# Eurus-Holmes/VAG-NMT

Hardware: AMD Instinct MI355X
Metric: training sentence-pairs/sec (Multi30K en->de, B=64) (higher is better)
Workload: dtype f32; 1 GPU; configs[1]: multimodal en->de train step, B=64/GPU, Ts=Tt=40, E=256, H=512, S=512, I=2048, Vs=8507, V=9391, dropout 0.3/0.5/0.5, tied emb, teacher_force_ratio=1; global_batch=64, parallelism=dp1, hip_graph=True

## Files before the change

include/vag_nmt.h:

```cpp
#ifndef VAG_NMT_H
#define VAG_NMT_H
#include <stddef.h>
#include <stdint.h>

#ifdef __cplusplus
extern "C" {
#endif

typedef void* vag_stream_t;

typedef struct { const float *w_ih, *w_hh, *b_ih, *b_hh; } vag_gru_w;
typedef struct { float *w_ih, *w_hh, *b_ih, *b_hh; } vag_gru_g;

typedef struct {
    const float* emb;
    vag_gru_w gru1;
    const float *attn_h, *attn_v, *c2h;
    vag_gru_w gru2;
} vag_dec_w;
typedef struct {
    float* emb;
    vag_gru_g gru1;
    float *attn_h, *attn_v, *c2h;
    vag_gru_g gru2;
// ... 328 lines not shown
#define VAG_ADAM_SCRATCH_SKIPPED_OFFSET 28
#define VAG_ADAM_SCRATCH_GUARD_OFFSET 32
int vag_clip_adam_flat(float* p, float* g, float* m, float* v, int64_t n, int nseg, const int64_t* seg_off,
                       const float* seg_lr, const float* seg_wd, float clip, float grad_scale, float beta1,
                       float beta2, float eps, int zero_grad, int32_t* step, float* norm_out, void* scratch,
                       const float* lr_dev, vag_stream_t stream);

int vag_clip_adam_shard(float* p, float* g, float* m, float* v, int64_t n, int nseg, const int64_t* seg_off,
                        const float* seg_lr, const float* seg_wd, float clip, float grad_scale, float beta1,
                        float beta2, float eps, int zero_grad, int32_t* step, float* norm_out, void* scratch,
                        const float* lr_dev, int64_t lo, int64_t hi, int phase, double* sumsq, vag_stream_t stream);

typedef struct {
    const float* enc_emb;
    vag_gru_w enc_fw, enc_bw;
    const float *im_w, *im_b, *txt_w, *txt_b, *ctx2ctx, *emb2ctx, *mlp_w;
    const float *ini_w, *ini_b;
    const float* attn_e;
    vag_dec_w dec;
    vag_head_w head;
} vag_model_w;
typedef struct {
    float* enc_emb;
    vag_gru_g enc_fw, enc_bw;
    float *im_w, *im_b, *txt_w, *txt_b, *ctx2ctx, *emb2ctx, *mlp_w;
    float *ini_w, *ini_b;
    float* attn_e;
    vag_dec_g dec;
    vag_head_g head;
} vag_model_g;
typedef struct {
    int64_t B, Ts, Tt, Es, Et, H, S, I, V, ldl;
    int32_t multimodal;
    int32_t attn_method;
    int32_t activation_vse;
    int32_t rank_kind;
    int32_t free_run;
    int32_t storage;
    float margin, loss_w, init_split, p_emb, p_ctx, p_out;
    int32_t loss_ring;
    void* guard;
    float label_smoothing;
    int32_t mrt_n;
    float mrt_alpha, mrt_scale;
    const float *mrt_cost, *mrt_valid;
} vag_step_cfg;
int64_t vag_step_ws_floats(const vag_step_cfg* cfg);
int64_t vag_step_ws_offset(const vag_step_cfg* cfg, int which);
int vag_train_step(const vag_step_cfg* cfg, const vag_model_w* w, const vag_model_g* g, const int64_t* src,
                   const int32_t* lengths, const int64_t* tgt, const float* im, const float* vocab_weight, uint64_t* rng,
                   const float* derived, float* ws, float* losses, int phases, vag_stream_t stream);
int vag_set_operator_context(const float* derived, int storage);
int vag_set_option(const char* name, int64_t value);
int vag_copy4(const void* const* src, void* const* dst, const int64_t* bytes, int n, vag_stream_t stream);
int64_t vag_derived_floats(int64_t H);
int vag_derive_weights(vag_dec_w w, const float* enc_whh_fw, const float* enc_whh_bw, int64_t H, int with_fp16,
                       float* derived, vag_stream_t stream);

int vag_recurrence_supported(int kind, int64_t B, int64_t Ts, int64_t Tt, int64_t H);
int vag_persistent_timeouts(void);
int vag_set_operator_guard(void* guard);
int vag_recurrence_time(int kind, double* ms_total, int* launches);
int vag_gemm_group_plan(int n, const int64_t* M, const int64_t* N, const int64_t* K, const int* accumulate, int* split, int* order);
int64_t vag_recurrence_sync_words(int kind, int64_t B, int64_t T);
int vag_cgru_recurrence_fwd(const float* pe, const float* mask, const float* h0, const float* xp1, vag_dec_w w, const float* wcat,
                            const float* bcat, const float* encwp, int64_t B, int64_t Ts, int64_t Tt, int64_t H, float* h1,
                            float* g1, float* qhp, float* alpha, float* h2_all, float* g2, float* psc, void* sync,
                            vag_stream_t stream);

#define VAG_COMM_ID_BYTES 128
typedef struct vag_comm_s* vag_comm_t;
int vag_comm_unique_id(void* id);
int vag_comm_init(vag_comm_t* comm, int nranks, int rank, const void* id);
int vag_comm_allreduce(vag_comm_t comm, float* buf, int64_t n, vag_stream_t stream);
int vag_comm_size(vag_comm_t comm);
int vag_comm_destroy(vag_comm_t comm);

int vag_dropout_mask(const uint64_t* rng, int which, int64_t n, float p, float* out, vag_stream_t stream);
int vag_rng_advance(uint64_t* rng, vag_stream_t stream);

#ifdef __cplusplus
}
#endif
#endif
```

vag-nmt_amd/csrc/api.hip:

```cpp
#include "../../include/vag_nmt.h"
#include "kernels.h"
#include <cstring>

#define S_(x) reinterpret_cast<hipStream_t>(x)

static inline int zero_async(void* p, size_t bytes, hipStream_t s) {
    if (bytes == 0) return VAG_OK;
    return vag_axpy_launch(0.f, reinterpret_cast<const float*>(p), reinterpret_cast<float*>(p), (int64_t)(bytes / 4), 2, s);
}
static inline int copy_async(void* dst, const void* src, size_t bytes, hipStream_t s) {
    if (bytes == 0) return VAG_OK;
    return vag_axpy_launch(1.f, reinterpret_cast<const float*>(src), reinterpret_cast<float*>(dst), (int64_t)(bytes / 4), 0, s);
}
static int linear_fwd(int64_t M, int64_t N, int64_t K, const float* x, int64_t ldx, const float* W, const float* bias,
                      int act, float* y, int64_t ldy, hipStream_t s) {
    if (M <= 256) return vag_skinny_launch(M, N, K, x, ldx, W, K, bias, nullptr, 0, y, ldy, act, s);
    return vag_gemm_launch(M, N, K, 1.f, x, ldx, 1, W, 1, K, 0.f, y, ldy, bias, act, s);
}
static int gemm_tn_acc(int64_t M, int64_t N, int64_t R, const float* A, int64_t lda, const float* B, int64_t ldb, float* C,
                       int64_t ldc, hipStream_t s, float* g_bias = nullptr) {
    if (R == 0) return VAG_OK;
    return vag_gemm_launch(M, N, R, 1.f, A, 1, lda, B, ldb, 1, 1.f, C, ldc, nullptr, VAG_ACT_NONE, s, 0, g_bias);
}
static int gemm_nn(int64_t M, int64_t N, int64_t K, const float* A, int64_t lda, const float* B, int64_t ldb, float beta,
// ... 4 lines not shown

static thread_local VagCallCtx g_base_ctx;
static thread_local VagCallCtx* g_active_ctx = nullptr;
VagCallCtx& vag_ctx() { return g_active_ctx ? *g_active_ctx : g_base_ctx; }
VagCallScope::VagCallScope(VagCallCtx& c) : ctx(c), prev(g_active_ctx) { g_active_ctx = &c; }
VagCallScope::~VagCallScope() {
    (void)vag_loss_defer_flush();
    if (ctx.leaf_on) vag_leaf_drop();
    g_active_ctx = prev;
}
static inline const float* as_f(const vag_half* p) { return reinterpret_cast<const float*>(p); }

static bool head_grads_one_plane() {
    return vag_opt().head_bf16_grads != 0 && vag_ctx().store16;
}
static int head_dt_gemm(int64_t R, int64_t E, int64_t V, const float* dlogits, int64_t ldl, const float* out_w, float* dt,
                        hipStream_t s, const void* dl16 = nullptr) {
    if (dl16) return vag_gemm_launch_planes(1, R, E, V, 1.f, reinterpret_cast<const float*>(dl16), ldl, 1, out_w, E, 1, 0.f, dt, E, s, 1);
    if (head_grads_one_plane() && R > 128) return vag_gemm_launch_planes(1, R, E, V, 1.f, dlogits, ldl, 1, out_w, E, 1, 0.f, dt, E, s);
    return gemm_nn(R, E, V, dlogits, ldl, out_w, E, 0.f, dt, E, s);
}
static int head_outw_gemm(int64_t V, int64_t E, int64_t R, const float* dlogits, int64_t ldl, const float* tmid, float* g_out_w,
                          hipStream_t s, const void* dl16 = nullptr) {
    if (R == 0) return VAG_OK;
    if (dl16) return vag_gemm_launch_planes(1, V, E, R, 1.f, reinterpret_cast<const float*>(dl16), 1, ldl, tmid, E, 1, 1.f, g_out_w, E, s, 1);
    if (head_grads_one_plane() && R > 128) return vag_gemm_launch_planes(1, V, E, R, 1.f, dlogits, 1, ldl, tmid, E, 1, 1.f, g_out_w, E, s);
    return gemm_tn_acc(V, E, R, dlogits, ldl, tmid, E, g_out_w, E, s);
}

static void* head_dl16_slot(float* logits, int64_t ldl, int64_t R, int64_t CH, int64_t E) {
    if (!head_grads_one_plane() || CH <= 128 || vag_opt().head_bf16_dlogits == 0) return nullptr;
    if (E <= 64 || vag_opt().gemm_f32mfma != 0 || vag_opt().gemm_force_tile != 0) return nullptr;
    if (CH * 3 > R * 2) return nullptr;
    return logits + CH * ldl;
}

VagOptions& vag_opt() {
    static VagOptions o;
    return o;
}

extern "C" {

int vag_version(void) { return 330; }

int vag_set_option(const char* name, int64_t value) {
    VAG_CHECK_ARG(name != nullptr);
    VagOptions& o = vag_opt();
    const struct { const char* n; int* p; } ints[] = {
        {"gemm_f32mfma", &o.gemm_f32mfma}, {"gemm_slabs", &o.gemm_slabs}, {"gemm_nogroup", &o.gemm_nogroup}, {"gemm_big", &o.gemm_big}, {"gemm_force_tile", &o.gemm_force_tile},
        {"gemm_force_splitk", &o.gemm_force_splitk}, {"head_fuse", &o.head_fuse},
        {"head_bf16_grads", &o.head_bf16_grads}, {"persistent", &o.persistent}, {"persistent_dec_bwd", &o.persistent_dec_bwd}, {"persistent_enc_bwd", &o.persistent_enc_bwd}, {"free_persistent", &o.free_persistent}, {"attn_dot_reg", &o.attn_dot_reg},
        {"persist_timing", &o.persist_timing}, {"s16_one_plane", &o.s16_one_plane}, {"leaf_queue", &o.leaf_queue}, {"attn_row", &o.attn_row}, {"dec_xcd_map", &o.dec_xcd_map}, {"loss_ride", &o.loss_ride}, {"step_fork", &o.step_fork},
        {"head_bf16_dlogits", &o.head_bf16_dlogits}};
    for (const auto& e : ints)
        if (strcmp(name, e.n) == 0) { *e.p = (int)value; return VAG_OK; }
    if (strcmp(name, "head_chunk") == 0) { o.head_chunk = value; return VAG_OK; }
    if (strcmp(name, "persist_spin_limit") == 0) { o.persist_spin_limit = value; return VAG_OK; }
#ifdef VAG_LAB
    if (strcmp(name, "dec_stamps") == 0) { o.dec_stamps = value; return VAG_OK; }
    if (strcmp(name, "dec_bwd_stamps") == 0) { o.dec_bwd_stamps = value; return VAG_OK; }
    if (strcmp(name, "gemm_debug") == 0) { o.gemm_debug = (int)value; return VAG_OK; }
    if (strcmp(name, "gemm_planes") == 0) {
        g_base_ctx.gemm_planes = (value == 2 || value == 1 || value == 11) ? (int)value : 3;
        return VAG_OK;
    }
#endif
    return VAG_EINVAL;
}

int vag_set_operator_context(const float* derived, int storage) {
    VAG_CHECK_ARG(storage == 0 || (storage == 1 && derived));
    g_base_ctx.derived = derived;
    g_base_ctx.store16 = storage == 1;
    g_base_ctx.gemm_planes = storage == 1 ? 2 : 3;
    return VAG_OK;
}

int vag_gemm_f32(int64_t M, int64_t N, int64_t K, float alpha, const float* A, int64_t sam, int64_t sak, const float* B,
                 int64_t sbk, int64_t sbn, float beta, float* C, int64_t ldc, const float* bias, int act,
                 vag_stream_t stream) {
    return vag_gemm_launch(M, N, K, alpha, A, sam, sak, B, sbk, sbn, beta, C, ldc, bias, act, S_(stream));
}

int vag_linear_fwd(int64_t M, int64_t N, int64_t K, const float* x, const float* W, const float* bias, int act, float* y,
                   vag_stream_t stream) {
    VAG_CHECK_ARG(x && W && y && M >= 0 && N > 0 && K > 0);
    return linear_fwd(M, N, K, x, K, W, bias, act, y, N, S_(stream));
}

int vag_linear_bwd(int64_t M, int64_t N, int64_t K, const float* x, const float* W, const float* y, float* dy, int act,
                   float* d_x, int accumulate_dx, float* g_W, float* g_b, vag_stream_t stream) {
    hipStream_t s = S_(stream);
    VAG_CHECK_ARG(x && W && dy && M >= 0 && N > 0 && K > 0 && (!act || y));
    if (M == 0) return VAG_OK;
    if (act) VAG_TRY(vag_tanh_bwd_launch(y, dy, dy, M * N, nullptr, 0, 0.f, s));
    if (d_x) VAG_TRY(gemm_nn(M, K, N, dy, N, W, K, accumulate_dx ? 1.f : 0.f, d_x, K, s));
    if (g_W) VAG_TRY(gemm_tn_acc(N, K, M, dy, N, x, K, g_W, K, s));
    if (g_b) VAG_TRY(vag_colsum_launch(dy, M, N, N, g_b, s));
    return VAG_OK;
}

int vag_embed_fwd(const int64_t* idx, int64_t n, const float* W, int64_t E, float* out, vag_stream_t stream) {
    return vag_embed_gather_launch(idx, 1, 0, n, 1, W, E, out, nullptr, 0, 0.f, S_(stream));
}
int vag_embed_bwd(const int64_t* idx, int64_t n, const float* d_out, int64_t E, float* g_W, vag_stream_t stream) {
    return vag_embed_scatter_launch(idx, 1, 0, n, 1, d_out, E, g_W, nullptr, 0, 0.f, S_(stream));
}

struct DerivedW {
    float *prep, *wcatT, *whh1T, *encT;
    vag_half *wcat16, *wcatT16, *whh1_16, *whh1T16, *enc16, *encT16;
    int64_t total;
};
static int64_t cgru_prep_total(int64_t H);
static DerivedW derived_layout(float* p, int64_t H) {
    DerivedW w;
    const int64_t C = 2 * H, Q = C + 3 * H;
    WsCarver c(p);
    w.prep = c.take(cgru_prep_total(H)); w.wcatT = c.take(Q * H); w.whh1T = c.take(3 * H * H); w.encT = c.take(2 * 3 * H * H);
    w.wcat16 = c.take_as<vag_half>(Q * H); w.wcatT16 = c.take_as<vag_half>(Q * H);
    w.whh1_16 = c.take_as<vag_half>(3 * H * H); w.whh1T16 = c.take_as<vag_half>(3 * H * H);
    w.enc16 = c.take_as<vag_half>(2 * 3 * H * H); w.encT16 = c.take_as<vag_half>(2 * 3 * H * H);
    w.total = c.off;
    return w;
}

struct BiGruWs {
    float *x, *xp, *hst, *gates, *dgh, *carry, *dx, *whhT, *gx;
    unsigned *sync, *sync_b;
    int64_t total;
};
static BiGruWs bigru_ws(float* ws, int64_t B, int64_t Ts, int64_t E, int64_t H) {
    BiGruWs w;
    WsCarver c(ws);
    w.x = c.take(Ts * B * E);
    w.xp = c.take(Ts * B * 6 * H);
    w.hst = c.take(2 * (Ts + 1) * B * H);
    w.gates = c.take(2 * Ts * 4 * B * H);
    w.dgh = c.take(2 * Ts * B * 3 * H);
    w.carry = c.take(4 * B * H);
    w.dx = c.take(Ts * B * E);
    w.whhT = c.take(2 * 3 * H * H);
    w.gx = c.take(3 * Ts * B * H);
    w.sync = c.take_as<unsigned>(vag_enc_persistent_sync_words(B, Ts));
    w.sync_b = c.take_as<unsigned>(vag_enc_persistent_sync_words(B, Ts));
    w.total = c.off;
    return w;
}
int64_t vag_bigru_ws_floats(int64_t B, int64_t Ts, int64_t E, int64_t H) { return bigru_ws(nullptr, B, Ts, E, H).total; }

int vag_bigru_seq_fwd(const int64_t* src, const int32_t* lengths, const float* emb, vag_gru_w fw, vag_gru_w bw, float p_emb,
                      float p_ctx, const uint64_t* rng, int64_t B, int64_t Ts, int64_t E, int64_t H, float* enc,
                      float* mask, float* ws, vag_stream_t stream) {
    hipStream_t s = S_(stream);
    VAG_CHECK_ARG(src && lengths && emb && enc && mask && ws && B > 0 && Ts > 0 && E > 0 && H > 0);
    VAG_CHECK_ARG(E % 4 == 0 && H % 4 == 0 && aligned16(ws) && aligned16(enc));
    VAG_CHECK_ARG(fw.w_ih && fw.w_hh && fw.b_ih && fw.b_hh && bw.w_ih && bw.w_hh && bw.b_ih && bw.b_hh);
    BiGruWs w = bigru_ws(ws, B, Ts, E, H);
    const int64_t R = Ts * B;
    VAG_TRY(vag_embed_gather_launch(src, 1, Ts, Ts, B, emb, E, w.x, rng, VAG_DROP_ENC_EMB, p_emb, s, mask));
    VagGemmGroup grp0;
    VAG_TRY(vag_gemm_launch(R, 3 * H, E, 1.f, w.x, E, 1, fw.w_ih, 1, E, 0.f, w.xp, 6 * H, fw.b_ih, 0, s));
    VAG_TRY(vag_gemm_launch(R, 3 * H, E, 1.f, w.x, E, 1, bw.w_ih, 1, E, 0.f, w.xp + 3 * H, 6 * H, bw.b_ih, 0, s));
    VAG_TRY(grp0.end(s));
    const int64_t BH = B * H;
    const bool s16 = vag_ctx().store16 && vag_ctx().derived;
    VAG_CHECK_ARG(!vag_ctx().store16 || (vag_ctx().derived && H % 8 == 0));
    if (!s16 && vag_opt().persistent && vag_enc_persistent_ok(B, Ts, H)) {
        return vag_enc_fwd_persistent_launch(w.xp, fw.w_hh, bw.w_hh, fw.b_hh, bw.b_hh, lengths, w.hst, w.gates, enc, w.sync, rng,
                                             p_ctx, B, Ts, H, s);
    }
    const vag_half* w16 = s16 ? derived_layout(const_cast<float*>(vag_ctx().derived), H).enc16 : nullptr;
    if (s16 && vag_opt().persistent && vag_enc_wide16_ok(B, Ts, H) && B >= 64) {
        return vag_enc_fwd_wide16_launch(w.xp, w16, w16 + 3 * H * H, fw.b_hh, bw.b_hh, lengths, w.hst, w.gates, enc,
                                         reinterpret_cast<vag_half*>(w.dgh), w.sync, rng, p_ctx, B, Ts, H, s);
    }
    {
        const VagJob zj[2] = {{nullptr, w.hst, B, H, H, H, 0}, {nullptr, w.hst + (Ts + 1) * BH, B, H, H, H, 0}};
        VAG_TRY(vag_jobs_launch(zj, 2, s));
    }
    GruStepArgs a = {};
    a.lda = H; a.ldw = H; a.ldother = 6 * H; a.ldh = H; a.ld2 = Ts * 2 * H;
    a.M = (int)B; a.K = (int)H; a.H = (int)H; a.lengths = lengths; a.comp_hidden = 1;
    for (int64_t k = 0; k < Ts; ++k) {
        for (int d = 0; d < 2; ++d) {
            const int64_t t = d == 0 ? k : Ts - 1 - k;
            const vag_gru_w& g = d == 0 ? fw : bw;
            float* hs = w.hst + d * (Ts + 1) * BH;
            GruSide& sd = a.s[d];
            sd.A = hs + k * BH; sd.W = s16 ? as_f(w16 + d * 3 * H * H) : g.w_hh; sd.bias = g.b_hh;
            sd.other = w.xp + t * B * 6 * H + d * 3 * H;
            sd.hprev = hs + k * BH; sd.hout = hs + (k + 1) * BH;
            sd.out2 = enc + t * 2 * H + d * H;
            sd.save = w.gates + (d * Ts + k) * 4 * BH;
            sd.t = (int)t;
        }
        VAG_TRY(vag_gru_step_launch(a, 2, s, s16));
    }
    VAG_TRY(vag_dropout_apply_launch(enc, B * Ts * 2 * H, 0, rng, VAG_DROP_ENC_CTX, p_ctx, s));
    return VAG_OK;
}

int vag_bigru_seq_bwd(const int64_t* src, const int32_t* lengths, vag_gru_w fw, vag_gru_w bw, float p_emb, float p_ctx,
                      const uint64_t* rng, int64_t B, int64_t Ts, int64_t E, int64_t H, float* d_enc, float* ws,
                      float* g_emb, vag_gru_g g_fw, vag_gru_g g_bw, vag_stream_t stream) {
    hipStream_t s = S_(stream);
    VAG_CHECK_ARG(src && lengths && d_enc && ws && g_emb && B > 0 && Ts > 0 && E % 4 == 0 && H % 4 == 0);
    BiGruWs w = bigru_ws(ws, B, Ts, E, H);
    const int64_t R = Ts * B, BH = B * H;
    float* d_xp = w.xp;
    const float* whhT = w.whhT;
    const bool s16 = vag_ctx().store16 && vag_ctx().derived;
    VAG_CHECK_ARG(!vag_ctx().store16 || (vag_ctx().derived && H % 8 == 0));
    if (s16) {
        whhT = as_f(derived_layout(const_cast<float*>(vag_ctx().derived), H).encT16);
    } else if (vag_ctx().derived) {
        whhT = derived_layout(const_cast<float*>(vag_ctx().derived), H).encT;
    } else {
        for (int d = 0; d < 2; ++d) {
            const vag_gru_w& g = d == 0 ? fw : bw;
            VAG_TRY(vag_transpose_launch(g.w_hh, 3 * H, H, w.whhT + d * 3 * H * H, s));
        }
    }
    const bool pers_on = vag_opt().persistent && vag_opt().persistent_enc_bwd;
    const bool wide16 = s16 && pers_on && vag_enc_wide16_ok(B, Ts, H) && B >= 64;
    const bool persist = wide16 || (!s16 && pers_on && (H == 512 || H == 256) && vag_enc_persistent_ok(B, Ts, H));
    if (wide16) {
        VAG_TRY(vag_enc_bwd_wide16_launch(reinterpret_cast<const vag_half*>(whhT), d_enc, w.gates, w.hst, lengths, rng, p_ctx, d_xp,
                                          w.dgh, reinterpret_cast<vag_half*>(w.gx), w.sync_b, B, Ts, H, s));
    } else if (persist) {
        VAG_TRY(vag_enc_bwd_persistent_launch(whhT, d_enc, w.gates, w.hst, lengths, rng, p_ctx, d_xp, w.dgh, w.sync_b, B, Ts, H, s));
    }
    GruBwdArgs a = {};
    a.ld_add = Ts * 2 * H; a.ldh = H; a.ldgi = 6 * H; a.ldgh = 3 * H;
    a.M = (int)B; a.H = (int)H; a.lengths = lengths; a.rng = rng; a.sid = VAG_DROP_ENC_CTX; a.p = p_ctx;
    int cur = 0;
    auto cell_of = [&](auto& sd, int d, int64_t k) {
        const int64_t t = d == 0 ? k : Ts - 1 - k;
        sd.dh_add = d_enc + t * 2 * H + d * H;
        sd.drop_idx0 = t * 2 * H + d * H;
        sd.save = w.gates + (d * Ts + k) * 4 * BH;
        sd.hprev = w.hst + (d * (Ts + 1) + k) * BH;
        sd.dgi = d_xp + t * B * 6 * H + d * 3 * H;
        sd.dgh = w.dgh + (d * Ts + k) * B * 3 * H;
        sd.t = (int)t;
    };
    for (int d = 0; d < 2; ++d) {
        GruBwdSide& sd = a.s[d];
        cell_of(sd, d, Ts - 1);
        sd.dh_carry = nullptr;
        sd.dh_prev = w.carry + (d * 2 + cur) * BH;
    }
    if (!persist) VAG_TRY(vag_gru_bwd_elem_launch(a, 2, s));
    GruBwdStepArgs f = {};
    f.lda = 3 * H; f.ldw = 3 * H; f.ld_add = Ts * 2 * H; f.ldh = H; f.ldgi = 6 * H; f.ldgh = 3 * H;
    f.M = (int)B; f.K = (int)(3 * H); f.H = (int)H; f.lengths = lengths; f.rng = rng; f.sid = VAG_DROP_ENC_CTX; f.p = p_ctx;
    f.has_cell = 1;
    for (int64_t k = Ts - 1; k >= 1 && !persist; --k) {
        for (int d = 0; d < 2; ++d) {
            GruBwdStepSide& sd = f.s[d];
            cell_of(sd, d, k - 1);
            sd.A = w.dgh + (d * Ts + k) * B * 3 * H;
            sd.WT = s16 ? as_f(reinterpret_cast<const vag_half*>(whhT) + d * 3 * H * H) : whhT + d * 3 * H * H;
            sd.addend = w.carry + (d * 2 + cur) * BH;
            sd.dh_direct = w.carry + (d * 2 + (cur ^ 1)) * BH;
            sd.dh_out = nullptr;
        }
        VAG_TRY(vag_gru_bwd_step_launch(f, 2, s, s16));
        cur ^= 1;
    }
    VagGemmGroup grp1;
    for (int d = 0; d < 2; ++d) {
        const vag_gru_g& gg = d == 0 ? g_fw : g_bw;
        const float* dgh = w.dgh + d * Ts * B * 3 * H;
        const float* hs = w.hst + d * (Ts + 1) * BH;
        VAG_TRY(gemm_tn_acc(3 * H, H, R, dgh, 3 * H, hs, H, gg.w_hh, H, s, gg.b_hh));
        VAG_TRY(gemm_tn_acc(3 * H, E, R, d_xp + d * 3 * H, 6 * H, w.x, E, gg.w_ih, E, s, gg.b_ih));
    }
    VAG_TRY(grp1.end(s));
    if (!vag_ctx().step_zeroed) VAG_TRY(zero_async(w.dx, R * E * sizeof(float), s));
    VagGemmGroup grp2;
    for (int d = 0; d < 2; ++d)
        VAG_TRY(gemm_nn(R, E, 3 * H, d_xp + d * 3 * H, 6 * H, (d == 0 ? fw : bw).w_ih, E, 1.f, w.dx, E, s));
    VAG_TRY(grp2.end(s));
// ... 407 lines not shown
    return cgru_bwd_scratch(scratch, B, Ts, Tt, E, H).du_all;
}
extern "C" {
int64_t vag_cgru_bwd_scratch_floats(int64_t B, int64_t Ts, int64_t Tt, int64_t E, int64_t H) {
    return cgru_bwd_scratch(nullptr, B, Ts, Tt, E, H).total;
}

int vag_cgru_attn_decode_seq_bwd_loop(const float* enc, const float* pe, const float* mask, const float* h0, const int64_t* tok,
                                 vag_dec_w w, int64_t B, int64_t Ts, int64_t Tt, int64_t E, int64_t H, int64_t V,
                                 const float* h2_all, const float* c_all, const float* e_all, float* d_h2_all,
                                 float* d_c_all, const float* d_e_all, float* ws, float* d_enc_out, int accumulate_enc,
                                 float* d_pe, float* d_h0, float* scratch, vag_stream_t stream) {
    hipStream_t s = S_(stream);
    VAG_CHECK_ARG(enc && pe && mask && h0 && tok && h2_all && c_all && e_all && d_h2_all && d_c_all && ws && d_enc_out &&
                  d_pe && d_h0 && scratch && dec_w_ok(w));
    VAG_CHECK_ARG(B > 0 && Ts > 0 && Tt > 0 && E % 4 == 0 && H % 4 == 0 && aligned16(ws) && aligned16(scratch));
    (void)V; (void)mask; (void)d_e_all;
    const int64_t C = 2 * H, Q = C + 3 * H, BH = B * H;
    CgruWs k = cgru_ws(ws, B, Ts, Tt, E, H);
    CgruPrep p = cgru_prep(k.prep, H);
    CgruBwdScratch z = cgru_bwd_scratch(scratch, B, Ts, Tt, E, H);
    const bool s16 = vag_ctx().store16;
    VAG_CHECK_ARG(!s16 || (vag_ctx().derived && H % 8 == 0));
    if (vag_ctx().derived) {
        DerivedW dw = derived_layout(const_cast<float*>(vag_ctx().derived), H);
        p = cgru_prep(dw.prep, H);
        z.wcatT = dw.wcatT; z.whh1T = dw.whh1T;
        if (s16) {
            z.wcatT = const_cast<float*>(as_f(dw.wcatT16)); z.whh1T = const_cast<float*>(as_f(dw.whh1T16));
        }
    } else {
        VAG_TRY(vag_transpose_launch(p.wcat, Q, H, z.wcatT, s));
        VAG_TRY(vag_transpose_launch(w.gru1.w_hh, 3 * H, H, z.whh1T, s));
    }
    const bool persist = !s16 && vag_opt().persistent && vag_opt().persistent_dec_bwd && vag_dec_bwd_persistent_ok(B, Ts, Tt, H);
    if (!persist) {
        GruBwdArgs a = {};
        a.ld_add = H; a.ldh = H; a.ldgi = 3 * H; a.ldgh = Q; a.M = (int)B; a.H = (int)H;
        const int64_t t = Tt - 1;
        GruBwdSide& sd = a.s[0];
        sd.dh_carry = nullptr; sd.dh_add = d_h2_all + t * BH; sd.drop_idx0 = 0;
        sd.save = k.g2 + t * 4 * BH; sd.hprev = k.h1 + t * BH;
        sd.dgi = z.dgi2 + t * B * 3 * H; sd.dgh = z.dqgh + t * B * Q + C; sd.dh_prev = z.dh1d; sd.t = 0;
        VAG_TRY(vag_gru_bwd_elem_launch(a, 1, s));
    }
    GruBwdStepArgs f = {};
    f.ld_add = H; f.ldh = H; f.M = (int)B; f.H = (int)H; f.lengths = nullptr; f.rng = nullptr; f.sid = 0; f.p = 0.f;
    if (C % 4 == 0 && aligned16(enc) && aligned16(d_c_all) && B < 65536)
        VAG_TRY(vag_skinny_batched_launch(B, Tt, Ts, C, d_c_all, B * C, C, enc, C, Ts * C, z.dah, B * Ts, Ts, s));
    else
        VAG_TRY(vag_attn_scores_ex_launch(1, enc, d_c_all, C, nullptr, nullptr, Tt * B, 1, B, Ts, C, nullptr, z.dah, s));
    if (persist) {
        VAG_TRY(vag_dec_bwd_persistent_launch(pe, k.encwp, w.attn_v, z.wcatT, z.whh1T, h0, h2_all, k.h1, k.g1, k.g2, k.qhp, k.alpha,
                                              d_h2_all, z.dah, z.dgi2, z.dqgh, z.ds, z.dgi1, z.dgh1, d_h0, k.dal, k.sync_b, B, Ts, Tt, H,
                                              s));
    }
    for (int64_t t = Tt - 1; t >= 0 && !persist; --t) {
        float* dgi2 = z.dgi2 + t * B * 3 * H;
        float* dqgh = z.dqgh + t * B * Q;
        const float* wside = s16 ? as_f(reinterpret_cast<const vag_half*>(z.wcatT) + C) : z.wcatT + C;
        VAG_TRY(vag_attn_dot_side_launch(1, k.encwp, dgi2, 3 * H, nullptr, nullptr, z.dah + t * B * Ts, B, Ts, 3 * H, z.dalpha,
                                         B, H, 3 * H, dqgh + C, Q, wside, Q, nullptr, z.dh1d, z.pbuf, H, s, s16));
        VAG_TRY(vag_attn_dq_launch(pe, k.qhp + t * B * Q, Q, w.attn_v, k.alpha + t * B * Ts, z.dalpha, z.ds + t * B * Ts, B,
                                   Ts, C, dqgh, Q, s, s16));
        f.lda = Q; f.ldw = Q; f.K = (int)C; f.ldgi = 3 * H; f.ldgh = 3 * H; f.has_cell = 1;
        GruBwdStepSide& sd = f.s[0];
        sd.A = dqgh; sd.WT = z.wcatT; sd.addend = z.pbuf; sd.dh_add = nullptr; sd.drop_idx0 = 0;
        sd.save = k.g1 + t * 4 * BH; sd.hprev = (t == 0) ? h0 : h2_all + (t - 1) * BH;
        sd.dgi = z.dgi1 + t * B * 3 * H; sd.dgh = z.dgh1 + t * B * 3 * H; sd.dh_direct = z.carry; sd.dh_out = nullptr; sd.t = 0;
        VAG_TRY(vag_gru_bwd_step_launch(f, 1, s, s16));
        f.lda = 3 * H; f.ldw = 3 * H; f.K = (int)(3 * H);
        sd.A = z.dgh1 + t * B * 3 * H; sd.WT = z.whh1T; sd.addend = z.carry;
        if (t > 0) {
            const int64_t t1 = t - 1;
            f.has_cell = 1; f.ldgi = 3 * H; f.ldgh = Q;
            sd.dh_add = d_h2_all + t1 * BH;
            sd.save = k.g2 + t1 * 4 * BH; sd.hprev = k.h1 + t1 * BH;
            sd.dgi = z.dgi2 + t1 * B * 3 * H; sd.dgh = z.dqgh + t1 * B * Q + C; sd.dh_direct = z.dh1d; sd.dh_out = nullptr;
        } else {
            f.has_cell = 0;
            sd.dh_add = nullptr; sd.save = nullptr; sd.hprev = nullptr; sd.dgi = nullptr; sd.dgh = nullptr;
            sd.dh_direct = nullptr; sd.dh_out = d_h0;
        }
        VAG_TRY(vag_gru_bwd_step_launch(f, 1, s, s16));
    }
    VAG_TRY(vag_attn_post_bwd_launch(pe, k.qhp, Q, w.attn_v, z.ds, k.alpha, d_c_all, B, Ts, Tt, C, d_pe, z.dvp, d_enc_out,
                                     accumulate_enc, s, s16));
    {
        VagGemmGroup now;
        VAG_TRY(gemm_nn(Tt * B, H, 3 * H, z.dgi2, 3 * H, w.gru2.w_ih, H, 0.f, z.du_all, H, s));
        VAG_TRY(now.end(s));
    }
    VAG_TRY(vag_attn_wsum_pair_launch(k.alpha, z.du_all, H, z.duk, k.uk, H, z.u_all, B, Ts, Tt, s));
    vag_ctx().u_all_ready = z.u_all;
    return gemm_nn(B * Ts, C, H, z.duk, H, w.c2h, C, 1.f, d_enc_out, C, s);
}

int vag_cgru_attn_decode_seq_bwd_weights(const float* h0, const int64_t* tok, vag_dec_w w, int64_t B, int64_t Ts, int64_t Tt,
                                         int64_t E, int64_t H, const float* h2_all, const float* c_all, const float* e_all,
                                         const float* d_e_all, float* ws, vag_dec_g g, float* scratch, vag_stream_t stream) {
    hipStream_t s = S_(stream);
    VAG_CHECK_ARG(h0 && tok && h2_all && c_all && e_all && ws && scratch && dec_w_ok(w));
    VAG_CHECK_ARG(g.emb && g.gru1.w_ih && g.gru1.w_hh && g.gru1.b_ih && g.gru1.b_hh && g.attn_h && g.attn_v && g.c2h &&
                  g.gru2.w_ih && g.gru2.w_hh && g.gru2.b_ih && g.gru2.b_hh);
    const int64_t C = 2 * H;
    CgruBwdScratch z = cgru_bwd_scratch(scratch, B, Ts, Tt, E, H);
    VagGemmGroup grp3;
    VAG_TRY(vag_colsum_launch(z.dvp, VAG_POST_CHUNKS(Ts) * B, C, C, g.attn_v, s));
// ... 858 lines not shown
                          int32_t* di_state, int64_t max_len, int64_t* tok_out, int64_t B, int64_t n, int64_t V, float temperature,
                          int64_t top_k, const uint64_t* rng, int32_t* n_alive, float top_p, int32_t* set_size,
                          vag_stream_t stream) {
    VAG_CHECK_ARG(di_state != nullptr);
    return vag_sample_step_p_launch(logp, ldl, M, toks, token_logp, 0, di_state, max_len, nullptr, nullptr, nullptr, tok_out, B, n,
                                    V, temperature, top_k, rng, n_alive, top_p, set_size, S_(stream));
}
int vag_sample_noise(const uint64_t* rng, int64_t di, int64_t N, int64_t V, float* out, vag_stream_t stream) {
    return vag_sample_noise_launch(rng, di, N, V, out, S_(stream));
}

int vag_mbr_supported(int64_t Nh, int64_t Lh, int64_t Nr, int64_t Lr) { return vag_mbr_supported_host(Nh, Lh, Nr, Lr); }
int vag_mbr_select(const int64_t* hyps, const int64_t* refs, const float* weights, int64_t B, int64_t Nh, int64_t Lh, int64_t Nr,
                   int64_t Lr, int utility, int32_t* matches, float* util, float* expected, int64_t* best, vag_stream_t stream) {
    return vag_mbr_select_launch(hyps, refs, weights, B, Nh, Lh, Nr, Lr, utility, matches, util, expected, best, S_(stream));
}

int vag_mrt_weights(const float* nll, const float* cost, const float* valid, int64_t B, int64_t Tt, int64_t N, float alpha, float scale,
                    float* inv_cnt, float* q, float* risk, vag_stream_t stream) {
    VAG_CHECK_ARG(risk != nullptr);
    return vag_mrt_weights_launch(nll, cost, valid, B, Tt, N, alpha, scale, inv_cnt, q, risk, nullptr, 0.f, 0, S_(stream));
}
int vag_mrt_pack(const int64_t* cand, int64_t G, int64_t Nc, int64_t L, const int64_t* gold, int64_t Tg, int include_gold, int64_t* tgt,
                 int64_t Tt, float* valid, vag_stream_t stream) {
    return vag_mrt_pack_launch(cand, G, Nc, L, gold, Tg, include_gold, tgt, Tt, valid, S_(stream));
}

int vag_clip_adam_flat(float* p, float* g, float* m, float* v, int64_t n, int nseg, const int64_t* seg_off,
                       const float* seg_lr, const float* seg_wd, float clip, float grad_scale, float beta1, float beta2,
                       float eps, int zero_grad, int32_t* step, float* norm_out, void* scratch, const float* lr_dev,
                       vag_stream_t stream) {
    return vag_clip_adam_launch(p, g, m, v, n, nseg, seg_off, seg_lr, seg_wd, clip, grad_scale, beta1, beta2, eps, zero_grad,
                                step, norm_out, scratch, lr_dev, S_(stream));
}

int vag_clip_adam_shard(float* p, float* g, float* m, float* v, int64_t n, int nseg, const int64_t* seg_off, const float* seg_lr,
                        const float* seg_wd, float clip, float grad_scale, float beta1, float beta2, float eps, int zero_grad,
                        int32_t* step, float* norm_out, void* scratch, const float* lr_dev, int64_t lo, int64_t hi, int phase,
                        double* sumsq, vag_stream_t stream) {
    return vag_clip_adam_shard_launch(p, g, m, v, n, nseg, seg_off, seg_lr, seg_wd, clip, grad_scale, beta1, beta2, eps, zero_grad,
                                      step, norm_out, scratch, lr_dev, lo, hi, phase, sumsq, S_(stream));
}

int vag_copy4(const void* const* src, void* const* dst, const int64_t* bytes, int n, vag_stream_t stream) {
    return vag_copy4_launch(src, dst, bytes, n, S_(stream));
}

int vag_recurrence_supported(int kind, int64_t B, int64_t Ts, int64_t Tt, int64_t H) {
    if (kind == 0) return vag_enc_persistent_ok(B, Ts, H) ? 1 : 0;
    if (kind == 1) return vag_dec_persistent_ok(B, Ts, Tt, H) ? 1 : 0;
    return 0;
}
int vag_persistent_timeouts(void) { return vag_persistent_timeouts_read(); }
int vag_set_operator_guard(void* guard) {
    VAG_CHECK_ARG((reinterpret_cast<uintptr_t>(guard) & 3) == 0);
    g_base_ctx.guard = reinterpret_cast<unsigned*>(guard);
    return VAG_OK;
}
int vag_gemm_group_plan(int n, const int64_t* M, const int64_t* N, const int64_t* K, const int* accumulate, int* split,
                        int* order) {
    return vag_gemm_group_plan_host(n, M, N, K, accumulate, split, order);
}
int vag_recurrence_time(int kind, double* ms_total, int* launches) { return vag_persistent_time_read(kind, ms_total, launches); }
int64_t vag_recurrence_sync_words(int kind, int64_t B, int64_t T) {
    return kind == 0 ? vag_enc_persistent_sync_words(B, T) : vag_dec_persistent_sync_words(B, T);
}
int vag_cgru_recurrence_fwd(const float* pe, const float* mask, const float* h0, const float* xp1, vag_dec_w w, const float* wcat,
                            const float* bcat, const float* encwp, int64_t B, int64_t Ts, int64_t Tt, int64_t H, float* h1,
                            float* g1, float* qhp, float* alpha, float* h2_all, float* g2, float* psc, void* sync,
                            vag_stream_t stream) {
    VAG_CHECK_ARG(dec_w_ok(w) && vag_dec_persistent_ok(B, Ts, Tt, H));
    return vag_dec_fwd_persistent_launch(pe, mask, h0, xp1, w.gru1.w_hh, w.gru1.b_hh, wcat, bcat, w.attn_v, encwp, w.gru2.b_ih, h1,
                                         g1, qhp, alpha, h2_all, g2, psc, reinterpret_cast<unsigned*>(sync), B, Ts, Tt, H,
                                         S_(stream));
}

int vag_dropout_mask(const uint64_t* rng, int which, int64_t n, float p, float* out, vag_stream_t stream) {
    VAG_CHECK_ARG(which >= 1 && which <= 3);
    return vag_dropout_mask_launch(rng, which, n, p, out, S_(stream));
}
int vag_rng_advance(uint64_t* rng, vag_stream_t stream) { return vag_rng_advance_launch(rng, S_(stream)); }

}
```

vag-nmt_amd/csrc/call_ctx.h:

```cpp
#pragma once
#include <hip/hip_runtime.h>
#include <stdint.h>
#include "../../include/vag_nmt.h"

struct LossTask {
    const float* nll = nullptr; const float* inv_cnt = nullptr; float* losses = nullptr;
    int B = 0, Tt = 0, has_vse = 0, ring = 0;
    float w_mt = 0.f, w_vse = 0.f;
};
struct RmwDefer {
    float* out = nullptr;
    const float *a1 = nullptr, *x1 = nullptr, *a2 = nullptr, *x2 = nullptr;
    const float *mask = nullptr, *dx = nullptr; float coef = 0.f;
    int64_t B = 0, Ts = 0, C = 0;
};

struct VagCallCtx {
    const float* derived = nullptr;
    bool store16 = false;
    int gemm_planes = 3;
    unsigned* guard = nullptr;

    int64_t head_chunk = 0;
    struct HeadFuse { const vag_head_g* g = nullptr; const float* d_loss = nullptr; float* dt = nullptr; bool done = false; } head_fuse;
    bool step_zeroed = false;
    bool step_gathered = false;
    bool poison_inject = false;
    bool persist_prezeroed = false;
    int loss_ring = 0;
    struct Mrt { int n = 0; float alpha = 0.f, scale = 0.f; const float* cost = nullptr; const float* valid = nullptr; } mrt;
    struct GemmScratch { float* slab = nullptr; int64_t floats = 0; unsigned* tickets = nullptr; int64_t ntickets = 0; hipStream_t stream = nullptr; } gemm_scratch;
    const float* gemm_prezeroed[4] = {nullptr, nullptr, nullptr, nullptr};
    struct LeafStream { hipStream_t stream = nullptr; hipEvent_t event = nullptr; bool used = false; } leaf_stream;

    struct RowMix { float* xmix = nullptr; float split = 0.f; const float* done = nullptr; } row_mix;
    struct Dh0Tanh { bool req = false; const float* done = nullptr; } dh0_tanh;
    struct LossDefer { bool on = false; LossTask task; hipStream_t stream = nullptr; } loss_defer;
    RmwDefer rmw;
    bool leaf_on = false;
    const float* u_all_ready = nullptr;
};

VagCallCtx& vag_ctx();

struct VagCallScope {
    VagCallCtx& ctx;
    VagCallCtx* prev;
    explicit VagCallScope(VagCallCtx& c);
    ~VagCallScope();
    VagCallScope(const VagCallScope&) = delete;
    VagCallScope& operator=(const VagCallScope&) = delete;
};
```

vag-nmt_amd/csrc/common.h:

```cpp
#pragma once
#include <hip/hip_runtime.h>
#include <stdint.h>
#include <stddef.h>

#define VAG_OK 0
#define VAG_EINVAL (-22)
#define VAG_ENOSYS (-38)

#define VAG_CHECK_ARG(cond)                     \
    do {                                        \
        if (!(cond)) return VAG_EINVAL;         \
    } while (0)

#define VAG_LAUNCH_CHECK()                                  \
    do {                                                    \
        hipError_t e__ = hipGetLastError();                 \
        if (e__ != hipSuccess) return (int)e__;             \
    } while (0)

#define VAG_TRY(expr)                  \
    do {                               \
        int r__ = (expr);              \
        if (r__ != 0) return r__;      \
    } while (0)
// ... 26 lines not shown
}
__device__ __forceinline__ float wave_sum(float v) { return wave_allreduce<false>(v); }
__device__ __forceinline__ float wave_max(float v) { return wave_allreduce<true>(v); }
__device__ __forceinline__ float vag_tanh(float x) {
    float e = __expf(2.0f * x);
    return 1.0f - 2.0f * __builtin_amdgcn_rcpf(e + 1.0f);
}
__device__ __forceinline__ float vag_sigmoid(float x) { return __builtin_amdgcn_rcpf(1.0f + __expf(-x)); }

__device__ __host__ __forceinline__ uint64_t vag_mix64(uint64_t z) {
    z += 0x9E3779B97F4A7C15ull;
    z = (z ^ (z >> 30)) * 0xBF58476D1CE4E5B9ull;
    z = (z ^ (z >> 27)) * 0x94D049BB133111EBull;
    return z ^ (z >> 31);
}
__device__ __forceinline__ float vag_drop_mul(const uint64_t* rng, uint32_t stream_id, uint64_t idx, float p) {
    if (rng == nullptr || p <= 0.0f) return 1.0f;
    uint64_t key = vag_mix64(rng[0] ^ (rng[1] * 0xD1342543DE82EF95ull) ^ ((uint64_t)stream_id << 56));
    uint64_t r = vag_mix64(key + idx);
    float u = (float)(r >> 40) * (1.0f / 16777216.0f);
    return (u >= p) ? 1.0f / (1.0f - p) : 0.0f;
}

typedef _Float16 vag_half;
__device__ __forceinline__ float h16_lo(unsigned p) { return (float)__builtin_bit_cast(vag_half, (unsigned short)(p & 0xffffu)); }
__device__ __forceinline__ float h16_hi(unsigned p) { return (float)__builtin_bit_cast(vag_half, (unsigned short)(p >> 16)); }
template <bool XH> __device__ __forceinline__ float4 ld4_any(const float* base, int64_t elem) {
    if (XH) {
        const uint2 p = *reinterpret_cast<const uint2*>(reinterpret_cast<const vag_half*>(base) + elem);
        return make_float4(h16_lo(p.x), h16_hi(p.x), h16_lo(p.y), h16_hi(p.y));
    }
    return *reinterpret_cast<const float4*>(base + elem);
}
template <bool XH> __device__ __forceinline__ float ld1_any(const float* base, int64_t elem) {
    if (XH) return (float)reinterpret_cast<const vag_half*>(base)[elem];
    return base[elem];
}

struct VagOptions {
    int gemm_f32mfma = 0;
    int gemm_big = 1;
    int gemm_slabs = 1;
    int gemm_nogroup = 0;
    int gemm_force_tile = 0;
    int gemm_force_splitk = 0;
    int gemm_debug = 0;
    int64_t head_chunk = -1;
    int head_fuse = 1;
    int head_bf16_grads = 1;
    int persistent = 1;
    int persistent_dec_bwd = 1;
    int persistent_enc_bwd = 1;
    int attn_dot_reg = 1;
    int free_persistent = 1;
    int s16_one_plane = 1;
    int head_bf16_dlogits = 1;
    int leaf_queue = 1;
    int attn_row = 1;
    int loss_ride = 1;
    int dec_xcd_map = 33;
    int step_fork = 0;
    int64_t persist_spin_limit = 0;
    int persist_timing = 0;
    int64_t dec_bwd_stamps = 0;
    int64_t dec_stamps = 0;
};
VagOptions& vag_opt();

enum { VAG_ACT_NONE = 0, VAG_ACT_TANH = 1 };
enum { VAG_DROP_ENC_EMB = 1, VAG_DROP_ENC_CTX = 2, VAG_DROP_DEC_OUT = 3 };

int vag_gemm_launch(int64_t M, int64_t N, int64_t K, float alpha, const float* A, int64_t sam, int64_t sak,
                    const float* B, int64_t sbk, int64_t sbn, float beta, float* C, int64_t ldc,
                    const float* bias, int act, hipStream_t stream, int c_half = 0,
                    float* rowsum = nullptr,
                    int a_bf16 = 0);
int vag_gemm_launch_planes(int planes, int64_t M, int64_t N, int64_t K, float alpha, const float* A, int64_t sam, int64_t sak,
                           const float* B, int64_t sbk, int64_t sbn, float beta, float* C, int64_t ldc, hipStream_t stream,
                           int a_bf16 = 0);
int64_t vag_logits_parts_count(int64_t M, int64_t N, int64_t K, const float* A, int64_t lda, const float* W, int64_t ldw);
int vag_logits_parts_launch(int64_t M, int64_t N, int64_t K, const float* A, int64_t lda, const float* W, int64_t ldw,
                            const float* bias, float* out, int64_t ldo, float* parts, hipStream_t stream);
int vag_skinny_launch(int64_t M, int64_t N, int64_t K, const float* A, int64_t lda, const float* W, int64_t ldw,
                      const float* bias, const float* addend, int64_t ldadd, float* out, int64_t ldo, int act,
                      hipStream_t stream, bool w16 = false);
int vag_attn_dot_side_launch(int mode, const float* x, const float* q, int64_t ldq, const float* v, const float* mask,
                             const float* addend, int64_t N, int64_t Ts, int64_t W, float* out, int64_t M, int64_t Np,
                             int64_t K, const float* A, int64_t lda, const float* Wt, int64_t ldw, const float* pbias,
                             const float* padd, float* P, int64_t ldp, hipStream_t stream, bool s16 = false);
int vag_skinny_gather_launch(int64_t M, int64_t N, int64_t K, const float* table, int64_t ldt, const int64_t* idx, const float* W,
                             int64_t ldw, const float* bias, float* out, int64_t ldo, float* gathered, int64_t ldg,
                             hipStream_t stream);
int vag_skinny3_launch(int64_t M, int64_t N, const float* const* A, const int64_t* lda, const float* const* W, const int64_t* ldw,
                       const int64_t* K, const float* const* bias, float* out, int64_t ldo, int act, const uint64_t* rng, int sid,
                       float p, int64_t drop_idx0, hipStream_t stream, const float* addend = nullptr, int64_t ldadd = 0,
                       const float* addend2 = nullptr, const int64_t* idx2 = nullptr, int64_t ldadd2 = 0);
int vag_skinny_batched_launch(int64_t nb, int64_t M, int64_t N, int64_t K, const float* A, int64_t lda, int64_t bsA,
                              const float* W, int64_t ldw, int64_t bsW, float* out, int64_t ldo, int64_t bsO,
                              hipStream_t stream);
int vag_skinny_nn_launch(int64_t M, int64_t N, int64_t K, const float* A, int64_t lda, const float* B, int64_t ldb,
                         float beta, float* C, int64_t ldc, hipStream_t stream,
                         float* out2 = nullptr, int64_t ldo2 = 0, float scale2 = 0.f, int acc2 = 0);
void vag_gemm_group_begin();
int vag_gemm_group_end(hipStream_t stream);
void vag_gemm_group_abort();
struct VagGemmGroup {
// ... 59 lines not shown
```

vag-nmt_amd/csrc/kernels.h:

```cpp
#pragma once
#include "common.h"
#include "call_ctx.h"
#include "../../include/vag_nmt.h"

static inline int64_t round64(int64_t n) { return (n + 63) & ~63ll; }
struct WsCarver {
    float* base;
    int64_t off = 0;
    explicit WsCarver(float* b) : base(b) {}
    float* take(int64_t n) {
        float* q = base ? base + off : nullptr;
        off += round64(n);
        return q;
    }
    template <class T> T* take_as(int64_t n) {
        return reinterpret_cast<T*>(take((n * (int64_t)sizeof(T) + 3) / 4));
    }
};
struct DecTables {
    float *embp, *embw3, *encw2;
    unsigned long long* cand;
    int64_t total;
};
DecTables vag_dec_tables(float* base, int64_t B, int64_t Ts, int64_t Tt, int64_t E, int64_t H, int64_t V, bool token_only = false);
// ... 74 lines not shown
                        int64_t C, float* alpha, float* ctx, hipStream_t s);
int vag_softmax_bwd_launch(const float* alpha, const float* dalpha, int64_t N, int64_t Ts, float* dscore, hipStream_t s);
int vag_attn_dq_launch(const float* pe, const float* q, int64_t ldq, const float* v, const float* alpha,
                       const float* dalpha, float* dscore, int64_t N, int64_t Ts, int64_t C, float* dq, int64_t lddq,
                       hipStream_t s, bool x16 = false);
int vag_attn_post_bwd_launch(const float* pe, const float* q_all, int64_t ldq, const float* v, const float* ds_all,
                             const float* alpha_all, const float* dc_all, int64_t B, int64_t Ts, int64_t Tt,
                             int64_t C, float* d_pe, float* dvp, float* d_enc, int accumulate_enc, hipStream_t s,
                             bool x16 = false);
int vag_outer2_launch(const float* a1, const float* x1, const float* a2, const float* x2, int64_t B, int64_t Ts,
                      int64_t C, float* out, int accumulate, hipStream_t s);

inline bool vag_label_smoothing_ok(float eps) { return eps >= 0.f && eps < 1.f; }
int vag_lse_nll_launch(const float* logits, int64_t ldl, int64_t rows, int64_t V, const int64_t* tgt, int64_t B,
                       int64_t Tt, const float* vw, float* lse, float* nll, int64_t* argmax, int64_t argmax_stride,
                       float* logp_out, int64_t ldlp, hipStream_t s, float eps);
int vag_inv_cnt_launch(const int64_t* tgt, int64_t B, int64_t Tt, float* inv_cnt, hipStream_t s);
int vag_loss_mt_launch(const float* nll, const float* inv_cnt, int64_t B, int64_t Tt, float* loss, hipStream_t s);
int vag_loss_mt_mix_launch(const float* nll, const float* inv_cnt, int64_t B, int64_t Tt, float* losses, float w_mt,
                           float w_vse, int has_vse, hipStream_t s);
int vag_ce_bwd_launch(float* logits, int64_t ldl, int64_t rows, int64_t V, const int64_t* tgt, int64_t B, int64_t Tt,
                      const float* vw, const float* lse, const float* inv_cnt, const float* d_loss, hipStream_t s,
                      float eps);
int vag_ce_bwd_colsum_launch(float* logits, int64_t ldl, int64_t rows, int64_t V, const int64_t* tgt, int64_t B, int64_t Tt,
                             const float* vw, const float* lse, const float* inv_cnt, const float* d_loss, float* g_bias,
                             hipStream_t s, void* out16, float eps);

int vag_logsoftmax_bwd_launch(const float* logp, int64_t ldlp, float* d, int64_t ldd, int64_t rows, int64_t V,
                              hipStream_t s);

int vag_l2norm_fwd_launch(const float* y, int64_t B, int64_t S, float* nrm, float* out, hipStream_t s);
int vag_l2norm_bwd_launch(const float* y, const float* nrm, const float* out, const float* d_out, int64_t B, int64_t S,
                          int act, float* dy, hipStream_t s);
int vag_rank_loss_launch(const float* scores, int64_t B, float margin, int kind, float* G, float* loss, hipStream_t s,
                         const float* g_scale = nullptr);
int vag_retrieval_rank_launch(const float* scores, int64_t N, int* ranks, hipStream_t s);
int vag_scale_by_dev_launch(float* x, int64_t n, const float* scalar, hipStream_t s);

int vag_clip_adam_shard_launch(float* p, float* g, float* m, float* v, int64_t n, int nseg, const int64_t* seg_off,
                               const float* seg_lr, const float* seg_wd, float clip, float grad_scale, float beta1, float beta2,
                               float eps, int zero_grad, int32_t* step, float* norm_out, void* scratch, const float* lr_dev,
                               int64_t lo, int64_t hi, int phase, double* sumsq, hipStream_t s);
int vag_clip_adam_launch(float* p, float* g, float* m, float* v, int64_t n, int nseg, const int64_t* seg_off,
                         const float* seg_lr, const float* seg_wd, float clip, float grad_scale, float beta1,
                         float beta2, float eps, int zero_grad, int32_t* step, float* norm_out, void* scratch, const float* lr_dev,
                         hipStream_t s);

bool vag_enc_persistent_ok(int64_t B, int64_t Ts, int64_t H);
int64_t vag_enc_persistent_sync_words(int64_t B, int64_t Ts);
int vag_enc_fwd_persistent_launch(const float* xp, const float* w_fw, const float* w_bw, const float* b_fw, const float* b_bw,
                                  const int* lengths, float* hst, float* gates, float* enc, unsigned* sync, const uint64_t* rng,
                                  float p_ctx, int64_t B, int64_t Ts, int64_t H, hipStream_t s);
int vag_enc_bwd_persistent_launch(const float* whhT, const float* d_enc, const float* gates, const float* hst, const int* lengths,
                                  const uint64_t* rng, float p_ctx, float* d_xp, float* dgh, unsigned* sync, int64_t B, int64_t Ts,
                                  int64_t H, hipStream_t s);
bool vag_enc_wide16_ok(int64_t B, int64_t Ts, int64_t H);
int vag_enc_fwd_wide16_launch(const float* xp, const vag_half* w16_fw, const vag_half* w16_bw, const float* b_fw, const float* b_bw,
                              const int* lengths, float* hst, float* gates, float* enc, vag_half* hx, unsigned* sync, const uint64_t* rng,
                              float p_ctx, int64_t B, int64_t Ts, int64_t H, hipStream_t s);
int vag_enc_bwd_wide16_launch(const vag_half* wt16, const float* d_enc, const float* gates, const float* hst, const int* lengths,
                              const uint64_t* rng, float p_ctx, float* d_xp, float* dgh, vag_half* gx, unsigned* sync, int64_t B,
                              int64_t Ts, int64_t H, hipStream_t s);
int vag_gemm_group_plan_host(int n, const int64_t* M, const int64_t* N, const int64_t* K, const int* accumulate, int* split,
                             int* order);
int vag_persistent_timeouts_read(void);
unsigned* vag_persist_guard(void);
int vag_persistent_time_read(int kind, double* ms_total, int* launches);
bool vag_dec_bwd_persistent_ok(int64_t B, int64_t Ts, int64_t Tt, int64_t H);
int vag_dec_bwd_persistent_launch(const float* pe, const float* encwp, const float* v, const float* wcatT, const float* whh1T,
                                  const float* h0, const float* h2_all, const float* h1, const float* g1, const float* g2,
                                  const float* qhp, const float* alpha, const float* d_h2_all, const float* dah, float* dgi2,
                                  float* dqgh, float* ds, float* dgi1, float* dgh1, float* d_h0, float* dal, unsigned* sync,
                                  int64_t B, int64_t Ts, int64_t Tt, int64_t H, hipStream_t s);
float* vag_cgru_bwd_scratch_de(float* scratch, int64_t B, int64_t Ts, int64_t Tt, int64_t E, int64_t H);
float* vag_cgru_bwd_scratch_du(float* scratch, int64_t B, int64_t Ts, int64_t Tt, int64_t E, int64_t H);
int vag_attn_dot_row_launch(bool bwd, const float* x, const float* q, int64_t ldq, const float* mask, const float* alpha, int64_t B,
                            int64_t Ts, int64_t C, float* wout, float* sum, hipStream_t s);
int vag_rank_bwd_launch(const float* G, const float* im, const float* sv, const float* d_loss, int64_t B, int64_t S, float* d_im,
                        float* d_s, hipStream_t s);
int vag_attn_wsum_pair_launch(const float* a, const float* y, int64_t Wy, float* out_src, const float* x, int64_t Wx, float* out_time,
                              int64_t B, int64_t Ts, int64_t T, hipStream_t s);
int vag_loss_defer_flush();
bool vag_attn_row_gru_ok(int64_t N, int64_t Ts, int64_t H, int64_t W2);
int vag_attn_row_gru_launch(const float* pe, const float* q, int64_t ldq, const float* v, const float* mask, const float* keys,
                            const float* x2, int64_t N, int64_t rps, int64_t Ts, int64_t H, int64_t W2, const float* b_ih,
                            const float* hp, int64_t ldhp, const float* hprev, float* alpha, float* hout, float* out2, hipStream_t s);
int vag_rmw_defer_flush(hipStream_t s);
bool vag_rmw_defer_meanpool(const float* mask, const float* dx, float coef, int64_t B, int64_t Ts, int64_t C, float* out, int accumulate);
void vag_step_zero_ranges(float* ws_enc, float* ws_dec, int64_t B, int64_t Ts, int64_t Tt, int64_t Es, int64_t Et, int64_t H,
                          unsigned** p, int64_t* n);
bool vag_dec_persistent_ok(int64_t B, int64_t Ts, int64_t Tt, int64_t H);
int64_t vag_dec_persistent_sync_words(int64_t B, int64_t Tt);
int vag_dec_fwd_persistent_launch(const float* pe, const float* mask, const float* h0, const float* xp1, const float* W1,
                                  const float* b1, const float* wcat, const float* bcat, const float* v, const float* encwp,
                                  const float* b_ih2, float* h1, float* g1, float* qhp, float* alpha, float* h2_all, float* g2,
                                  float* psc, unsigned* sync, int64_t B, int64_t Ts, int64_t Tt, int64_t H, hipStream_t s);
bool vag_dec_free_persistent_ok(int64_t B, int64_t Ts, int64_t Tt, int64_t E, int64_t H, int64_t V);
int vag_dec_free_persistent_launch(const float* pe, const float* mask, const float* h0, const float* W1, const float* b1,
                                   const float* wcat, const float* bcat, const float* v, const float* encwp, const float* b_ih2,
                                   float* h1, float* g1, float* qhp, float* alpha, float* h2_all, float* g2, float* psc,
                                   unsigned* sync, const DecTables& tab, const float* hw1, const float* hb1, const float* hb2,
                                   const float* hb3, const float* out_w, const float* out_b, float* tmid, float* logits, int64_t ldl,
                                   int64_t* tok, const uint64_t* rng, float p_out, int64_t B, int64_t Ts, int64_t Tt, int64_t E,
                                   int64_t H, int64_t V, hipStream_t s);

int64_t vag_beam_scratch_bytes_impl(int64_t B, int64_t k, int64_t V);
int vag_beam_step_launch(float* logp, int64_t ldl, float* nll, int64_t* beam, int64_t di, int32_t* di_state,
                         int64_t max_len, const float* h_in, float* h_out, int64_t* tok_out, int64_t B, int64_t k,
                         int64_t V, int64_t H, int32_t* n_alive, void* scratch, hipStream_t s, const float* parts = nullptr,
                         int64_t nparts = 0, int flags = 0);
int vag_beam_finish_launch(const float* nll, const int64_t* beam, int64_t max_len, int64_t steps, int64_t B, int64_t k,
                           int64_t* out, float* best, hipStream_t s);
int vag_beam_ens_step_launch(const float* const* logp, const int64_t* ldl, int64_t M, float* nll, int64_t* beam, int64_t di,
                             int32_t* di_state, int64_t max_len, const float* const* h_in, float* const* h_out, const int64_t* H,
                             int64_t* tok_out, int64_t B, int64_t k, int64_t V, int32_t* n_alive, void* scratch, hipStream_t s,
                             int flags = 0);
int vag_beam_finish_nbest_launch(const float* nll, const int64_t* beam, int64_t max_len, int64_t steps, int64_t B, int64_t k,
                                 int64_t n, int64_t* out, float* scores, hipStream_t s);
int vag_beam_finish_nbest_slots_launch(const float* nll, const int64_t* beam, int64_t max_len, int64_t steps, int64_t B, int64_t k,
                                       int64_t n, int64_t* out, float* scores, int64_t* slots, hipStream_t s);
int64_t vag_beam_div_scratch_bytes_impl(int64_t B, int64_t k, int64_t V);
int vag_beam_div_step_launch(const float* const* logp, const int64_t* ldl, int64_t M, float* nll, int64_t* beam, int64_t di,
                             int32_t* di_state, int64_t max_len, const float* const* h_in, float* const* h_out, const int64_t* H,
                             int64_t* tok_out, int64_t B, int64_t k, int64_t V, int32_t* n_alive, void* scratch, int flags,
                             int64_t groups, float strength, hipStream_t s);
int64_t vag_beam_req_scratch_bytes_impl(int64_t B, int64_t k, int64_t V);
// ... 82 lines not shown
```

vag-nmt_amd/csrc/persist.hip:

```cpp
#include "kernels.h"
#include "gemm_shared.h"
#include <algorithm>
#include <atomic>
#include <mutex>

namespace {

typedef unsigned __attribute__((address_space(1))) gu32;
#define RLX_AGENT __ATOMIC_RELAXED, __HIP_MEMORY_SCOPE_AGENT

constexpr unsigned SPIN_LIMIT = 1u << 19;
__device__ unsigned g_persist_timeouts;
__device__ unsigned g_persist_guard[2];
__device__ __forceinline__ void note_timeout(unsigned* err, unsigned* guard) {
    __hip_atomic_store((gu32*)err, 1u, RLX_AGENT);
    __hip_atomic_store((gu32*)guard, 1u, RLX_AGENT);
    atomicAdd(guard + 1, 1u);
    atomicAdd(&g_persist_timeouts, 1u);
}

struct EncPArgs {
    const float* xp;
    const float* W[2];
    const float* bias[2];
// ... 65 lines not shown
#ifndef VAG_TAGGED
#define VAG_TAGGED 1
#endif
__device__ __forceinline__ float tag1(float x) { return VAG_TAGGED ? __uint_as_float(__float_as_uint(x) | 1u) : x; }
__device__ __forceinline__ float4 tag4(float4 v) { return make_float4(tag1(v.x), tag1(v.y), tag1(v.z), tag1(v.w)); }
__device__ __forceinline__ unsigned tagbits(float4 v) {
    return __float_as_uint(v.x) & __float_as_uint(v.y) & __float_as_uint(v.z) & __float_as_uint(v.w);
}
template <int N>
__device__ __forceinline__ void ld_rows_tagged(const float* p, float4 (&a)[N], float4 (&b)[N], unsigned spin, bool& dead,
                                               unsigned* err, unsigned* guard) {
    for (unsigned tries = 0;; ++tries) {
        ld_rows_sc1<N>(p, a, b);
        if (!VAG_TAGGED) return;
        unsigned m = 1u;
#pragma unroll
        for (int s = 0; s < N; ++s) m &= tagbits(a[s]) & tagbits(b[s]);
        if (__all((m & 1u) != 0u) || dead) return;
        if (tries > spin) { if ((threadIdx.x & 63) == 0) note_timeout(err, guard); dead = true; return; }
    }
}
__device__ __forceinline__ void st_sc1_f1(float* p, float v) {
    asm volatile("global_store_dword %0, %1, off sc1\n\ts_nop 1" :: "v"(p), "v"(v) : "memory");
}
__device__ __forceinline__ int ld_row(int lane) { return 4 * ((lane >> 2) & 3) + (lane >> 4); }
__device__ __forceinline__ int ld_src4(int lane) { return 4 * (16 * (lane & 3) + 4 * ((lane & 15) >> 2) + (lane >> 4)); }
__device__ __forceinline__ float4 perm4(float4 v, int src4) {
    float4 o;
    o.x = __int_as_float(__builtin_amdgcn_ds_bpermute(src4, __float_as_int(v.x)));
    o.y = __int_as_float(__builtin_amdgcn_ds_bpermute(src4, __float_as_int(v.y)));
    o.z = __int_as_float(__builtin_amdgcn_ds_bpermute(src4, __float_as_int(v.z)));
    o.w = __int_as_float(__builtin_amdgcn_ds_bpermute(src4, __float_as_int(v.w)));
    return o;
}
__device__ __forceinline__ void split8(const float4 a, const float4 b, bf16x8 (&p)[3]) {
    unsigned q[3][4];
    split3(a.x, a.y, q[0][0], q[1][0], q[2][0]);
    split3(a.z, a.w, q[0][1], q[1][1], q[2][1]);
    split3(b.x, b.y, q[0][2], q[1][2], q[2][2]);
    split3(b.z, b.w, q[0][3], q[1][3], q[2][3]);
#pragma unroll
    for (int i = 0; i < 3; ++i) {
        const u32x4 t = {q[i][0], q[i][1], q[i][2], q[i][3]};
        p[i] = __builtin_bit_cast(bf16x8, t);
    }
}
__device__ __forceinline__ f32x4 mma6(const bf16x8 (&a)[3], const bf16x8 (&b)[3], f32x4 acc) {
    acc = __builtin_amdgcn_mfma_f32_16x16x32_bf16(a[0], b[2], acc, 0, 0, 0);
    acc = __builtin_amdgcn_mfma_f32_16x16x32_bf16(a[1], b[1], acc, 0, 0, 0);
    acc = __builtin_amdgcn_mfma_f32_16x16x32_bf16(a[2], b[0], acc, 0, 0, 0);
    acc = __builtin_amdgcn_mfma_f32_16x16x32_bf16(a[0], b[1], acc, 0, 0, 0);
    acc = __builtin_amdgcn_mfma_f32_16x16x32_bf16(a[1], b[0], acc, 0, 0, 0);
    acc = __builtin_amdgcn_mfma_f32_16x16x32_bf16(a[0], b[0], acc, 0, 0, 0);
    return acc;
}

template <int KS>
__global__ __launch_bounds__(512, 1) void enc_fwd_persistent_kernel(EncPArgs a) {
    __shared__ __attribute__((aligned(16))) float lds[21504];
    const int wg = blockIdx.x;
    const int cs = wg % a.CS, rt = a.rt0 + (wg / a.CS) % a.RTP, d = wg / (a.CS * a.RTP);
    const int lane = threadIdx.x & 63, wave = threadIdx.x >> 6;
    const int H = a.H, B = a.B, Ts = a.Ts;
    const int m0 = rt * 16, u0 = cs * 16;
    const int fr = lane & 15, fg = lane >> 4;
    const int kbase = wave * (H >> 3);
    const int64_t BH = (int64_t)B * H;

    bf16x8 wf[KS][3][3];
    {
        const float* W = a.W[d];
#pragma unroll
        for (int s = 0; s < KS; ++s)
#pragma unroll
            for (int j = 0; j < 3; ++j) {
                const float* p = W + (int64_t)(j * H + u0 + fr) * H + kbase + 32 * s + 8 * fg;
                split8(*reinterpret_cast<const float4*>(p), *reinterpret_cast<const float4*>(p + 4), wf[s][j]);
            }
    }
    const int erow = lane >> 2, equad = lane & 3, eslot = erow + 16 * equad;
    const int em = m0 + erow, eu = u0 + 4 * equad;
    const bool eok = wave == 0 && em < B;
    float4 bb[3] = {make_float4(0, 0, 0, 0), make_float4(0, 0, 0, 0), make_float4(0, 0, 0, 0)};
    int len = 0;
    if (eok) {
#pragma unroll
        for (int j = 0; j < 3; ++j) bb[j] = *reinterpret_cast<const float4*>(a.bias[d] + j * H + eu);
        len = a.lengths[em];
    }
    float4 hp = make_float4(0.f, 0.f, 0.f, 0.f);

    float* hs = a.hst + (int64_t)d * (Ts + 1) * BH;
    if (eok) *reinterpret_cast<float4*>(hs + (int64_t)em * H + eu) = hp;
    const __amdgpu_buffer_rsrc_t rs = __builtin_amdgcn_make_buffer_rsrc(hs, 0, (unsigned)((int64_t)(Ts + 1) * BH * 4), 0x00020000);
    gu32* cnt = (gu32*)(a.cnt + ((int64_t)d * a.RT + rt) * Ts);
    const int lrow = min(m0 + ld_row(lane), B - 1);
    const int src4 = ld_src4(lane);
    float4* red = reinterpret_cast<float4*>(lds);
    bool dead = false;

    for (int k = 0; k < Ts; ++k) {
        const int t = d == 0 ? k : Ts - 1 - k;
        float4 xo[3];
        if (eok) {
            const float* xp = a.xp + ((int64_t)t * B + em) * 6 * H + d * 3 * H + eu;
#pragma unroll
// ... 221 lines not shown
            const float cr[4] = {c[0].x, c[0].y, c[0].z, c[0].w}, cz[4] = {c[1].x, c[1].y, c[1].z, c[1].w};
            const float cn[4] = {c[2].x, c[2].y, c[2].z, c[2].w};
            const float xr[4] = {xo[0].x, xo[0].y, xo[0].z, xo[0].w}, xz[4] = {xo[1].x, xo[1].y, xo[1].z, xo[1].w};
            const float xn[4] = {xo[2].x, xo[2].y, xo[2].z, xo[2].w};
            const float hpv[4] = {hp.x, hp.y, hp.z, hp.w};
            float rr[4], zz[4], nn[4], ho[4], o2[4];
#pragma unroll
            for (int i = 0; i < 4; ++i) {
                rr[i] = vag_sigmoid(cr[i] + xr[i]);
                zz[i] = vag_sigmoid(cz[i] + xz[i]);
                nn[i] = vag_tanh(xn[i] + rr[i] * cn[i]);
                const float hn = (1.f - zz[i]) * nn[i] + zz[i] * hpv[i];
                ho[i] = active ? hn : hpv[i];
                o2[i] = active ? hn : 0.f;
            }
            hp = make_float4(ho[0], ho[1], ho[2], ho[3]);
            const int64_t o = (int64_t)em * H + eu;
            st_sc1_h4(hx + (int64_t)(k + 1) * BH + o, ho[0], ho[1], ho[2], ho[3]);
            asm volatile("s_waitcnt vmcnt(0)" ::: "memory");
            if (lane == 0) __hip_atomic_fetch_add(cnt + k, 1u, RLX_AGENT);
            *reinterpret_cast<float4*>(hs + (int64_t)(k + 1) * BH + o) = hp;
            float* sv = a.gates + ((int64_t)(d * Ts + k) * 4) * BH + o;
            *reinterpret_cast<float4*>(sv) = make_float4(rr[0], rr[1], rr[2], rr[3]);
            *reinterpret_cast<float4*>(sv + BH) = make_float4(zz[0], zz[1], zz[2], zz[3]);
            *reinterpret_cast<float4*>(sv + 2 * BH) = make_float4(nn[0], nn[1], nn[2], nn[3]);
            *reinterpret_cast<float4*>(sv + 3 * BH) = c[2];
            const int64_t eo = ((int64_t)em * Ts + t) * 2 * H + d * H + eu;
            if (a.rng && a.p_ctx > 0.f) {
#pragma unroll
                for (int i = 0; i < 4; ++i) o2[i] *= vag_drop_mul(a.rng, VAG_DROP_ENC_CTX, (uint64_t)eo + i, a.p_ctx);
            }
            *reinterpret_cast<float4*>(a.enc + eo) = make_float4(o2[0], o2[1], o2[2], o2[3]);
        } else if (lane == 0) {
            __hip_atomic_fetch_add(cnt + k, 1u, RLX_AGENT);
        }
    }
}

struct EncBArgs {
    const float* WT[2];
    const float* d_enc;
    const float* gates;
    const float* hst;
    const int* lengths;
    const uint64_t* rng; float p_ctx;
    float* d_xp;
    float* dgh;
    unsigned* cnt;
    unsigned* err;
    unsigned* guard;
    unsigned spin;
    int B, Ts, H, RT, CS;
    int rt0, RTP;
};
template <int KS>
__global__ __launch_bounds__(512, 1) void enc_bwd_persistent_kernel(EncBArgs a) {
    __shared__ __attribute__((aligned(16))) float lds[21504];
    const int wg = blockIdx.x;
    const int cs = wg % a.CS, rt = a.rt0 + (wg / a.CS) % a.RTP, d = wg / (a.CS * a.RTP);
    const int lane = threadIdx.x & 63, wave = threadIdx.x >> 6;
    const int H = a.H, B = a.B, Ts = a.Ts, K = 3 * H;
    const int m0 = rt * 16, u0 = cs * 16;
    const int fr = lane & 15, fg = lane >> 4;
    const int kbase = wave * (K >> 3);
    const int64_t BH = (int64_t)B * H;
    bf16x8 wf[KS][3];
    {
        const float* WT = a.WT[d] + (int64_t)(u0 + fr) * K + kbase + 8 * fg;
#pragma unroll
        for (int s = 0; s < KS; ++s) split8(*reinterpret_cast<const float4*>(WT + 32 * s), *reinterpret_cast<const float4*>(WT + 32 * s + 4), wf[s]);
    }
    const int erow = lane >> 2, equad = lane & 3, eslot = erow + 16 * equad;
    const int em = m0 + erow, eu = u0 + 4 * equad;
    const bool eok = wave == 0 && em < B;
    const int len = eok ? a.lengths[em] : 0;
    float4 carry = make_float4(0.f, 0.f, 0.f, 0.f);
    float* dghd = a.dgh + (int64_t)d * Ts * B * K;
    gu32* cnt = (gu32*)(a.cnt + ((int64_t)d * a.RT + rt) * Ts);
    const int lrow = min(m0 + ld_row(lane), B - 1);
    const int src4 = ld_src4(lane);
    float4* red = reinterpret_cast<float4*>(lds);
    bool dead = false;
    const int64_t ld_add = (int64_t)Ts * 2 * H;

    for (int k = Ts - 1; k >= 0; --k) {
        const int t = d == 0 ? k : Ts - 1 - k;
        float4 sv[4], hp, e4;
        if (eok) {
            const int64_t o = (int64_t)em * H + eu;
            const float* g = a.gates + ((int64_t)(d * Ts + k) * 4) * BH + o;
#pragma unroll
            for (int q = 0; q < 4; ++q) sv[q] = *reinterpret_cast<const float4*>(g + q * BH);
            hp = *reinterpret_cast<const float4*>(a.hst + ((int64_t)d * (Ts + 1) + k) * BH + o);
            e4 = *reinterpret_cast<const float4*>(a.d_enc + (int64_t)em * ld_add + (int64_t)t * 2 * H + d * H + eu);
        }
        float4 dh = carry;
        if (k < Ts - 1) {
            if (threadIdx.x == 0 && !dead) {
                unsigned spins = 0;
                while (__hip_atomic_load(cnt + (k + 1), RLX_AGENT) < (unsigned)a.CS) {
                    if (++spins > a.spin) { note_timeout(a.err, a.guard); dead = true; break; }
                }
            }
            __syncthreads();
            f32x4 acc = {0.f, 0.f, 0.f, 0.f};
            float4 ga[KS], gb[KS];
            ld_rows_sc1<KS>(dghd + ((int64_t)(k + 1) * B + lrow) * K + kbase + 8 * (lane & 3), ga, gb);
#pragma unroll
            for (int s = 0; s < KS; ++s) {
                bf16x8 hf[3];
                split8(perm4(ga[s], src4), perm4(gb[s], src4), hf);
                acc = mma6(wf[s], hf, acc);
            }
            red[wave * 64 + lane] = make_float4(acc[0], acc[1], acc[2], acc[3]);
            __syncthreads();
            if (wave == 0) {
#pragma unroll
                for (int w = 0; w < 8; ++w) {
                    const float4 o = red[w * 64 + eslot];
                    dh.x += o.x; dh.y += o.y; dh.z += o.z; dh.w += o.w;
                }
            }
        }
        if (eok) {
            const bool active = t < len;
            float dhv[4] = {dh.x, dh.y, dh.z, dh.w};
            float gi[3][4], gh[3][4], cy[4];
            if (!active) {
#pragma unroll
                for (int q = 0; q < 4; ++q) { gi[0][q] = gi[1][q] = gi[2][q] = gh[0][q] = gh[1][q] = gh[2][q] = 0.f; cy[q] = dhv[q]; }
            } else {
                const float ev[4] = {e4.x, e4.y, e4.z, e4.w};
                const float r_[4] = {sv[0].x, sv[0].y, sv[0].z, sv[0].w}, z_[4] = {sv[1].x, sv[1].y, sv[1].z, sv[1].w};
                const float n_[4] = {sv[2].x, sv[2].y, sv[2].z, sv[2].w}, hn[4] = {sv[3].x, sv[3].y, sv[3].z, sv[3].w};
                const float hpv[4] = {hp.x, hp.y, hp.z, hp.w};
#pragma unroll
                for (int q = 0; q < 4; ++q) {
                    float e = ev[q];
                    if (a.rng && a.p_ctx > 0.f)
                        e *= vag_drop_mul(a.rng, VAG_DROP_ENC_CTX, (uint64_t)em * ld_add + (uint64_t)t * 2 * H + d * H + eu + q, a.p_ctx);
                    const float x = dhv[q] + e;
                    const float dn_pre = x * (1.f - z_[q]) * (1.f - n_[q] * n_[q]);
                    const float dz_pre = x * (hpv[q] - n_[q]) * z_[q] * (1.f - z_[q]);
                    const float dr_pre = dn_pre * hn[q] * r_[q] * (1.f - r_[q]);
                    gi[0][q] = dr_pre; gi[1][q] = dz_pre; gi[2][q] = dn_pre;
                    gh[0][q] = dr_pre; gh[1][q] = dz_pre; gh[2][q] = dn_pre * r_[q];
                    cy[q] = x * z_[q];
                }
            }
            carry = make_float4(cy[0], cy[1], cy[2], cy[3]);
            float* gho = dghd + ((int64_t)k * B + em) * K + eu;
#pragma unroll
            for (int g = 0; g < 3; ++g) st_sc1_f4(gho + g * H, make_float4(gh[g][0], gh[g][1], gh[g][2], gh[g][3]));
            asm volatile("s_waitcnt vmcnt(0)" ::: "memory");
            if (lane == 0) __hip_atomic_fetch_add(cnt + k, 1u, RLX_AGENT);
            float* gio = a.d_xp + ((int64_t)t * B + em) * 6 * H + d * 3 * H + eu;
#pragma unroll
            for (int g = 0; g < 3; ++g) *reinterpret_cast<float4*>(gio + g * H) = make_float4(gi[g][0], gi[g][1], gi[g][2], gi[g][3]);
        }
    }
}

struct EncWBArgs {
    const vag_half* WT16[2];
    const float* d_enc;
    const float* gates;
    const float* hst;
    const int* lengths;
    const uint64_t* rng; float p_ctx;
    float* d_xp;
    float* dgh;
    vag_half* gx;
    unsigned* cnt;
    unsigned* err;
    unsigned* guard;
    unsigned spin;
    int B, Ts, H, RG, CS;
};
template <> __device__ __forceinline__ void ld16_sc1<6>(const vag_half* p, u32x4 (&v)[6]) {
    asm volatile("global_load_dwordx4 %0, %6, off sc1\n\tglobal_load_dwordx4 %1, %6, off offset:64 sc1\n\t"
                 "global_load_dwordx4 %2, %6, off offset:128 sc1\n\tglobal_load_dwordx4 %3, %6, off offset:192 sc1\n\t"
                 "global_load_dwordx4 %4, %6, off offset:256 sc1\n\tglobal_load_dwordx4 %5, %6, off offset:320 sc1\n\t"
                 "s_waitcnt vmcnt(0)"
                 : "=&v"(v[0]), "=&v"(v[1]), "=&v"(v[2]), "=&v"(v[3]), "=&v"(v[4]), "=&v"(v[5]) : "v"(p) : "memory");
}
template <> __device__ __forceinline__ void ld16_sc1<12>(const vag_half* p, u32x4 (&v)[12]) {
    asm volatile("global_load_dwordx4 %0, %12, off sc1\n\tglobal_load_dwordx4 %1, %12, off offset:64 sc1\n\t"
                 "global_load_dwordx4 %2, %12, off offset:128 sc1\n\tglobal_load_dwordx4 %3, %12, off offset:192 sc1\n\t"
                 "global_load_dwordx4 %4, %12, off offset:256 sc1\n\tglobal_load_dwordx4 %5, %12, off offset:320 sc1\n\t"
                 "global_load_dwordx4 %6, %12, off offset:384 sc1\n\tglobal_load_dwordx4 %7, %12, off offset:448 sc1\n\t"
                 "global_load_dwordx4 %8, %12, off offset:512 sc1\n\tglobal_load_dwordx4 %9, %12, off offset:576 sc1\n\t"
                 "global_load_dwordx4 %10, %12, off offset:640 sc1\n\tglobal_load_dwordx4 %11, %12, off offset:704 sc1\n\t"
                 "s_waitcnt vmcnt(0)"
                 : "=&v"(v[0]), "=&v"(v[1]), "=&v"(v[2]), "=&v"(v[3]), "=&v"(v[4]), "=&v"(v[5]), "=&v"(v[6]), "=&v"(v[7]),
                   "=&v"(v[8]), "=&v"(v[9]), "=&v"(v[10]), "=&v"(v[11])
                 : "v"(p) : "memory");
}

template <int HK>
__global__ __launch_bounds__(512, 1) void enc_bwd_wide16_kernel(EncWBArgs a) {
    extern __shared__ __attribute__((aligned(16))) float wide_lds[];
    constexpr float GSCALE = 4096.f;
    const int wg = blockIdx.x;
    const int cs = wg % a.CS, rg = (wg / a.CS) % a.RG, d = wg / (a.CS * a.RG);
    const int lane = threadIdx.x & 63, wave = threadIdx.x >> 6;
    const int kq = wave & 3, ch = wave >> 2;
    const int er = wave & 3, ech = wave >> 2;
    const int H = a.H, B = a.B, Ts = a.Ts, K = 3 * H;
// ... 728 lines not shown
                const float4 x = *reinterpret_cast<const float4*>(bs_s + 48 + g * 8 + 4 * hq);
                const float4 y = *reinterpret_cast<const float4*>(hp_s + fr * 24 + g * 8 + 4 * hq);
                bi[g][0] = x.x; bi[g][1] = x.y; bi[g][2] = x.z; bi[g][3] = x.w;
                hh[g][0] = y.x; hh[g][1] = y.y; hh[g][2] = y.z; hh[g][3] = y.w;
            }
            const float* hr = hh[0];
            const float* hz = hh[1];
            const float* hn = hh[2];
            const float4 h1v = *reinterpret_cast<const float4*>(hs_s + fr * 8 + 4 * hq);
            const float h1a[4] = {h1v.x, h1v.y, h1v.z, h1v.w};
            float rr[4], zz[4], nn[4], ho[4];
#pragma unroll
            for (int q = 0; q < 4; ++q) {
                rr[q] = vag_sigmoid(gi[0][q] + bi[0][q] + hr[q]);
                zz[q] = vag_sigmoid(gi[1][q] + bi[1][q] + hz[q]);
                nn[q] = vag_tanh(gi[2][q] + bi[2][q] + rr[q] * hn[q]);
                ho[q] = (1.f - zz[q]) * nn[q] + zz[q] * h1a[q];
            }
            const float4 h2v = tag4(make_float4(ho[0], ho[1], ho[2], ho[3]));
            *reinterpret_cast<float4*>(hs_s + 128 + fr * 8 + 4 * hq) = h2v;
            const int64_t o = (int64_t)em * H + eu;
            st_sc1_f4(a.h2_all + (int64_t)t * BH + o, h2v);
            if (!VAG_TAGGED) asm volatile("s_waitcnt vmcnt(0)" ::: "memory");
            if (VAG_TAGGED && tx == 0) arrive(c1 + t * CNT_WORDS, i);
            float* sv = a.g2 + (int64_t)t * 4 * BH + o;
            *reinterpret_cast<float4*>(sv) = make_float4(rr[0], rr[1], rr[2], rr[3]);
            *reinterpret_cast<float4*>(sv + BH) = make_float4(zz[0], zz[1], zz[2], zz[3]);
            *reinterpret_cast<float4*>(sv + 2 * BH) = make_float4(nn[0], nn[1], nn[2], nn[3]);
            *reinterpret_cast<float4*>(sv + 3 * BH) = make_float4(hn[0], hn[1], hn[2], hn[3]);
        }
        if (tx == 0 && (!VAG_TAGGED || !eok)) arrive(c1 + t * CNT_WORDS, i);
    }
#ifdef VAG_LAB
    if (!FREE && a.dbg && threadIdx.x == 0 && i == 0 && rt < 8) a.dbg[(Tt + 2) * 8 + rt] = __builtin_amdgcn_s_memrealtime();
#endif
#undef VAG_STAMP
}

struct DecBArgs {
    const float *pe, *encwp, *v, *wcatT, *whh1T;
    const float *h0, *h2_all, *h1, *g1, *g2, *qhp, *alpha;
    const float *d_h2_all, *dah;
    float *dgi2, *dqgh, *ds, *dgi1, *dgh1, *d_h0;
    float* dal;
    unsigned* cnt;
    unsigned* err;
    unsigned* guard;
    unsigned spin;
    unsigned long long* dbg;
    int B, Ts, Tt, H, RT;
    int rt0;
    int xcd_map;
    int h0_tanh;
};

__device__ __forceinline__ void cell_bwd4(const float (&dh)[4], const float4 (&sv)[4], const float4 hp, float (&gi)[3][4],
                                          float (&gh)[3][4], float (&direct)[4]) {
    const float r_[4] = {sv[0].x, sv[0].y, sv[0].z, sv[0].w}, z_[4] = {sv[1].x, sv[1].y, sv[1].z, sv[1].w};
    const float n_[4] = {sv[2].x, sv[2].y, sv[2].z, sv[2].w}, hn[4] = {sv[3].x, sv[3].y, sv[3].z, sv[3].w};
    const float hpv[4] = {hp.x, hp.y, hp.z, hp.w};
#pragma unroll
    for (int q = 0; q < 4; ++q) {
        const float dn_pre = dh[q] * (1.f - z_[q]) * (1.f - n_[q] * n_[q]);
        const float dz_pre = dh[q] * (hpv[q] - n_[q]) * z_[q] * (1.f - z_[q]);
        const float dr_pre = dn_pre * hn[q] * r_[q] * (1.f - r_[q]);
        gi[0][q] = dr_pre; gi[1][q] = dz_pre; gi[2][q] = dn_pre;
        gh[0][q] = dr_pre; gh[1][q] = dz_pre; gh[2][q] = dn_pre * r_[q];
        direct[q] = dh[q] * z_[q];
    }
}

template <int WGS>
__global__ __launch_bounds__(512, 1) void dec_bwd_persistent_kernel(DecBArgs a) {
    extern __shared__ __attribute__((aligned(16))) float dlds[];
    constexpr int H = WGS * DEC_U, C = 2 * H, Q = C + 3 * H;
    constexpr unsigned PER_SHARD = WGS / SHARDS;
    int i, rt;
    dec_slice_map<WGS>(a.xcd_map, a.rt0, i, rt);
    const int lane = threadIdx.x & 63, wave = threadIdx.x >> 6;
    const int B = a.B, Ts = a.Ts, Tt = a.Tt;
#ifdef VAG_LAB
#define VAG_BPSTAMP(k) do { if (a.dbg && blockIdx.x == 0 && threadIdx.x == 0) a.dbg[Tt * 8 + (k)] = __builtin_amdgcn_s_memrealtime(); } while (0)
#else
#define VAG_BPSTAMP(k) do { } while (0)
#endif
    VAG_BPSTAMP(0);
    const int m0 = rt * 16, u0 = i * DEC_U;
    const int fr = lane & 15, fg = lane >> 4;
    const int64_t BH = (int64_t)B * H;
    const int NP = 16 * Ts;
    float4* red = reinterpret_cast<float4*>(dlds);
    float* pe_s = dlds + 2048;
    float* ew_t = pe_s + NP * 16;
    float* da_s = ew_t + 24 * NP;
    float* al_s = da_s + NP;
    float* gi_s = al_s + NP;
    float* d1_s = gi_s + 384;
    float* pb_s = d1_s + 128;
    float* c1_s = pb_s + 128;
    float* dq_s = c1_s + 128;
    float* wb_s = dq_s + 256;
    constexpr int WBLD = C + 4;

    constexpr int KB = C / 8 / 32, KC = 3 * H / 8 / 32;
    bf16x8 wc[KC][3];
    {
        const float* pc = a.whh1T + (int64_t)(u0 + (fr & 7)) * (3 * H) + wave * (3 * H >> 3) + 8 * fg;
#pragma unroll
        for (int s = 0; s < KC; ++s) split8(*reinterpret_cast<const float4*>(pc + 32 * s), *reinterpret_cast<const float4*>(pc + 32 * s + 4), wc[s]);
    }
    for (int x = threadIdx.x; x < 8 * (C / 4); x += 512) {
        const int u = x / (C / 4), c4 = x - u * (C / 4);
        *reinterpret_cast<float4*>(wb_s + u * WBLD + 4 * c4) = *reinterpret_cast<const float4*>(a.wcatT + (int64_t)(u0 + u) * Q + 4 * c4);
    }
    const float* wb_row = wb_s + (fr & 7) * WBLD + wave * (C >> 3) + 8 * fg;
    const float* wa_row = a.wcatT + (int64_t)(u0 + (ld_row(lane) & 7)) * Q + C + wave * (3 * H >> 3) + 8 * (lane & 3);
    for (int x = threadIdx.x; x < NP * 4; x += 512) {
        const int P = x >> 2, c4 = x & 3;
        const int r = P / Ts, sp = P - r * Ts, b = min(m0 + r, B - 1);
        reinterpret_cast<float4*>(pe_s)[x] = *reinterpret_cast<const float4*>(a.pe + ((int64_t)b * Ts + sp) * C + 16 * i + 4 * c4);
    }
    for (int x = threadIdx.x; x < NP * 6; x += 512) {
        const int hf = x & 1, g = (x >> 1) % 3, P = x / 6;
        const int r = P / Ts, sp = P - r * Ts, b = min(m0 + r, B - 1);
        const float4 e = *reinterpret_cast<const float4*>(a.encwp + ((int64_t)b * Ts + sp) * 3 * H + g * H + u0 + 4 * hf);
        const int col = g * 8 + 4 * hf;
        ew_t[(col + 0) * NP + P] = e.x; ew_t[(col + 1) * NP + P] = e.y; ew_t[(col + 2) * NP + P] = e.z; ew_t[(col + 3) * NP + P] = e.w;
    }
    const int hq = (threadIdx.x >> 4) & 1;
    const int em = m0 + fr, eu = u0 + 4 * hq;
    const bool ep = threadIdx.x < 32, eok = ep && em < B;
    const int lrow = min(m0 + ld_row(lane), B - 1);
    const int src4 = ld_src4(lane);
    gu32* cA = (gu32*)(a.cnt + ((int64_t)0 * a.RT + rt) * Tt * CNT_WORDS);
    gu32* cB = (gu32*)(a.cnt + ((int64_t)1 * a.RT + rt) * Tt * CNT_WORDS);
    gu32* cC = (gu32*)(a.cnt + ((int64_t)2 * a.RT + rt) * Tt * CNT_WORDS);
    bool dead = false;
    const float vq = a.v[16 * i + (threadIdx.x & 15)];

    auto cell2_bwd = [&](int t, const float (&dh2)[4], const float4 (&sv)[4], const float4 hp) {
        float gi[3][4], gh[3][4], dr[4];
        cell_bwd4(dh2, sv, hp, gi, gh, dr);
#pragma unroll
        for (int g = 0; g < 3; ++g) {
            st_sc1_f4(a.dqgh + ((int64_t)t * B + em) * Q + C + g * H + eu, make_float4(gh[g][0], gh[g][1], gh[g][2], gh[g][3]));
            const float4 x = make_float4(gi[g][0], gi[g][1], gi[g][2], gi[g][3]);
            *reinterpret_cast<float4*>(gi_s + fr * 24 + g * 8 + 4 * hq) = x;
            *reinterpret_cast<float4*>(a.dgi2 + ((int64_t)t * B + em) * 3 * H + g * H + eu) = x;
        }
        *reinterpret_cast<float4*>(d1_s + fr * 8 + 4 * hq) = make_float4(dr[0], dr[1], dr[2], dr[3]);
    };
    auto red4 = [&](float (&x)[4]) {
        float4 sum = red[hq * 16 + fr];
#pragma unroll
        for (int w = 1; w < 8; ++w) {
            const float4 o = red[w * 64 + hq * 16 + fr];
            sum.x += o.x; sum.y += o.y; sum.z += o.z; sum.w += o.w;
        }
        x[0] = sum.x; x[1] = sum.y; x[2] = sum.z; x[3] = sum.w;
    };

    VAG_BPSTAMP(1);
    if (ep) {
        if (eok) {
            const float4 d = *reinterpret_cast<const float4*>(a.d_h2_all + (int64_t)(Tt - 1) * BH + (int64_t)em * H + eu);
            const float dh2[4] = {d.x, d.y, d.z, d.w};
            const int64_t o = (int64_t)em * H + eu;
            float4 sv[4];
#pragma unroll
            for (int q = 0; q < 4; ++q) sv[q] = *reinterpret_cast<const float4*>(a.g2 + ((int64_t)(Tt - 1) * 4 + q) * BH + o);
            cell2_bwd(Tt - 1, dh2, sv, *reinterpret_cast<const float4*>(a.h1 + (int64_t)(Tt - 1) * BH + o));
        } else {
#pragma unroll
            for (int g = 0; g < 3; ++g) *reinterpret_cast<float4*>(gi_s + fr * 24 + g * 8 + 4 * hq) = make_float4(0.f, 0.f, 0.f, 0.f);
            *reinterpret_cast<float4*>(d1_s + fr * 8 + 4 * hq) = make_float4(0.f, 0.f, 0.f, 0.f);
        }
    }
    __syncthreads();

#ifdef VAG_LAB
    const bool stamp = a.dbg != nullptr && blockIdx.x == 0 && threadIdx.x == 0;
#define VAG_STAMP(k) do { if (stamp) a.dbg[t * 8 + (k)] = __builtin_amdgcn_s_memrealtime(); } while (0)
#else
#define VAG_STAMP(k) do { } while (0)
#endif
    for (int t = Tt - 1; t >= 0; --t) {
        VAG_STAMP(0);
        for (int P = threadIdx.x; P < NP; P += 512) {
            const int r = P / Ts;
            const float* g = gi_s + r * 24;
            float acc = 0.f;
#pragma unroll
            for (int k = 0; k < 24; ++k) acc += ew_t[k * NP + P] * g[k];
            if (m0 + r < B)
                atomicAdd(a.dal + (((int64_t)t * ACC_SHARDS + (i & (ACC_SHARDS - 1))) * B + m0 + r) * Ts + (P - r * Ts), acc);
        }
        asm volatile("s_waitcnt vmcnt(0)" ::: "memory");
        __syncthreads();
        if (threadIdx.x == 0) arrive(cA + t * CNT_WORDS, i);
        VAG_STAMP(1);
        float4 hga[KC], hgb[KC];
        static_assert(KC == 6 || KC == 3, "ld_acc_shards_and_rows<KC>");
        float al0 = 0.f, al1 = 0.f, dh0 = 0.f, dh1_ = 0.f;
        const int x0 = threadIdx.x, x1 = threadIdx.x + 512;
        {
            const int r0 = min(x0, NP - 1) / Ts, r1 = min(x1, NP - 1) / Ts;
            const int64_t o0 = ((int64_t)t * B + min(m0 + r0, B - 1)) * Ts + (min(x0, NP - 1) - r0 * Ts);
            const int64_t o1 = ((int64_t)t * B + min(m0 + r1, B - 1)) * Ts + (min(x1, NP - 1) - r1 * Ts);
            al0 = a.alpha[o0]; dh0 = a.dah[o0];
            if (x1 < NP) { al1 = a.alpha[o1]; dh1_ = a.dah[o1]; }
            const float qv = a.qhp[((int64_t)t * B + min(m0 + (int)((threadIdx.x & 255) >> 4), B - 1)) * Q + 16 * i + (threadIdx.x & 15)];
            wait_count(cA + t * CNT_WORDS, PER_SHARD, a.err, a.guard, a.spin, dead);
            VAG_STAMP(2);
            float v0, v1;
            const float* p0 = a.dal + o0 + (int64_t)t * (ACC_SHARDS - 1) * B * Ts;
            const float* p1 = a.dal + o1 + (int64_t)t * (ACC_SHARDS - 1) * B * Ts;
            ld_acc_shards_and_rows(p0, p1, (int64_t)B * Ts, v0, v1,
                                   a.dqgh + ((int64_t)t * B + lrow) * Q + C + wave * (3 * H >> 3) + 8 * (lane & 3), hga, hgb);
            if (x0 < NP) { da_s[x0] = v0 + dh0; al_s[x0] = al0; }
            if (x1 < NP) { da_s[x1] = v1 + dh1_; al_s[x1] = al1; }
            __syncthreads();
            for (int r = wave; r < 16; r += 8) {
                float dot = 0.f;
                for (int sp = lane; sp < Ts; sp += 64) dot += al_s[r * Ts + sp] * da_s[r * Ts + sp];
                dot = wave_sum(dot);
                for (int sp = lane; sp < Ts; sp += 64) {
                    const float d = al_s[r * Ts + sp] * (da_s[r * Ts + sp] - dot);
                    da_s[r * Ts + sp] = d;
                    if (((r * Ts + sp) & (WGS - 1)) == i && m0 + r < B) a.ds[((int64_t)t * B + m0 + r) * Ts + sp] = d;
                }
            }
            __syncthreads();
            {
                const int tt = threadIdx.x & 255, half = threadIdx.x >> 8;
                const int r = tt >> 4, c = tt & 15;
                const float* pr = pe_s + (int64_t)r * Ts * 16 + c;
                const float* dsr = da_s + r * Ts;
                float acc0 = 0.f, acc1 = 0.f;
                int sp = half;
                for (; sp + 2 < Ts; sp += 4) {
                    const float t0 = vag_tanh(pr[sp * 16] + qv), t1 = vag_tanh(pr[(sp + 2) * 16] + qv);
                    acc0 += dsr[sp] * (1.f - t0 * t0);
                    acc1 += dsr[sp + 2] * (1.f - t1 * t1);
                }
                if (sp < Ts) { const float t0 = vag_tanh(pr[sp * 16] + qv); acc0 += dsr[sp] * (1.f - t0 * t0); }
                float* half_s = reinterpret_cast<float*>(red);
                if (half) half_s[tt] = acc0 + acc1;
                __syncthreads();
                if (!half) dq_s[tt] = ((acc0 + acc1) + half_s[tt]) * vq;
            }
            __syncthreads();
            if (threadIdx.x < 64) {
                const int r = threadIdx.x >> 2, c4 = threadIdx.x & 3;
                if (m0 + r < B) st_sc1_f4(a.dqgh + ((int64_t)t * B + m0 + r) * Q + 16 * i + 4 * c4, *reinterpret_cast<const float4*>(dq_s + r * 16 + 4 * c4));
                asm volatile("s_waitcnt vmcnt(0)" ::: "memory");
                if (threadIdx.x == 0) arrive(cB + t * CNT_WORDS, i);
            }
        }
        VAG_STAMP(3);
        {
            f32x4 acc = {0.f, 0.f, 0.f, 0.f};
#pragma unroll
            for (int s = 0; s < KC; ++s) {
                bf16x8 wf[3], hf[3];
                split8(perm4(*reinterpret_cast<const float4*>(wa_row + 32 * s), src4),
                       perm4(*reinterpret_cast<const float4*>(wa_row + 32 * s + 4), src4), wf);
                split8(perm4(hga[s], src4), perm4(hgb[s], src4), hf);
                acc = mma6(wf, hf, acc);
            }
            red[wave * 64 + lane] = make_float4(acc[0], acc[1], acc[2], acc[3]);
            __syncthreads();
            if (ep) {
                float x[4];
                red4(x);
                const float4 d1 = *reinterpret_cast<const float4*>(d1_s + fr * 8 + 4 * hq);
                *reinterpret_cast<float4*>(pb_s + fr * 8 + 4 * hq) = make_float4(x[0] + d1.x, x[1] + d1.y, x[2] + d1.z, x[3] + d1.w);
            }
        }
        float4 s1[4], hp1 = make_float4(0.f, 0.f, 0.f, 0.f);
        if (eok) {
            const int64_t o = (int64_t)em * H + eu;
#pragma unroll
            for (int q = 0; q < 4; ++q) s1[q] = *reinterpret_cast<const float4*>(a.g1 + ((int64_t)t * 4 + q) * BH + o);
            hp1 = *reinterpret_cast<const float4*>((t > 0 ? a.h2_all + (int64_t)(t - 1) * BH : a.h0) + o);
        }
        VAG_STAMP(4);
        wait_count(cB + t * CNT_WORDS, PER_SHARD, a.err, a.guard, a.spin, dead);
        VAG_STAMP(5);
        {
            f32x4 acc = {0.f, 0.f, 0.f, 0.f};
            float4 ga[KB], gb[KB];
            ld_rows_sc1<KB>(a.dqgh + ((int64_t)t * B + lrow) * Q + wave * (C >> 3) + 8 * (lane & 3), ga, gb);
#pragma unroll
            for (int s = 0; s < KB; ++s) { ga[s] = perm4(ga[s], src4); gb[s] = perm4(gb[s], src4); }
#pragma unroll
            for (int s = 0; s < KB; ++s) {
                bf16x8 wf[3], hf[3];
                split8(*reinterpret_cast<const float4*>(wb_row + 32 * s), *reinterpret_cast<const float4*>(wb_row + 32 * s + 4), wf);
                split8(ga[s], gb[s], hf);
                acc = mma6(wf, hf, acc);
            }
            red[wave * 64 + lane] = make_float4(acc[0], acc[1], acc[2], acc[3]);
        }
        __syncthreads();
        if (ep) {
            float x[4];
            red4(x);
            if (eok) {
                const float4 pbv = *reinterpret_cast<const float4*>(pb_s + fr * 8 + 4 * hq);
                const float dh1[4] = {x[0] + pbv.x, x[1] + pbv.y, x[2] + pbv.z, x[3] + pbv.w};
                float gi[3][4], gh[3][4], dr[4];
                cell_bwd4(dh1, s1, hp1, gi, gh, dr);
#pragma unroll
                for (int g = 0; g < 3; ++g)
                    st_sc1_f4(a.dgh1 + ((int64_t)t * B + em) * 3 * H + g * H + eu, make_float4(gh[g][0], gh[g][1], gh[g][2], gh[g][3]));
                asm volatile("s_waitcnt vmcnt(0)" ::: "memory");
                if (threadIdx.x == 0) arrive(cC + t * CNT_WORDS, i);
#pragma unroll
                for (int g = 0; g < 3; ++g)
                    *reinterpret_cast<float4*>(a.dgi1 + ((int64_t)t * B + em) * 3 * H + g * H + eu) = make_float4(gi[g][0], gi[g][1], gi[g][2], gi[g][3]);
                *reinterpret_cast<float4*>(c1_s + fr * 8 + 4 * hq) = make_float4(dr[0], dr[1], dr[2], dr[3]);
            } else if (threadIdx.x == 0) {
                arrive(cC + t * CNT_WORDS, i);
            }
        }
        float4 dadd = make_float4(0.f, 0.f, 0.f, 0.f), s2[4], hp2 = make_float4(0.f, 0.f, 0.f, 0.f);
        if (eok && t > 0) {
            const int64_t o = (int64_t)em * H + eu;
            dadd = *reinterpret_cast<const float4*>(a.d_h2_all + (int64_t)(t - 1) * BH + o);
#pragma unroll
            for (int q = 0; q < 4; ++q) s2[q] = *reinterpret_cast<const float4*>(a.g2 + ((int64_t)(t - 1) * 4 + q) * BH + o);
            hp2 = *reinterpret_cast<const float4*>(a.h1 + (int64_t)(t - 1) * BH + o);
        }
        VAG_STAMP(6);
        wait_count(cC + t * CNT_WORDS, PER_SHARD, a.err, a.guard, a.spin, dead);
        VAG_STAMP(7);
        {
            f32x4 acc = {0.f, 0.f, 0.f, 0.f};
            float4 ga[KC], gb[KC];
            ld_rows_sc1<KC>(a.dgh1 + ((int64_t)t * B + lrow) * 3 * H + wave * (3 * H >> 3) + 8 * (lane & 3), ga, gb);
#pragma unroll
            for (int s = 0; s < KC; ++s) { ga[s] = perm4(ga[s], src4); gb[s] = perm4(gb[s], src4); }
#pragma unroll
            for (int s = 0; s < KC; ++s) {
                bf16x8 hf[3];
                split8(ga[s], gb[s], hf);
                acc = mma6(wc[s], hf, acc);
            }
            red[wave * 64 + lane] = make_float4(acc[0], acc[1], acc[2], acc[3]);
        }
        __syncthreads();
        if (ep) {
            float x[4];
            red4(x);
            if (eok) {
                const float4 c1 = *reinterpret_cast<const float4*>(c1_s + fr * 8 + 4 * hq);
                const float dh2[4] = {x[0] + c1.x + dadd.x, x[1] + c1.y + dadd.y, x[2] + c1.z + dadd.z, x[3] + c1.w + dadd.w};
                if (t > 0) cell2_bwd(t - 1, dh2, s2, hp2);
                else {
                    float4 o = make_float4(dh2[0], dh2[1], dh2[2], dh2[3]);
                    if (a.h0_tanh) {
                        const float4 h = *reinterpret_cast<const float4*>(a.h0 + (int64_t)em * H + eu);
                        o.x *= 1.f - h.x * h.x; o.y *= 1.f - h.y * h.y; o.z *= 1.f - h.z * h.z; o.w *= 1.f - h.w * h.w;
                    }
                    *reinterpret_cast<float4*>(a.d_h0 + (int64_t)em * H + eu) = o;
                }
            }
        }
        __syncthreads();
    }
    VAG_BPSTAMP(2);
#undef VAG_STAMP
}

__global__ __launch_bounds__(256) void zero_u32_kernel(unsigned* p, int n) {
    const int i = blockIdx.x * 256 + threadIdx.x;
    if (i < n) p[i] = 0u;
}
__global__ __launch_bounds__(256) void zero2_u32_kernel(unsigned* p, int n, unsigned* q, int m) {
    const int i = blockIdx.x * 256 + threadIdx.x;
    if (i < n) p[i] = 0u;
    else if (i - n < m) q[i - n] = 0u;
}

}

struct PersistTimer { hipEvent_t e0 = nullptr, e1 = nullptr; bool pending = false; double ms = 0.0; int n = 0; };
static PersistTimer g_ptimer[4];
static std::mutex g_ptimer_mu;
static void ptimer_collect(PersistTimer& t) {
    if (!t.pending) return;
    float ms = 0.f;
    if (hipEventSynchronize(t.e1) == hipSuccess && hipEventElapsedTime(&ms, t.e0, t.e1) == hipSuccess) { t.ms += ms; ++t.n; }
    t.pending = false;
}
static bool ptimer_begin(int kind, hipStream_t s) {
    if (!vag_opt().persist_timing) return false;
    hipStreamCaptureStatus st = hipStreamCaptureStatusNone;
    if (hipStreamIsCapturing(s, &st) != hipSuccess) { (void)hipGetLastError(); return false; }
    if (st != hipStreamCaptureStatusNone) return false;
    std::lock_guard<std::mutex> lk(g_ptimer_mu);
    PersistTimer& t = g_ptimer[kind];
    ptimer_collect(t);
    if (!t.e0 && (hipEventCreate(&t.e0) != hipSuccess || hipEventCreate(&t.e1) != hipSuccess)) return false;
    return hipEventRecord(t.e0, s) == hipSuccess;
}
static void ptimer_end(int kind, hipStream_t s) {
    std::lock_guard<std::mutex> lk(g_ptimer_mu);
    if (hipEventRecord(g_ptimer[kind].e1, s) == hipSuccess) g_ptimer[kind].pending = true;
}
struct PTimerScope {
    const int kind;
    const hipStream_t s;
    const bool on;
    PTimerScope(int k, hipStream_t st) : kind(k), s(st), on(ptimer_begin(k, st)) {}
    ~PTimerScope() { if (on) ptimer_end(kind, s); }
};
int vag_persistent_time_read(int kind, double* ms_total, int* launches) {
// ... 221 lines not shown
    if (!(H == 512 || H == 1024) || B < 1 || Ts < 1) return false;
    const int64_t wgs = 2 * cdiv64(B, 64) * (H / 32);
    if (wgs > persist_cu_count() || !persist_lds_ok(160 * 1024)) return false;
    return 2 * cdiv64(B, 64) * Ts + 64 <= vag_enc_persistent_sync_words(B, Ts);
}
int vag_enc_fwd_wide16_launch(const float* xp, const vag_half* w16_fw, const vag_half* w16_bw, const float* b_fw, const float* b_bw,
                              const int* lengths, float* hst, float* gates, float* enc, vag_half* hx, unsigned* sync, const uint64_t* rng,
                              float p_ctx, int64_t B, int64_t Ts, int64_t H, hipStream_t s) {
    VAG_CHECK_ARG(xp && w16_fw && w16_bw && b_fw && b_bw && lengths && hst && gates && enc && hx && sync &&
                  vag_enc_wide16_ok(B, Ts, H));
    VAG_CHECK_ARG(aligned16(xp) && aligned16(w16_fw) && aligned16(w16_bw) && aligned16(b_fw) && aligned16(b_bw) && aligned16(hst) &&
                  aligned16(gates) && aligned16(enc) && aligned16(hx));
    EncWArgs a;
    a.xp = xp; a.W16[0] = w16_fw; a.W16[1] = w16_bw; a.bias[0] = b_fw; a.bias[1] = b_bw; a.lengths = lengths;
    a.hst = hst; a.gates = gates; a.enc = enc; a.hx = hx; a.rng = rng; a.p_ctx = p_ctx;
    a.B = (int)B; a.Ts = (int)Ts; a.H = (int)H; a.RG = (int)cdiv64(B, 64); a.CS = (int)(H / 32);
    VAG_TRY(sync_begin(a, sync, vag_enc_persistent_sync_words(B, Ts), s));
    const size_t lds = 96 * 1024;
    if (!max_lds_once<enc_fwd_wide16_kernel<4>>() || !max_lds_once<enc_fwd_wide16_kernel<8>>()) return VAG_EINVAL;
    const dim3 grid((unsigned)(2 * a.RG * a.CS));
    {
        PTimerScope timed(0, s);
        if (H == 512) hipLaunchKernelGGL(enc_fwd_wide16_kernel<4>, grid, dim3(512), lds, s, a);
        else hipLaunchKernelGGL(enc_fwd_wide16_kernel<8>, grid, dim3(512), lds, s, a);
    }
    VAG_LAUNCH_CHECK();
    return VAG_OK;
}

int vag_enc_bwd_wide16_launch(const vag_half* wt16, const float* d_enc, const float* gates, const float* hst, const int* lengths,
                              const uint64_t* rng, float p_ctx, float* d_xp, float* dgh, vag_half* gx, unsigned* sync, int64_t B,
                              int64_t Ts, int64_t H, hipStream_t s) {
    VAG_CHECK_ARG(wt16 && d_enc && gates && hst && lengths && d_xp && dgh && gx && sync && vag_enc_wide16_ok(B, Ts, H));
    VAG_CHECK_ARG(aligned16(wt16) && aligned16(d_enc) && aligned16(gates) && aligned16(hst) && aligned16(d_xp) && aligned16(dgh) &&
                  aligned16(gx));
    EncWBArgs a;
    a.WT16[0] = wt16; a.WT16[1] = wt16 + 3 * H * H; a.d_enc = d_enc; a.gates = gates; a.hst = hst; a.lengths = lengths;
    a.rng = rng; a.p_ctx = p_ctx; a.d_xp = d_xp; a.dgh = dgh; a.gx = gx;
    a.B = (int)B; a.Ts = (int)Ts; a.H = (int)H; a.RG = (int)cdiv64(B, 64); a.CS = (int)(H / 32);
    VAG_TRY(sync_begin(a, sync, vag_enc_persistent_sync_words(B, Ts), s));
    const size_t lds = 84 * 1024;
    if (!max_lds_once<enc_bwd_wide16_kernel<6>>() || !max_lds_once<enc_bwd_wide16_kernel<12>>()) return VAG_EINVAL;
    const dim3 grid((unsigned)(2 * a.RG * a.CS));
    {
        PTimerScope timed(2, s);
        if (H == 512) hipLaunchKernelGGL(enc_bwd_wide16_kernel<6>, grid, dim3(512), lds, s, a);
        else hipLaunchKernelGGL(enc_bwd_wide16_kernel<12>, grid, dim3(512), lds, s, a);
    }
    VAG_LAUNCH_CHECK();
    return VAG_OK;
}

int vag_enc_bwd_persistent_launch(const float* whhT, const float* d_enc, const float* gates, const float* hst, const int* lengths,
                                  const uint64_t* rng, float p_ctx, float* d_xp, float* dgh, unsigned* sync, int64_t B, int64_t Ts,
                                  int64_t H, hipStream_t s) {
    VAG_CHECK_ARG(whhT && d_enc && gates && hst && lengths && d_xp && dgh && sync && (H == 512 || H == 256) && vag_enc_persistent_ok(B, Ts, H));
    VAG_CHECK_ARG(aligned16(whhT) && aligned16(d_enc) && aligned16(gates) && aligned16(hst) && aligned16(d_xp) && aligned16(dgh));
    EncBArgs a;
    a.WT[0] = whhT; a.WT[1] = whhT + 3 * H * H; a.d_enc = d_enc; a.gates = gates; a.hst = hst; a.lengths = lengths;
    a.rng = rng; a.p_ctx = p_ctx; a.d_xp = d_xp; a.dgh = dgh;
    a.B = (int)B; a.Ts = (int)Ts; a.H = (int)H; a.RT = (int)cdiv64(B, 16); a.CS = (int)(H / 16);
    VAG_TRY(sync_begin(a, sync, vag_enc_persistent_sync_words(B, Ts), s));
    {
        PTimerScope timed(2, s);
        row_tile_passes(a.RT, enc_tiles_per_pass(H), [&](int rt0, int tiles) {
            a.rt0 = rt0; a.RTP = tiles;
            const dim3 grid((unsigned)(2 * a.RTP * a.CS));
            if (H == 512) hipLaunchKernelGGL(enc_bwd_persistent_kernel<6>, grid, dim3(512), 0, s, a);
            else hipLaunchKernelGGL(enc_bwd_persistent_kernel<3>, grid, dim3(512), 0, s, a);
        });
    }
    VAG_LAUNCH_CHECK();
    return VAG_OK;
}

unsigned* vag_persist_guard(void) {
    if (vag_ctx().guard) return vag_ctx().guard;
    void* p = nullptr;
    if (hipGetSymbolAddress(&p, HIP_SYMBOL(g_persist_guard)) != hipSuccess) { (void)hipGetLastError(); return nullptr; }
    return reinterpret_cast<unsigned*>(p);
}
int vag_persistent_timeouts_read(void) {
    unsigned v = 0, z = 0;
    const unsigned zz[2] = {0u, 0u};
    if (hipMemcpyFromSymbol(&v, HIP_SYMBOL(g_persist_timeouts), sizeof(v)) != hipSuccess) return -1;
    if (v != 0 && (hipMemcpyToSymbol(HIP_SYMBOL(g_persist_timeouts), &z, sizeof(z)) != hipSuccess ||
                   hipMemcpyToSymbol(HIP_SYMBOL(g_persist_guard), zz, sizeof(zz)) != hipSuccess)) return -1;
    return (int)v;
}

static int64_t dec_bwd_persistent_lds_bytes(int64_t Ts, int64_t H = 512) {
    const int64_t NP = 16 * Ts;
    return 4 * (2048 + NP * 16 + 24 * NP + 2 * NP + 384 + 3 * 128 + 256 + 8 * (2 * H + 4) + 64);
}
bool vag_dec_bwd_persistent_ok(int64_t B, int64_t Ts, int64_t Tt, int64_t H) {
    return vag_dec_persistent_ok(B, Ts, Tt, H) && dec_bwd_persistent_lds_bytes(Ts, H) <= 160 * 1024;
}
int vag_dec_bwd_persistent_launch(const float* pe, const float* encwp, const float* v, const float* wcatT, const float* whh1T,
                                  const float* h0, const float* h2_all, const float* h1, const float* g1, const float* g2,
                                  const float* qhp, const float* alpha, const float* d_h2_all, const float* dah, float* dgi2,
                                  float* dqgh, float* ds, float* dgi1, float* dgh1, float* d_h0, float* dal, unsigned* sync,
                                  int64_t B, int64_t Ts, int64_t Tt, int64_t H, hipStream_t s) {
    VAG_CHECK_ARG(pe && encwp && v && wcatT && whh1T && h0 && h2_all && h1 && g1 && g2 && qhp && alpha && d_h2_all && dah && dgi2 &&
                  dqgh && ds && dgi1 && dgh1 && d_h0 && dal && sync && vag_dec_bwd_persistent_ok(B, Ts, Tt, H));
    VAG_CHECK_ARG(aligned16(pe) && aligned16(encwp) && aligned16(wcatT) && aligned16(whh1T) && aligned16(h0) && aligned16(h2_all) &&
                  aligned16(h1) && aligned16(g1) && aligned16(g2) && aligned16(qhp) && aligned16(d_h2_all) && aligned16(dgi2) &&
                  aligned16(dqgh) && aligned16(dgi1) && aligned16(dgh1) && aligned16(d_h0));
    DecBArgs a;
    a.pe = pe; a.encwp = encwp; a.v = v; a.wcatT = wcatT; a.whh1T = whh1T; a.h0 = h0; a.h2_all = h2_all; a.h1 = h1; a.g1 = g1;
    a.g2 = g2; a.qhp = qhp; a.alpha = alpha; a.d_h2_all = d_h2_all; a.dah = dah; a.dgi2 = dgi2; a.dqgh = dqgh; a.ds = ds;
    a.dgi1 = dgi1; a.dgh1 = dgh1; a.d_h0 = d_h0; a.dal = dal;
    VagCallCtx::Dh0Tanh& dh0 = vag_ctx().dh0_tanh;
    a.h0_tanh = dh0.req ? 1 : 0;
    if (dh0.req) dh0.done = d_h0;
    dh0.req = false;
#ifdef VAG_LAB
    a.dbg = reinterpret_cast<unsigned long long*>(vag_opt().dec_bwd_stamps);
#else
    a.dbg = nullptr;
#endif
    a.B = (int)B; a.Ts = (int)Ts; a.Tt = (int)Tt; a.H = (int)H; a.RT = (int)cdiv64(B, 16);
    a.xcd_map = vag_opt().dec_xcd_map >> 4;
    VAG_TRY(sync_begin(a, sync, vag_dec_persistent_sync_words(B, Tt), s, dal, (int)(Tt * B * Ts) * ACC_SHARDS));
    int64_t lds = dec_bwd_persistent_lds_bytes(Ts, H);
    if (lds < 84 * 1024) lds = 84 * 1024;
    if (!max_lds_once<dec_bwd_persistent_kernel<64>>()) return VAG_EINVAL;
    if (H == 256 && !max_lds_once<dec_bwd_persistent_kernel<32>>()) return VAG_EINVAL;
    {
        PTimerScope timed(3, s);
        row_tile_passes(a.RT, dec_tiles_per_pass(H), [&](int rt0, int tiles) {
            a.rt0 = rt0;
            if (H == 512) hipLaunchKernelGGL(dec_bwd_persistent_kernel<64>, dim3(tiles * 64u), dim3(512), (size_t)lds, s, a);
            else hipLaunchKernelGGL(dec_bwd_persistent_kernel<32>, dim3(tiles * 32u), dim3(512), (size_t)lds, s, a);
        });
    }
    VAG_LAUNCH_CHECK();
    return VAG_OK;
}
```

vag-nmt_amd/vagnmt_hip/_lib.py:

```python
import ctypes as C
import os
import subprocess

import torch

_HERE = os.path.dirname(os.path.abspath(__file__))
PKG_ROOT = os.path.dirname(_HERE)
CSRC = os.path.join(PKG_ROOT, "csrc")
LIB_PATH = os.environ.get("VAG_LIB") or os.path.join(PKG_ROOT, "lib", "libvagnmt.so")

P = C.c_void_p
I64 = C.c_int64
I32 = C.c_int
F = C.c_float


class GruW(C.Structure):
    _fields_ = [("w_ih", P), ("w_hh", P), ("b_ih", P), ("b_hh", P)]


class DecW(C.Structure):
    _fields_ = [("emb", P), ("gru1", GruW), ("attn_h", P), ("attn_v", P), ("c2h", P), ("gru2", GruW)]


# ... 112 lines not shown
    "vag_ens_max_models": (I32, []),
    "vag_beam_ens_step": (I32, [P, P, I64, P, P, I64, I64, P, P, P, I64, I64, I64, P, P, P]),
    "vag_beam_ens_step_dev": (I32, [P, P, I64, P, P, P, I64, P, P, P, P, I64, I64, I64, P, P, P]),
    "vag_ens_argmax": (I32, [P, P, I64, I64, I64, P, P]),
    "vag_beam_step_opt": (I32, [P, I64, P, P, I64, I64, P, P, I64, I64, I64, I64, P, P, I32, P]),
    "vag_beam_step_dev_opt": (I32, [P, I64, P, P, P, I64, P, P, P, I64, I64, I64, I64, P, P, I32, P]),
    "vag_beam_step_logits_dev_opt": (I32, [P, I64, P, I64, P, P, P, I64, P, P, P, I64, I64, I64, I64, P, P, I32, P]),
    "vag_beam_ens_step_opt": (I32, [P, P, I64, P, P, I64, I64, P, P, P, I64, I64, I64, P, P, I32, P]),
    "vag_beam_ens_step_dev_opt": (I32, [P, P, I64, P, P, P, I64, P, P, P, P, I64, I64, I64, P, P, I32, P]),
    "vag_beam_finish_nbest": (I32, [P, P, I64, I64, I64, I64, I64, P, P, P]),
    "vag_beam_finish_nbest_slots": (I32, [P, P, I64, I64, I64, I64, I64, P, P, P, P]),
    "vag_beam_div_scratch_bytes": (I64, [I64, I64, I64, I64]),
    "vag_beam_div_step": (I32, [P, P, I64, P, P, I64, I64, P, P, P, I64, I64, I64, P, P, I32, I64, F, P]),
    "vag_beam_div_step_dev": (I32, [P, P, I64, P, P, P, I64, P, P, P, P, I64, I64, I64, P, P, I32, I64, F, P]),
    "vag_beam_req_scratch_bytes": (I64, [I64, I64, I64, I64]),
    "vag_beam_req_step": (I32, [P, P, I64, P, P, I64, I64, P, P, P, I64, I64, I64, P, P, I32, P, P, P]),
    "vag_beam_req_step_dev": (I32, [P, P, I64, P, P, P, I64, P, P, P, P, I64, I64, I64, P, P, I32, P, P, P]),
    "vag_beam_sbs_scratch_bytes": (I64, [I64, I64, I64, I64]),
    "vag_beam_sbs_step": (I32, [P, P, I64, P, P, I64, I64, P, P, P, I64, I64, I64, P, P, I32, P, P, P]),
    "vag_beam_sbs_step_dev": (I32, [P, P, I64, P, P, P, I64, P, P, P, P, I64, I64, I64, P, P, I32, P, P, P]),
    "vag_beam_pen_scratch_bytes": (I64, [I64, I64, I64, I64]),
    "vag_beam_cover": (I32, [P, I64, P, P, P, I64, I64, I64, I64, I64, F, P, P, P]),
    "vag_beam_cover_dev": (I32, [P, I64, P, P, P, P, I64, I64, I64, I64, F, P, P, P]),
    "vag_beam_pen_step": (I32, [P, P, I64, P, P, I64, I64, P, P, P, I64, I64, I64, P, P, I32, P, P, P, P, P, I64, P, P, I32, P]),
    "vag_beam_pen_step_dev": (I32, [P, P, I64, P, P, P, I64, P, P, P, P, I64, I64, I64, P, P, I32, P, P, P, P, P, I64, P, P, I32,
                                    P]),
    "vag_beam_finish_pen": (I32, [P, P, P, P, P, P, I64, I64, I64, I64, I64, P, P, P, P, P, P, P]),
    "vag_beam_constrain": (I32, [P, P, I64, P, I64, I64, I64, I64, I64, P, I64, P, P, I64, I64, P]),
    "vag_beam_constrain_dev": (I32, [P, P, I64, P, P, I64, I64, I64, I64, P, I64, P, P, I64, I64, P]),
    "vag_forced_score": (I32, [P, P, P, I64, P, I64, I64, I64, P, P, P, P]),
    "vag_beam_attn_record": (I32, [P, I64, P, I64, I64, I64, I64, I64, P]),
    "vag_beam_attn_record_dev": (I32, [P, I64, P, P, I64, I64, I64, I64, P]),
    "vag_beam_finish_align": (I32, [P, P, P, I64, I64, I64, I64, I64, I64, I64, P, P, P, P, P]),
    "vag_forced_align": (I32, [P, I64, P, I64, I64, I64, P, P, P]),
    "vag_sample_step": (I32, [P, P, I64, P, P, I64, I64, P, P, P, P, I64, I64, I64, F, I64, P, P, P]),
    "vag_sample_step_dev": (I32, [P, P, I64, P, P, P, I64, P, I64, I64, I64, F, I64, P, P, P]),
    "vag_sample_step_p": (I32, [P, P, I64, P, P, I64, I64, P, P, P, P, I64, I64, I64, F, I64, P, P, F, P, P]),
    "vag_sample_step_p_dev": (I32, [P, P, I64, P, P, P, I64, P, I64, I64, I64, F, I64, P, P, F, P, P]),
    "vag_sample_noise": (I32, [P, I64, I64, I64, P, P]),
    "vag_mbr_supported": (I32, [I64, I64, I64, I64]),
    "vag_mbr_select": (I32, [P, P, P, I64, I64, I64, I64, I64, I32, P, P, P, P, P]),
    "vag_mrt_weights": (I32, [P, P, P, I64, I64, I64, F, F, P, P, P, P]),
    "vag_mrt_pack": (I32, [P, I64, I64, I64, P, I64, I32, P, I64, P, P]),
    "vag_clip_adam_flat": (I32, [P, P, P, P, I64, I32, C.POINTER(I64), C.POINTER(F), C.POINTER(F), F, F, F, F, F, I32, P,
                                 P, P, P, P]),
    "vag_clip_adam_shard": (I32, [P, P, P, P, I64, I32, C.POINTER(I64), C.POINTER(F), C.POINTER(F), F, F, F, F, F, I32, P,
                                  P, P, P, I64, I64, I32, P, P]),
    "vag_step_ws_floats": (I64, [StepCfgArg]),
    "vag_step_ws_offset": (I64, [StepCfgArg, I32]),
    "vag_train_step": (I32, [StepCfgArg, C.POINTER(ModelW), C.POINTER(ModelW), P, P, P, P, P, P, P, P, P, I32, P]),
    "vag_copy4": (I32, [C.POINTER(P), C.POINTER(P), C.POINTER(I64), I32, P]),
    "vag_set_operator_context": (I32, [P, I32]),
    "vag_set_option": (I32, [C.c_char_p, I64]),
    "vag_recurrence_supported": (I32, [I32, I64, I64, I64, I64]),
    "vag_persistent_timeouts": (I32, []),
    "vag_set_operator_guard": (I32, [P]),
    "vag_recurrence_time": (I32, [I32, P, P]),
    "vag_gemm_group_plan": (I32, [I32, P, P, P, P, P, P]),
    "vag_comm_unique_id": (I32, [P]),
    "vag_comm_init": (I32, [P, I32, I32, P]),
    "vag_comm_allreduce": (I32, [P, P, I64, P]),
    "vag_comm_size": (I32, [P]),
    "vag_comm_destroy": (I32, [P]),
    "vag_recurrence_sync_words": (I64, [I32, I64, I64]),
    "vag_cgru_recurrence_fwd": (I32, [P, P, P, P, DecW, P, P, P, I64, I64, I64, I64, P, P, P, P, P, P, P, P, P]),
    "vag_derived_floats": (I64, [I64]),
    "vag_derive_weights": (I32, [DecW, P, P, I64, I32, P, P]),
    "vag_cgru_ws_offset": (I64, [I64, I64, I64, I64, I64, I32]),
    "vag_dropout_mask": (I32, [P, I32, I64, F, P, P]),
    "vag_rng_advance": (I32, [P, P]),
}

_lib = None


def use_lab_build():
    global LIB_PATH
    assert _lib is None, "use_lab_build() must come before the library is loaded"
    r = subprocess.run(["make", "-C", CSRC, "-j8", "LAB=1"], capture_output=True, text=True)
    if r.returncode != 0:
        raise RuntimeError("building libvagnmt_lab.so failed:\n" + r.stderr[-2000:])
    LIB_PATH = os.path.join(os.path.dirname(LIB_PATH), "libvagnmt_lab.so")
    return LIB_PATH


def build(verbose=False):
    r = subprocess.run(["make", "-C", CSRC, "-j8"], capture_output=True, text=True)
    if verbose or r.returncode != 0:
        print(r.stdout[-4000:])
        print(r.stderr[-4000:])
    if r.returncode != 0:
        raise RuntimeError("building libvagnmt.so failed")
    return LIB_PATH


def lib():
    global _lib
    if _lib is None:
        if not os.path.exists(LIB_PATH):
            raise RuntimeError(
                "libvagnmt.so not found at %s: build it with `make -C %s` (or __graft_entry__.build()). "
                "There is no CPU fallback for the VAG-NMT hot path." % (LIB_PATH, CSRC))
        L = C.CDLL(LIB_PATH)
        for name, (res, args) in PROTOS.items():
            fn = getattr(L, name)
            fn.restype = res
# ... 93 lines not shown
```

vag-nmt_amd/vagnmt_hip/fused.py:

```python
import ctypes as C

import torch
import torch.nn as nn

from . import _lib as L
from ._lib import DecW, GruW, HeadW, ModelW, StepCfgMrt, call, gru_w, ptr, stream
from .state import dropout_rng


def mt_label_smoothing(criterion_mt):
    from machine_translation_vision.losses import LabelSmoothedNLLLoss
    if type(criterion_mt) is nn.NLLLoss:
        ok = criterion_mt.reduction == 'none' and criterion_mt.weight is not None and criterion_mt.ignore_index < 0
        return 0.0 if ok else None
    if type(criterion_mt) is LabelSmoothedNLLLoss:
        return float(criterion_mt.label_smoothing)
    return None


def fusable(model, criterion_mt, criterion_vse):
    from machine_translation_vision.losses import ImageRetrievalRankingLoss, PairwiseRankingLoss
    ok_mt = mt_label_smoothing(criterion_mt) is not None
    ok_vse = criterion_vse is None or type(criterion_vse) in (PairwiseRankingLoss, ImageRetrievalRankingLoss)
    return ok_mt and ok_vse and hasattr(model, "encoder") and hasattr(model, "decoder")
# ... 12 lines not shown
    s = ModelW()
    s.enc_emb = t(enc.embedding.weight)
    s.enc_fw = gw(g.weight_ih_l0, g.weight_hh_l0, g.bias_ih_l0, g.bias_hh_l0)
    s.enc_bw = gw(g.weight_ih_l0_reverse, g.weight_hh_l0_reverse, g.bias_ih_l0_reverse, g.bias_hh_l0_reverse)
    if mm:
        v = model.vse_imagine
        s.im_w, s.im_b = t(v.im_embedding.weight), t(v.im_embedding.bias)
        s.txt_w, s.txt_b = t(v.text_embedding.weight), t(v.text_embedding.bias)
        s.ctx2ctx, s.emb2ctx = t(v.imagine_attn.ctx2ctx.weight), t(v.imagine_attn.emb2ctx.weight)
        s.mlp_w = t(v.imagine_attn.mlp.weight) if v.imagine_attn.method == "mlp" else None
    s.ini_w, s.ini_b = t(model.decoderini.weight), t(model.decoderini.bias)
    s.attn_e = t(dec.attn.attn_e.weight)
    dp = dec.dec_params()
    s.dec = DecW(t(dec.embedding.weight), gw(dp[0], dp[1], dp[2], dp[3]), t(dp[4]), t(dp[5]), t(dp[6]),
                 gw(dp[7], dp[8], dp[9], dp[10]))
    s.head = HeadW(*[t(p) for p in dec.head_params()])
    return s


class FusedStep:
    LOSS_RING = 256
    def __init__(self, model, criterion_mt, criterion_vse, storage="f32"):
        if storage not in ("f32", "f16"):
            raise ValueError("storage must be 'f32' or 'f16'")
        self.storage16 = storage == "f16"
        self.model = model
        self.mm = hasattr(model, "vse_imagine")
        self.vw = criterion_mt.weight
        self.label_smoothing = mt_label_smoothing(criterion_mt)
        if self.label_smoothing is None:
            raise ValueError("FusedStep: criterion_mt is not one the fused step implements (see fusable())")
        self.dev = self.vw.device
        dec, enc = model.decoder, model.encoder
        self.H = dec.hidden_size
        self.V = dec.out.bias.shape[0]
        self.ldl = (self.V + 3) // 4 * 4
        self.Es = enc.embedding.weight.shape[1]
        self.Et = dec.embedding.weight.shape[1]
        if self.storage16 and self.H % 8 != 0:
            raise ValueError("fp16 storage needs hidden_size % 8 == 0")
        self.S = model.vse_imagine.shared_embedding_size if self.mm else 0
        self.I = model.vse_imagine.im_size if self.mm else 0
        self.rank_kind, self.margin = -1, 0.0
        if self.mm and criterion_vse is not None:
            from machine_translation_vision.losses import PairwiseRankingLoss
            self.rank_kind = 0 if type(criterion_vse) is PairwiseRankingLoss else 1
            self.margin = float(criterion_vse.margin)
        self.w = model_struct(model, grad=False)
        self.g = model_struct(model, grad=True)
        self.derived = torch.empty(L.lib().vag_derived_floats(self.H), dtype=torch.float32, device=self.dev)
        self.losses = torch.zeros(4 + 4 * self.LOSS_RING, dtype=torch.float32, device=self.dev)
        self.executed = 0
        self.ws = None
        self.cap = (0, 0, 0)
        self.src = self.tgt = self.im = self.lens = None
        self.mrt_cost = self.mrt_valid = None
        self.generation = 0
        self.guard = None
        self.refresh_derived()

    def cfg(self, B, Ts, Tt, teacher, train=True, mrt=None):
        m = self.model
        c = StepCfgMrt()
        c.B, c.Ts, c.Tt, c.Es, c.Et, c.H, c.S, c.I, c.V, c.ldl = B, Ts, Tt, self.Es, self.Et, self.H, self.S, self.I, self.V, self.ldl
        c.multimodal = 1 if self.mm else 0
        c.attn_method = 1 if (self.mm and m.vse_imagine.imagine_attn.method == "mlp") else 0
        c.activation_vse = 1 if (self.mm and m.vse_imagine.activation_vse) else 0
        c.rank_kind = self.rank_kind
        c.free_run = 0 if teacher else 1
        c.storage = 1 if (self.storage16 and teacher) else 0
        c.margin = self.margin
        c.loss_w = float(m.loss_w) if self.mm else 1.0
        c.init_split = float(m.init_split) if self.mm else 0.0
        c.p_emb = float(m.encoder.dropout_emb) if train else 0.0
        c.p_ctx = float(m.encoder.dropout_ctx) if train else 0.0
        c.p_out = float(m.decoder.dropout_out) if train else 0.0
        c.loss_ring = self.LOSS_RING
        c.guard = self.guard
        c.label_smoothing = self.label_smoothing
        if mrt is not None:
            c.mrt_n, c.mrt_alpha, c.mrt_scale = int(mrt[0]), float(mrt[1]), float(mrt[2])
            c.mrt_cost, c.mrt_valid = ptr(self.mrt_cost), ptr(self.mrt_valid)
            c.rank_kind, c.loss_w = -1, 1.0
        return c

    def reserve(self, B, Ts, Tt):
        c = self.cfg(B, Ts, Tt, True)
        need = L.lib().vag_step_ws_floats(c.ref())
        if need < 0:
            raise L.VagError("vag_step_ws_floats: bad configuration")
        grown = False
        if self.ws is None or self.ws.numel() < need:
            self.ws = torch.empty(int(need * 1.25), dtype=torch.float32, device=self.dev)
            grown = True
        cap = (max(self.cap[0], B * Ts), max(self.cap[1], B * Tt), max(self.cap[2], B))
        if cap != self.cap:
            self.cap = cap
            self.src = torch.zeros(cap[0], dtype=torch.int64, device=self.dev)
            self.tgt = torch.zeros(cap[1], dtype=torch.int64, device=self.dev)
            self.lens = torch.zeros(cap[2], dtype=torch.int32, device=self.dev)
            self.im = torch.zeros(cap[2] * max(self.I, 1), dtype=torch.float32, device=self.dev)
            self.mrt_cost = torch.zeros(cap[2], dtype=torch.float32, device=self.dev)
            self.mrt_valid = torch.zeros(cap[2], dtype=torch.float32, device=self.dev)
            grown = True
        if grown:
            self.generation += 1
        return grown

    def load_batch(self, src, lengths, tgt, im):
        B, Ts = src.shape
        Tt = tgt.shape[1]
        srcs = [src, tgt, lengths] + ([im] if self.mm else [])
        dsts = [self.src, self.tgt, self.lens] + ([self.im] if self.mm else [])
        for t in srcs:
            if not (t.is_cuda and t.is_contiguous()):
                raise L.VagError("batch tensors must be contiguous HIP tensors")
        if src.dtype != torch.int64 or tgt.dtype != torch.int64 or lengths.dtype != torch.int32 or \
                (self.mm and im.dtype != torch.float32):
            raise L.VagError("batch dtypes: src/tgt int64, lengths int32, im float32")
        n = len(srcs)
        sp = (C.c_void_p * 4)(*[t.data_ptr() for t in srcs])
        dp = (C.c_void_p * 4)(*[t.data_ptr() for t in dsts])
        nb = (C.c_int64 * 4)(*[t.numel() * t.element_size() for t in srcs])
        assert srcs[0].numel() == B * Ts and srcs[1].numel() == B * Tt and srcs[2].numel() == B
        call("vag_copy4", sp, dp, nb, n, stream())

    def load_mrt(self, cost, valid):
        B = cost.numel()
        if valid.numel() != B or B > self.mrt_cost.numel():
            raise L.VagError("load_mrt: cost and valid must both hold one float per row of the loaded batch")
        self.mrt_cost[:B].copy_(cost.reshape(-1))
        self.mrt_valid[:B].copy_(valid.reshape(-1))

    def refresh_derived(self):
        g = self.model.encoder.gru
        call("vag_derive_weights", self.w.dec, ptr(g.weight_hh_l0), ptr(g.weight_hh_l0_reverse), self.H,
             1 if self.storage16 else 0, ptr(self.derived), stream())

    def run(self, B, Ts, Tt, teacher, phases, mrt=None):
        m = self.model
        train = m.training
        c = self.cfg(B, Ts, Tt, teacher, train, mrt)
        rng = None
        if train and max(c.p_emb, c.p_ctx, c.p_out) > 0:
            rng = dropout_rng(m, self.dev)
        if (int(phases) & 1) and not (self.dev.type == "cuda" and torch.cuda.is_current_stream_capturing()):
            self.executed += 1
        call("vag_train_step", c.ref(), C.byref(self.w), C.byref(self.g), ptr(self.src, torch.int64),
             ptr(self.lens, torch.int32), ptr(self.tgt, torch.int64), ptr(self.im) if self.mm else None, ptr(self.vw),
             ptr(rng, torch.int64) if rng is not None else None, ptr(self.derived), ptr(self.ws), ptr(self.losses),
             int(phases), stream())
```

vag-nmt_amd/vagnmt_hip/ops.py:

```python
import ctypes as C

import torch
from torch.autograd import Function

from . import _lib as L
from ._lib import DecW, GruW, HeadW, call, gru_w, ptr, stream

I64 = torch.int64


_OPERATOR_GUARD = None


def set_operator_guard(address):
    global _OPERATOR_GUARD
    _OPERATOR_GUARD = address


def _recurrence_call(name, *args):
    g = _OPERATOR_GUARD
    if g is None:
        return call(name, *args)
    call("vag_set_operator_guard", g)
    try:
        return call(name, *args)
    finally:
        call("vag_set_operator_guard", None)


def _f32(*shape, like):
    return torch.empty(*shape, dtype=torch.float32, device=like.device)


def _zeros(*shape, like):
    return torch.zeros(*shape, dtype=torch.float32, device=like.device)


def _grad_views(params):
    return [getattr(p, "_vag_grad", None) for p in params]


def _grad_targets(views, params):
    return [(v, False) if v is not None else (torch.zeros_like(p), True) for v, p in zip(views, params)]


def _ret(targets):
    return tuple(t if give else None for t, give in targets)


def _c(t):
    return t if t.is_contiguous() else t.contiguous()


class BiGRUEncode(Function):

    @staticmethod
    def forward(ctx, src, lengths, emb, wf_ih, wf_hh, bf_ih, bf_hh, wb_ih, wb_hh, bb_ih, bb_hh, p_emb, p_ctx, rng):
        B, Ts = src.shape
        E, H = emb.shape[1], wf_hh.shape[1]
        enc = _f32(B, Ts, 2 * H, like=emb)
        mask = _f32(B, Ts, like=emb)
        ws = _f32(L.lib().vag_bigru_ws_floats(B, Ts, E, H), like=emb)
        src = _c(src)
        _recurrence_call("vag_bigru_seq_fwd", ptr(src, I64), ptr(lengths, torch.int32), ptr(emb),
             gru_w(wf_ih, wf_hh, bf_ih, bf_hh), gru_w(wb_ih, wb_hh, bb_ih, bb_hh), p_emb, p_ctx,
             ptr(rng, torch.int64) if rng is not None else None, B, Ts, E, H, ptr(enc), ptr(mask), ptr(ws), stream())
        params = (emb, wf_ih, wf_hh, bf_ih, bf_hh, wb_ih, wb_hh, bb_ih, bb_hh)
        ctx.save_for_backward(src, lengths, ws, *params)
        ctx.gviews = _grad_views(params)
        ctx.cfg = (B, Ts, E, H, p_emb, p_ctx, rng)
        ctx.mark_non_differentiable(mask)
        return enc, mask

    @staticmethod
    def backward(ctx, d_enc, _d_mask):
        src, lengths, ws, emb, wf_ih, wf_hh, bf_ih, bf_hh, wb_ih, wb_hh, bb_ih, bb_hh = ctx.saved_tensors
        B, Ts, E, H, p_emb, p_ctx, rng = ctx.cfg
        d_enc = _c(d_enc)
        t = _grad_targets(ctx.gviews, ctx.saved_tensors[3:])
        g = [x[0] for x in t]
        _recurrence_call("vag_bigru_seq_bwd", ptr(src, I64), ptr(lengths, torch.int32), gru_w(wf_ih, wf_hh, bf_ih, bf_hh),
             gru_w(wb_ih, wb_hh, bb_ih, bb_hh), p_emb, p_ctx, ptr(rng, torch.int64) if rng is not None else None,
             B, Ts, E, H, ptr(d_enc), ptr(ws), ptr(g[0]), gru_w(g[1], g[2], g[3], g[4]), gru_w(g[5], g[6], g[7], g[8]),
             stream())
        return (None, None) + _ret(t) + (None, None, None)


class LinearAct(Function):

    @staticmethod
    def forward(ctx, x, W, b, act):
        x2 = _c(x).view(-1, x.shape[-1])
        M, K = x2.shape
        N = W.shape[0]
        y = _f32(M, N, like=x)
        call("vag_linear_fwd", M, N, K, ptr(x2), ptr(W), ptr(b) if b is not None else None, int(act), ptr(y), stream())
        ctx.save_for_backward(x2, W, y)
        ctx.gviews = _grad_views((W,) + ((b,) if b is not None else ()))
        ctx.bshape = b.shape if b is not None else None
        ctx.act = int(act)
        ctx.has_b = b is not None
        ctx.xshape = x.shape
        return y.view(*x.shape[:-1], N)

    @staticmethod
    def backward(ctx, dy):
        x2, W, y = ctx.saved_tensors
        M, K = x2.shape
        N = W.shape[0]
        dy = _c(dy).view(M, N).clone()
        dx = _f32(M, K, like=x2) if ctx.needs_input_grad[0] else None
        t = [(ctx.gviews[0], False) if ctx.gviews[0] is not None else (torch.zeros_like(W), True)]
        if ctx.has_b:
            t.append((ctx.gviews[1], False) if ctx.gviews[1] is not None else (_zeros(*ctx.bshape, like=W), True))
        call("vag_linear_bwd", M, N, K, ptr(x2), ptr(W), ptr(y), ptr(dy), ctx.act, ptr(dx) if dx is not None else None,
             0, ptr(t[0][0]), ptr(t[1][0]) if ctx.has_b else None, stream())
        r = _ret(t)
        return (dx.view(ctx.xshape) if dx is not None else None, r[0], r[1] if ctx.has_b else None, None)


class Embedding(Function):

    @staticmethod
    def forward(ctx, idx, W):
        flat = _c(idx).view(-1)
        out = _f32(flat.numel(), W.shape[1], like=W)
        call("vag_embed_fwd", ptr(flat, I64), flat.numel(), ptr(W), W.shape[1], ptr(out), stream())
        ctx.save_for_backward(flat, W)
        ctx.gviews = _grad_views((W,))
        ctx.E = W.shape[1]
        return out.view(*idx.shape, W.shape[1])

    @staticmethod
    def backward(ctx, d_out):
# ... 41 lines not shown
        dec, head = rest[:ndec], rest[ndec:]
        B, Ts, Cc = enc.shape
        H = Cc // 2
        E = emb.shape[1]
        Tt = tok.shape[0] - 1
        hseq = _f32(Tt + 1, B, H, like=enc)
        hseq[0].copy_(h0)
        h0, h2 = hseq[0], hseq[1:]
        c = _f32(Tt, B, Cc, like=enc)
        e = _f32(Tt, B, E, like=enc)
        ws = _f32(L.lib().vag_cgru_ws_floats(B, Ts, Tt, E, H), like=enc)
        tmid = logits = None
        hw = None
        if free_run:
            tmid = _f32(Tt, B, E, like=enc)
            logits = _f32(Tt * B, ldl, like=enc)
            hw = C.byref(_head_w(head))
        if free_run and L.lib().vag_cgru_free_supported(B, Ts, Tt, E, H, V):
            tables = _f32(L.lib().vag_cgru_free_tables_floats(B, Ts, Tt, E, H, V), like=enc)
            _recurrence_call("vag_cgru_attn_decode_free_fwd", ptr(enc), ptr(pe), ptr(mask), ptr(h0), ptr(tok, I64), _dec_w(emb, dec),
                 B, Ts, Tt, E, H, V, ptr(h2), ptr(c), ptr(e), ptr(ws), hw, float(p_out),
                 ptr(rng, torch.int64) if rng is not None else None, ptr(tmid), ptr(logits), ldl, ptr(tables), stream())
        else:
            _recurrence_call("vag_cgru_attn_decode_seq_fwd", ptr(enc), ptr(pe), ptr(mask), ptr(h0), ptr(tok, I64), _dec_w(emb, dec),
                 B, Ts, Tt, E, H, V, ptr(h2), ptr(c), ptr(e), ptr(ws), int(bool(free_run)), hw, float(p_out),
                 ptr(rng, torch.int64) if rng is not None else None, ptr(tmid), ptr(logits), ldl, stream())
        ctx.save_for_backward(enc, pe, mask, h0, tok, ws, h2, c, e, emb, *dec)
        ctx.gviews = _grad_views((emb,) + tuple(dec))
        ctx.cfg = (B, Ts, Tt, E, H, V)
        ctx.nrest = len(rest)
        ctx.ndec = ndec
        if free_run:
            ctx.mark_non_differentiable(tmid, logits)
            return h2, c, e, tmid, logits
        return h2, c, e

    @staticmethod
    def backward(ctx, d_h2, d_c, d_e, *_unused):
        enc, pe, mask, h0, tok, ws, h2, c, e, emb = ctx.saved_tensors[:10]
        dec = ctx.saved_tensors[10:]
        B, Ts, Tt, E, H, V = ctx.cfg
        Cc = 2 * H
        d_h2 = _c(d_h2).clone() if d_h2 is not None else _zeros(Tt, B, H, like=enc)
        d_c = _c(d_c).clone() if d_c is not None else _zeros(Tt, B, Cc, like=enc)
        d_e = _c(d_e) if d_e is not None else None
        d_enc = _f32(B, Ts, Cc, like=enc)
        d_pe = _f32(B, Ts, Cc, like=enc)
        d_h0 = _f32(B, H, like=enc)
        scratch = _f32(L.lib().vag_cgru_bwd_scratch_floats(B, Ts, Tt, E, H), like=enc)
        t = _grad_targets(ctx.gviews, (emb,) + tuple(dec))
        g = [x[0] for x in t]
        gdec = DecW(ptr(g[0]), gru_w(g[1], g[2], g[3], g[4]), ptr(g[5]), ptr(g[6]), ptr(g[7]),
                    gru_w(g[8], g[9], g[10], g[11]))
        _recurrence_call("vag_cgru_attn_decode_seq_bwd", ptr(enc), ptr(pe), ptr(mask), ptr(h0), ptr(tok, I64), _dec_w(emb, dec),
             B, Ts, Tt, E, H, V, ptr(h2), ptr(c), ptr(e), ptr(d_h2), ptr(d_c), ptr(d_e), ptr(ws), ptr(d_enc), 0,
             ptr(d_pe), ptr(d_h0), gdec, ptr(scratch), stream())
        r = _ret(t)
        return (d_enc, d_pe, None, d_h0, None, r[0], None, None, None, None, None, None) + tuple(r[1:]) + \
            (None,) * (ctx.nrest - ctx.ndec)


def cgru_decode_seq(enc, pe, mask, h0, tok, emb, dec, free_run=False, head=None, p_out=0.0, rng=None, V=0, ldl=0):
    return _CGRUDecodeSeq.apply(enc, pe, mask, h0, tok, emb, bool(free_run), p_out, rng, V, ldl, len(dec), *dec,
                                *(head or ()))


class HeadCE(Function):

    @staticmethod
    def forward(ctx, h2, c, e, tgt, vw, p_out, rng, tmid, logits, ldl, *head):
        return _head_ce_forward(ctx, None, h2, c, e, tgt, vw, p_out, rng, tmid, logits, ldl, head)

    @staticmethod
    def backward(ctx, d_loss):
        return _head_ce_backward(ctx, d_loss, 10)


class HeadCESmoothed(Function):

    @staticmethod
    def forward(ctx, h2, c, e, tgt, vw, p_out, rng, tmid, logits, ldl, eps, *head):
        return _head_ce_forward(ctx, float(eps), h2, c, e, tgt, vw, p_out, rng, tmid, logits, ldl, head)

    @staticmethod
    def backward(ctx, d_loss):
        return _head_ce_backward(ctx, d_loss, 11)


def _head_ce_forward(ctx, eps, h2, c, e, tgt, vw, p_out, rng, tmid, logits, ldl, head):
    Tt, B, H = h2.shape
    E = e.shape[2]
    V = head[7].shape[0]
    R = Tt * B
    ready = logits is not None
    if not ready:
        tmid = _f32(Tt, B, E, like=h2)
        logits = _f32(R, ldl, like=h2)
    lse = _f32(R, like=h2)
    nll = _f32(R, like=h2)
    inv_cnt = _f32(B, like=h2)
    loss = _f32(1, like=h2)
    tgt = _c(tgt)
    args = (ptr(h2), ptr(c), ptr(e), _head_w(head), ptr(tgt, I64), ptr(vw), B, Tt, E, H, V, p_out,
            ptr(rng, torch.int64) if rng is not None else None, int(ready), ptr(tmid), ptr(logits), ldl, ptr(lse),
            ptr(nll), ptr(inv_cnt), ptr(loss))
    if eps is None:
        call("vag_head_ce_seq_fwd", *args, stream())
# ... 340 lines not shown
```

Before: 21330 sentence-pairs/s.

## Hand off backward recurrence gradients via pre-split bf16 planes buffer

Adds a side buffer of pre-split bf16x3 'planes' so that the persistent encoder and decoder backward kernels store each step's dgh/dq hand-off already split and laid out in MFMA fragment order. Consumers then load the fragments directly instead of reloading f32 rows, permuting and splitting them on the critical serial path. This costs extra stores, a second plain f32 write of dgh, another buffer allocation and new kernel template variants. The option is enabled by default and the fused step sets the buffer around each call.

New measurement: 22180 sentence-pairs/s (median of 6 runs). +4.0%, better.

```diff
diff --git a/include/vag_nmt.h b/include/vag_nmt.h
--- a/include/vag_nmt.h
+++ b/include/vag_nmt.h
@@ -404,6 +404,8 @@
                    const float* derived, float* ws, float* losses, int phases, vag_stream_t stream);
 int vag_set_operator_context(const float* derived, int storage);
 int vag_set_option(const char* name, int64_t value);
+int64_t vag_handoff_planes_floats(int64_t B, int64_t Ts, int64_t Tt, int64_t H);
+int vag_set_handoff_planes(float* buf, int64_t floats);
 int vag_copy4(const void* const* src, void* const* dst, const int64_t* bytes, int n, vag_stream_t stream);
 int64_t vag_derived_floats(int64_t H);
 int vag_derive_weights(vag_dec_w w, const float* enc_whh_fw, const float* enc_whh_bw, int64_t H, int with_fp16,
diff --git a/vag-nmt_amd/csrc/api.hip b/vag-nmt_amd/csrc/api.hip
--- a/vag-nmt_amd/csrc/api.hip
+++ b/vag-nmt_amd/csrc/api.hip
@@ -80,7 +80,7 @@
         {"gemm_force_splitk", &o.gemm_force_splitk}, {"head_fuse", &o.head_fuse},
         {"head_bf16_grads", &o.head_bf16_grads}, {"persistent", &o.persistent}, {"persistent_dec_bwd", &o.persistent_dec_bwd}, {"persistent_enc_bwd", &o.persistent_enc_bwd}, {"free_persistent", &o.free_persistent}, {"attn_dot_reg", &o.attn_dot_reg},
         {"persist_timing", &o.persist_timing}, {"s16_one_plane", &o.s16_one_plane}, {"leaf_queue", &o.leaf_queue}, {"attn_row", &o.attn_row}, {"dec_xcd_map", &o.dec_xcd_map}, {"loss_ride", &o.loss_ride}, {"step_fork", &o.step_fork},
-        {"head_bf16_dlogits", &o.head_bf16_dlogits}};
+        {"head_bf16_dlogits", &o.head_bf16_dlogits}, {"handoff_planes", &o.handoff_planes}};
     for (const auto& e : ints)
         if (strcmp(name, e.n) == 0) { *e.p = (int)value; return VAG_OK; }
     if (strcmp(name, "head_chunk") == 0) { o.head_chunk = value; return VAG_OK; }
@@ -152,6 +152,11 @@
     w.enc16 = c.take_as<vag_half>(2 * 3 * H * H); w.encT16 = c.take_as<vag_half>(2 * 3 * H * H);
     w.total = c.off;
     return w;
+}
+
+static float* handoff_planes(int64_t need) {
+    const VagCallCtx& c = vag_ctx();
+    return (need > 0 && c.handoff_planes && c.handoff_floats >= need) ? c.handoff_planes : nullptr;
 }
 
 struct BiGruWs {
@@ -258,7 +263,8 @@
         VAG_TRY(vag_enc_bwd_wide16_launch(reinterpret_cast<const vag_half*>(whhT), d_enc, w.gates, w.hst, lengths, rng, p_ctx, d_xp,
                                           w.dgh, reinterpret_cast<vag_half*>(w.gx), w.sync_b, B, Ts, H, s));
     } else if (persist) {
-        VAG_TRY(vag_enc_bwd_persistent_launch(whhT, d_enc, w.gates, w.hst, lengths, rng, p_ctx, d_xp, w.dgh, w.sync_b, B, Ts, H, s));
+        VAG_TRY(vag_enc_bwd_persistent_launch(whhT, d_enc, w.gates, w.hst, lengths, rng, p_ctx, d_xp, w.dgh,
+                                              handoff_planes(vag_enc_bwd_planes_floats(B, Ts, H)), w.sync_b, B, Ts, H, s));
     }
     GruBwdArgs a = {};
     a.ld_add = Ts * 2 * H; a.ldh = H; a.ldgi = 6 * H; a.ldgh = 3 * H;
@@ -772,8 +778,8 @@
         VAG_TRY(vag_attn_scores_ex_launch(1, enc, d_c_all, C, nullptr, nullptr, Tt * B, 1, B, Ts, C, nullptr, z.dah, s));
     if (persist) {
         VAG_TRY(vag_dec_bwd_persistent_launch(pe, k.encwp, w.attn_v, z.wcatT, z.whh1T, h0, h2_all, k.h1, k.g1, k.g2, k.qhp, k.alpha,
-                                              d_h2_all, z.dah, z.dgi2, z.dqgh, z.ds, z.dgi1, z.dgh1, d_h0, k.dal, k.sync_b, B, Ts, Tt, H,
-                                              s));
+                                              d_h2_all, z.dah, z.dgi2, z.dqgh, z.ds, z.dgi1, z.dgh1, d_h0, k.dal,
+                                              handoff_planes(vag_dec_bwd_planes_floats(B, Tt, H)), k.sync_b, B, Ts, Tt, H, s));
     }
     for (int64_t t = Tt - 1; t >= 0 && !persist; --t) {
         float* dgi2 = z.dgi2 + t * B * 3 * H;
@@ -1738,6 +1744,16 @@
     return 0;
 }
 int vag_persistent_timeouts(void) { return vag_persistent_timeouts_read(); }
+int64_t vag_handoff_planes_floats(int64_t B, int64_t Ts, int64_t Tt, int64_t H) {
+    const int64_t e = vag_enc_bwd_planes_floats(B, Ts, H), d = vag_dec_bwd_planes_floats(B, Tt, H);
+    return e > d ? e : d;
+}
+int vag_set_handoff_planes(float* buf, int64_t floats) {
+    VAG_CHECK_ARG((buf == nullptr || (floats > 0 && aligned16(buf))));
+    g_base_ctx.handoff_planes = buf;
+    g_base_ctx.handoff_floats = buf ? floats : 0;
+    return VAG_OK;
+}
 int vag_set_operator_guard(void* guard) {
     VAG_CHECK_ARG((reinterpret_cast<uintptr_t>(guard) & 3) == 0);
     g_base_ctx.guard = reinterpret_cast<unsigned*>(guard);
diff --git a/vag-nmt_amd/csrc/call_ctx.h b/vag-nmt_amd/csrc/call_ctx.h
--- a/vag-nmt_amd/csrc/call_ctx.h
+++ b/vag-nmt_amd/csrc/call_ctx.h
@@ -20,6 +20,8 @@
     bool store16 = false;
     int gemm_planes = 3;
     unsigned* guard = nullptr;
+    float* handoff_planes = nullptr;
+    int64_t handoff_floats = 0;
 
     int64_t head_chunk = 0;
     struct HeadFuse { const vag_head_g* g = nullptr; const float* d_loss = nullptr; float* dt = nullptr; bool done = false; } head_fuse;
diff --git a/vag-nmt_amd/csrc/common.h b/vag-nmt_amd/csrc/common.h
--- a/vag-nmt_amd/csrc/common.h
+++ b/vag-nmt_amd/csrc/common.h
@@ -102,6 +102,7 @@
     int persistent_dec_bwd = 1;
     int persistent_enc_bwd = 1;
     int attn_dot_reg = 1;
+    int handoff_planes = 1;
     int free_persistent = 1;
     int s16_one_plane = 1;
     int head_bf16_dlogits = 1;
diff --git a/vag-nmt_amd/csrc/kernels.h b/vag-nmt_amd/csrc/kernels.h
--- a/vag-nmt_amd/csrc/kernels.h
+++ b/vag-nmt_amd/csrc/kernels.h
@@ -150,8 +150,10 @@
                                   const int* lengths, float* hst, float* gates, float* enc, unsigned* sync, const uint64_t* rng,
                                   float p_ctx, int64_t B, int64_t Ts, int64_t H, hipStream_t s);
 int vag_enc_bwd_persistent_launch(const float* whhT, const float* d_enc, const float* gates, const float* hst, const int* lengths,
-                                  const uint64_t* rng, float p_ctx, float* d_xp, float* dgh, unsigned* sync, int64_t B, int64_t Ts,
-                                  int64_t H, hipStream_t s);
+                                  const uint64_t* rng, float p_ctx, float* d_xp, float* dgh, float* planes, unsigned* sync, int64_t B,
+                                  int64_t Ts, int64_t H, hipStream_t s);
+int64_t vag_enc_bwd_planes_floats(int64_t B, int64_t Ts, int64_t H);
+int64_t vag_dec_bwd_planes_floats(int64_t B, int64_t Tt, int64_t H);
 bool vag_enc_wide16_ok(int64_t B, int64_t Ts, int64_t H);
 int vag_enc_fwd_wide16_launch(const float* xp, const vag_half* w16_fw, const vag_half* w16_bw, const float* b_fw, const float* b_bw,
                               const int* lengths, float* hst, float* gates, float* enc, vag_half* hx, unsigned* sync, const uint64_t* rng,
@@ -168,8 +170,8 @@
 int vag_dec_bwd_persistent_launch(const float* pe, const float* encwp, const float* v, const float* wcatT, const float* whh1T,
                                   const float* h0, const float* h2_all, const float* h1, const float* g1, const float* g2,
                                   const float* qhp, const float* alpha, const float* d_h2_all, const float* dah, float* dgi2,
-                                  float* dqgh, float* ds, float* dgi1, float* dgh1, float* d_h0, float* dal, unsigned* sync,
-                                  int64_t B, int64_t Ts, int64_t Tt, int64_t H, hipStream_t s);
+                                  float* dqgh, float* ds, float* dgi1, float* dgh1, float* d_h0, float* dal, float* planes,
+                                  unsigned* sync, int64_t B, int64_t Ts, int64_t Tt, int64_t H, hipStream_t s);
 float* vag_cgru_bwd_scratch_de(float* scratch, int64_t B, int64_t Ts, int64_t Tt, int64_t E, int64_t H);
 float* vag_cgru_bwd_scratch_du(float* scratch, int64_t B, int64_t Ts, int64_t Tt, int64_t E, int64_t H);
 int vag_attn_dot_row_launch(bool bwd, const float* x, const float* q, int64_t ldq, const float* mask, const float* alpha, int64_t B,
diff --git a/vag-nmt_amd/csrc/persist.hip b/vag-nmt_amd/csrc/persist.hip
--- a/vag-nmt_amd/csrc/persist.hip
+++ b/vag-nmt_amd/csrc/persist.hip
@@ -141,6 +141,68 @@
     acc = __builtin_amdgcn_mfma_f32_16x16x32_bf16(a[0], b[1], acc, 0, 0, 0);
     acc = __builtin_amdgcn_mfma_f32_16x16x32_bf16(a[1], b[0], acc, 0, 0, 0);
     acc = __builtin_amdgcn_mfma_f32_16x16x32_bf16(a[0], b[0], acc, 0, 0, 0);
+    return acc;
+}
+
+constexpr int PL_PLANE_BYTES = 64 * 16, PL_KSTEP_BYTES = 3 * PL_PLANE_BYTES;
+__host__ __device__ constexpr int64_t pl_block_bytes(int64_t K) { return (K / 32) * PL_KSTEP_BYTES; }
+typedef unsigned u32x2 __attribute__((ext_vector_type(2)));
+__device__ __forceinline__ unsigned pl_slot_off(int r, int k0) { return (unsigned)((r + 16 * ((k0 & 31) >> 3)) * 16 + 8 * ((k0 >> 2) & 1)); }
+__device__ __forceinline__ void st_planes4(const char* kblk, unsigned voff, float4 v) {
+    unsigned q[3][2];
+    split3(v.x, v.y, q[0][0], q[1][0], q[2][0]);
+    split3(v.z, v.w, q[0][1], q[1][1], q[2][1]);
+    const u32x2 x0 = {q[0][0], q[0][1]}, x1 = {q[1][0], q[1][1]}, x2 = {q[2][0], q[2][1]};
+    asm volatile("global_store_dwordx2 %0, %1, %4 sc1\n\tglobal_store_dwordx2 %0, %2, %4 offset:1024 sc1\n\t"
+                 "global_store_dwordx2 %0, %3, %4 offset:2048 sc1\n\ts_nop 1"
+                 :: "v"(voff), "v"(x0), "v"(x1), "v"(x2), "s"(kblk) : "memory");
+}
+#define VAG_PLD(o, v, a, off) "global_load_dwordx4 %" #o ", %" #v ", %" #a " offset:" #off " sc1\n\t"
+template <int N> __device__ __forceinline__ void ld_planes_sc1(const char* p, unsigned voff, u32x4 (&f)[3 * N]);
+template <> __device__ __forceinline__ void ld_planes_sc1<2>(const char* p, unsigned voff, u32x4 (&f)[6]) {
+    const char* p1 = p + 8192;
+    asm volatile(VAG_PLD(0, 6, 7, 0) VAG_PLD(1, 6, 7, 1024) VAG_PLD(2, 6, 7, 2048) VAG_PLD(3, 6, 7, 3072) VAG_PLD(4, 6, 8, -4096) VAG_PLD(5, 6, 8, -3072)
+                 "s_waitcnt vmcnt(0)"
+                 : "=&v"(f[0]), "=&v"(f[1]), "=&v"(f[2]), "=&v"(f[3]), "=&v"(f[4]), "=&v"(f[5]) : "v"(voff), "s"(p), "s"(p1) : "memory");
+}
+template <> __device__ __forceinline__ void ld_planes_sc1<3>(const char* p, unsigned voff, u32x4 (&f)[9]) {
+    const char* p1 = p + 8192;
+    asm volatile(VAG_PLD(0, 9, 10, 0) VAG_PLD(1, 9, 10, 1024) VAG_PLD(2, 9, 10, 2048) VAG_PLD(3, 9, 10, 3072) VAG_PLD(4, 9, 11, -4096)
+                 VAG_PLD(5, 9, 11, -3072) VAG_PLD(6, 9, 11, -2048) VAG_PLD(7, 9, 11, -1024) VAG_PLD(8, 9, 11, 0)
+                 "s_waitcnt vmcnt(0)"
+                 : "=&v"(f[0]), "=&v"(f[1]), "=&v"(f[2]), "=&v"(f[3]), "=&v"(f[4]), "=&v"(f[5]), "=&v"(f[6]), "=&v"(f[7]), "=&v"(f[8])
+                 : "v"(voff), "s"(p), "s"(p1) : "memory");
+}
+template <> __device__ __forceinline__ void ld_planes_sc1<4>(const char* p, unsigned voff, u32x4 (&f)[12]) {
+    const char* p1 = p + 8192;
+    asm volatile(VAG_PLD(0, 12, 13, 0) VAG_PLD(1, 12, 13, 1024) VAG_PLD(2, 12, 13, 2048) VAG_PLD(3, 12, 13, 3072) VAG_PLD(4, 12, 14, -4096)
+                 VAG_PLD(5, 12, 14, -3072) VAG_PLD(6, 12, 14, -2048) VAG_PLD(7, 12, 14, -1024) VAG_PLD(8, 12, 14, 0) VAG_PLD(9, 12, 14, 1024)
+                 VAG_PLD(10, 12, 14, 2048) VAG_PLD(11, 12, 14, 3072)
+                 "s_waitcnt vmcnt(0)"
+                 : "=&v"(f[0]), "=&v"(f[1]), "=&v"(f[2]), "=&v"(f[3]), "=&v"(f[4]), "=&v"(f[5]), "=&v"(f[6]), "=&v"(f[7]), "=&v"(f[8]),
+                   "=&v"(f[9]), "=&v"(f[10]), "=&v"(f[11])
+                 : "v"(voff), "s"(p), "s"(p1) : "memory");
+}
+template <> __device__ __forceinline__ void ld_planes_sc1<6>(const char* p, unsigned voff, u32x4 (&f)[18]) {
+    const char *p1 = p + 8192, *p2 = p + 16384;
+    asm volatile(VAG_PLD(0, 18, 19, 0) VAG_PLD(1, 18, 19, 1024) VAG_PLD(2, 18, 19, 2048) VAG_PLD(3, 18, 19, 3072) VAG_PLD(4, 18, 20, -4096)
+                 VAG_PLD(5, 18, 20, -3072) VAG_PLD(6, 18, 20, -2048) VAG_PLD(7, 18, 20, -1024) VAG_PLD(8, 18, 20, 0) VAG_PLD(9, 18, 20, 1024)
+                 VAG_PLD(10, 18, 20, 2048) VAG_PLD(11, 18, 20, 3072) VAG_PLD(12, 18, 21, -4096) VAG_PLD(13, 18, 21, -3072)
+                 VAG_PLD(14, 18, 21, -2048) VAG_PLD(15, 18, 21, -1024) VAG_PLD(16, 18, 21, 0) VAG_PLD(17, 18, 21, 1024)
+                 "s_waitcnt vmcnt(0)"
+                 : "=&v"(f[0]), "=&v"(f[1]), "=&v"(f[2]), "=&v"(f[3]), "=&v"(f[4]), "=&v"(f[5]), "=&v"(f[6]), "=&v"(f[7]), "=&v"(f[8]),
+                   "=&v"(f[9]), "=&v"(f[10]), "=&v"(f[11]), "=&v"(f[12]), "=&v"(f[13]), "=&v"(f[14]), "=&v"(f[15]), "=&v"(f[16]), "=&v"(f[17])
+                 : "v"(voff), "s"(p), "s"(p1), "s"(p2) : "memory");
+}
+#undef VAG_PLD
+template <int N>
+__device__ __forceinline__ f32x4 mma6_planes(const bf16x8 (&w)[N][3], const u32x4 (&f)[3 * N], f32x4 acc) {
+#pragma unroll
+    for (int s = 0; s < N; ++s) {
+        const bf16x8 hf[3] = {__builtin_bit_cast(bf16x8, f[3 * s]), __builtin_bit_cast(bf16x8, f[3 * s + 1]),
+                              __builtin_bit_cast(bf16x8, f[3 * s + 2])};
+        acc = mma6(w[s], hf, acc);
+    }
     return acc;
 }
 
@@ -468,8 +530,9 @@
     unsigned spin;
     int B, Ts, H, RT, CS;
     int rt0, RTP;
+    char* pl;
 };
-template <int KS>
+template <int KS, bool PL>
 __global__ __launch_bounds__(512, 1) void enc_bwd_persistent_kernel(EncBArgs a) {
     __shared__ __attribute__((aligned(16))) float lds[21504];
     const int wg = blockIdx.x;
@@ -492,6 +555,11 @@
     const int len = eok ? a.lengths[em] : 0;
     float4 carry = make_float4(0.f, 0.f, 0.f, 0.f);
     float* dghd = a.dgh + (int64_t)d * Ts * B * K;
+    const char* pld = PL ? a.pl + ((int64_t)d * Ts * a.RT + rt) * pl_block_bytes(K) : nullptr;
+    const int64_t pl_step = (int64_t)a.RT * pl_block_bytes(K);
+    const int pl_ld = __builtin_amdgcn_readfirstlane(wave) * KS * PL_KSTEP_BYTES;
+    const int pl_st = (u0 >> 5) * PL_KSTEP_BYTES, pl_gate = (H >> 5) * PL_KSTEP_BYTES;
+    const unsigned pl_so = pl_slot_off(lane >> 2, u0 + 4 * (lane & 3));
     gu32* cnt = (gu32*)(a.cnt + ((int64_t)d * a.RT + rt) * Ts);
     const int lrow = min(m0 + ld_row(lane), B - 1);
     const int src4 = ld_src4(lane);
@@ -520,13 +588,19 @@
             }
             __syncthreads();
             f32x4 acc = {0.f, 0.f, 0.f, 0.f};
-            float4 ga[KS], gb[KS];
-            ld_rows_sc1<KS>(dghd + ((int64_t)(k + 1) * B + lrow) * K + kbase + 8 * (lane & 3), ga, gb);
-#pragma unroll
-            for (int s = 0; s < KS; ++s) {
-                bf16x8 hf[3];
-                split8(perm4(ga[s], src4), perm4(gb[s], src4), hf);
-                acc = mma6(wf[s], hf, acc);
+            if (PL) {
+                u32x4 gf[3 * KS];
+                ld_planes_sc1<KS>(pld + (k + 1) * pl_step + pl_ld, 16u * lane, gf);
+                acc = mma6_planes<KS>(wf, gf, acc);
+            } else {
+                float4 ga[KS], gb[KS];
+                ld_rows_sc1<KS>(dghd + ((int64_t)(k + 1) * B + lrow) * K + kbase + 8 * (lane & 3), ga, gb);
+#pragma unroll
+                for (int s = 0; s < KS; ++s) {
+                    bf16x8 hf[3];
+                    split8(perm4(ga[s], src4), perm4(gb[s], src4), hf);
+                    acc = mma6(wf[s], hf, acc);
+                }
             }
             red[wave * 64 + lane] = make_float4(acc[0], acc[1], acc[2], acc[3]);
             __syncthreads();
@@ -537,6 +611,10 @@
                     dh.x += o.x; dh.y += o.y; dh.z += o.z; dh.w += o.w;
                 }
             }
+        }
+        if (PL && wave == 0 && !eok) {
+#pragma unroll
+            for (int g = 0; g < 3; ++g) st_planes4(pld + k * pl_step + pl_st + g * pl_gate, pl_so, make_float4(0.f, 0.f, 0.f, 0.f));
         }
         if (eok) {
             const bool active = t < len;
@@ -567,9 +645,17 @@
             carry = make_float4(cy[0], cy[1], cy[2], cy[3]);
             float* gho = dghd + ((int64_t)k * B + em) * K + eu;
 #pragma unroll
-            for (int g = 0; g < 3; ++g) st_sc1_f4(gho + g * H, make_float4(gh[g][0], gh[g][1], gh[g][2], gh[g][3]));
+            for (int g = 0; g < 3; ++g) {
+                const float4 x = make_float4(gh[g][0], gh[g][1], gh[g][2], gh[g][3]);
+                if (PL) st_planes4(pld + k * pl_step + pl_st + g * pl_gate, pl_so, x);
+                else st_sc1_f4(gho + g * H, x);
+            }
             asm volatile("s_waitcnt vmcnt(0)" ::: "memory");
             if (lane == 0) __hip_atomic_fetch_add(cnt + k, 1u, RLX_AGENT);
+            if (PL) {
+#pragma unroll
+                for (int g = 0; g < 3; ++g) *reinterpret_cast<float4*>(gho + g * H) = make_float4(gh[g][0], gh[g][1], gh[g][2], gh[g][3]);
+            }
             float* gio = a.d_xp + ((int64_t)t * B + em) * 6 * H + d * 3 * H + eu;
 #pragma unroll
             for (int g = 0; g < 3; ++g) *reinterpret_cast<float4*>(gio + g * H) = make_float4(gi[g][0], gi[g][1], gi[g][2], gi[g][3]);
@@ -1404,6 +1490,7 @@
     int rt0;
     int xcd_map;
     int h0_tanh;
+    char *pl_dq, *pl_dgh1;
 };
 
 __device__ __forceinline__ void cell_bwd4(const float (&dh)[4], const float4 (&sv)[4], const float4 hp, float (&gi)[3][4],
@@ -1422,7 +1509,7 @@
     }
 }
 
-template <int WGS>
+template <int WGS, bool PL>
 __global__ __launch_bounds__(512, 1) void dec_bwd_persistent_kernel(DecBArgs a) {
     extern __shared__ __attribute__((aligned(16))) float dlds[];
     constexpr int H = WGS * DEC_U, C = 2 * H, Q = C + 3 * H;
@@ -1489,6 +1576,13 @@
     gu32* cC = (gu32*)(a.cnt + ((int64_t)2 * a.RT + rt) * Tt * CNT_WORDS);
     bool dead = false;
     const float vq = a.v[16 * i + (threadIdx.x & 15)];
+    const char* pl_dq = PL ? a.pl_dq + (int64_t)rt * pl_block_bytes(C) : nullptr;
+    const char* pl_g1 = PL ? a.pl_dgh1 + (int64_t)rt * pl_block_bytes(3 * H) : nullptr;
+    const int64_t pl_dq_step = (int64_t)a.RT * pl_block_bytes(C), pl_g1_step = (int64_t)a.RT * pl_block_bytes(3 * H);
+    const int pl_wave = __builtin_amdgcn_readfirstlane(wave) * PL_KSTEP_BYTES;
+    constexpr int pl_gate = (H >> 5) * PL_KSTEP_BYTES;
+    const int pl_st_g1 = (u0 >> 5) * PL_KSTEP_BYTES, pl_st_dq = ((16 * i) >> 5) * PL_KSTEP_BYTES;
+    const unsigned pl_so_g1 = pl_slot_off(fr, eu), pl_so_dq = pl_slot_off((threadIdx.x >> 2) & 15, 16 * i + 4 * (threadIdx.x & 3));
 
     auto cell2_bwd = [&](int t, const float (&dh2)[4], const float4 (&sv)[4], const float4 hp) {
         float gi[3][4], gh[3][4], dr[4];
@@ -1537,6 +1631,8 @@
 #define VAG_STAMP(k) do { } while (0)
 #endif
     for (int t = Tt - 1; t >= 0; --t) {
+        int emL = em;
+        if (PL) asm volatile("" : "+v"(emL));
         VAG_STAMP(0);
         for (int P = threadIdx.x; P < NP; P += 512) {
             const int r = P / Ts;
@@ -1604,9 +1700,13 @@
             __syncthreads();
             if (threadIdx.x < 64) {
                 const int r = threadIdx.x >> 2, c4 = threadIdx.x & 3;
-                if (m0 + r < B) st_sc1_f4(a.dqgh + ((int64_t)t * B + m0 + r) * Q + 16 * i + 4 * c4, *reinterpret_cast<const float4*>(dq_s + r * 16 + 4 * c4));
+                const float4 dqv = *reinterpret_cast<const float4*>(dq_s + r * 16 + 4 * c4);
+                float* dqo = a.dqgh + ((int64_t)t * B + m0 + r) * Q + 16 * i + 4 * c4;
+                if (PL) st_planes4(pl_dq + t * pl_dq_step + pl_st_dq, pl_so_dq, m0 + r < B ? dqv : make_float4(0.f, 0.f, 0.f, 0.f));
+                else if (m0 + r < B) st_sc1_f4(dqo, dqv);
                 asm volatile("s_waitcnt vmcnt(0)" ::: "memory");
                 if (threadIdx.x == 0) arrive(cB + t * CNT_WORDS, i);
+                if (PL && m0 + r < B) *reinterpret_cast<float4*>(dqo) = dqv;
             }
         }
         VAG_STAMP(3);
@@ -1631,7 +1731,7 @@
         }
         float4 s1[4], hp1 = make_float4(0.f, 0.f, 0.f, 0.f);
         if (eok) {
-            const int64_t o = (int64_t)em * H + eu;
+            const int64_t o = (int64_t)emL * H + eu;
 #pragma unroll
             for (int q = 0; q < 4; ++q) s1[q] = *reinterpret_cast<const float4*>(a.g1 + ((int64_t)t * 4 + q) * BH + o);
             hp1 = *reinterpret_cast<const float4*>((t > 0 ? a.h2_all + (int64_t)(t - 1) * BH : a.h0) + o);
@@ -1641,16 +1741,29 @@
         VAG_STAMP(5);
         {
             f32x4 acc = {0.f, 0.f, 0.f, 0.f};
-            float4 ga[KB], gb[KB];
-            ld_rows_sc1<KB>(a.dqgh + ((int64_t)t * B + lrow) * Q + wave * (C >> 3) + 8 * (lane & 3), ga, gb);
-#pragma unroll
-            for (int s = 0; s < KB; ++s) { ga[s] = perm4(ga[s], src4); gb[s] = perm4(gb[s], src4); }
-#pragma unroll
-            for (int s = 0; s < KB; ++s) {
-                bf16x8 wf[3], hf[3];
-                split8(*reinterpret_cast<const float4*>(wb_row + 32 * s), *reinterpret_cast<const float4*>(wb_row + 32 * s + 4), wf);
-                split8(ga[s], gb[s], hf);
-                acc = mma6(wf, hf, acc);
+            if (PL) {
+                u32x4 gf[3 * KB];
+                ld_planes_sc1<KB>(pl_dq + t * pl_dq_step + KB * pl_wave, 16u * lane, gf);
+#pragma unroll
+                for (int s = 0; s < KB; ++s) {
+                    bf16x8 wf[3];
+                    split8(*reinterpret_cast<const float4*>(wb_row + 32 * s), *reinterpret_cast<const float4*>(wb_row + 32 * s + 4), wf);
+                    const bf16x8 hf[3] = {__builtin_bit_cast(bf16x8, gf[3 * s]), __builtin_bit_cast(bf16x8, gf[3 * s + 1]),
+                                          __builtin_bit_cast(bf16x8, gf[3 * s + 2])};
+                    acc = mma6(wf, hf, acc);
+                }
+            } else {
+                float4 ga[KB], gb[KB];
+                ld_rows_sc1<KB>(a.dqgh + ((int64_t)t * B + lrow) * Q + wave * (C >> 3) + 8 * (lane & 3), ga, gb);
+#pragma unroll
+                for (int s = 0; s < KB; ++s) { ga[s] = perm4(ga[s], src4); gb[s] = perm4(gb[s], src4); }
+#pragma unroll
+                for (int s = 0; s < KB; ++s) {
+                    bf16x8 wf[3], hf[3];
+                    split8(*reinterpret_cast<const float4*>(wb_row + 32 * s), *reinterpret_cast<const float4*>(wb_row + 32 * s + 4), wf);
+                    split8(ga[s], gb[s], hf);
+                    acc = mma6(wf, hf, acc);
+                }
             }
             red[wave * 64 + lane] = make_float4(acc[0], acc[1], acc[2], acc[3]);
         }
@@ -1658,19 +1771,29 @@
         if (ep) {
             float x[4];
             red4(x);
+            if (PL && !eok) {
+#pragma unroll
+                for (int g = 0; g < 3; ++g) st_planes4(pl_g1 + t * pl_g1_step + pl_st_g1 + g * pl_gate, pl_so_g1, make_float4(0.f, 0.f, 0.f, 0.f));
+            }
             if (eok) {
                 const float4 pbv = *reinterpret_cast<const float4*>(pb_s + fr * 8 + 4 * hq);
                 const float dh1[4] = {x[0] + pbv.x, x[1] + pbv.y, x[2] + pbv.z, x[3] + pbv.w};
                 float gi[3][4], gh[3][4], dr[4];
                 cell_bwd4(dh1, s1, hp1, gi, gh, dr);
 #pragma unroll
-                for (int g = 0; g < 3; ++g)
-                    st_sc1_f4(a.dgh1 + ((int64_t)t * B + em) * 3 * H + g * H + eu, make_float4(gh[g][0], gh[g][1], gh[g][2], gh[g][3]));
+                for (int g = 0; g < 3; ++g) {
+                    const float4 x = make_float4(gh[g][0], gh[g][1], gh[g][2], gh[g][3]);
+                    if (PL) st_planes4(pl_g1 + t * pl_g1_step + pl_st_g1 + g * pl_gate, pl_so_g1, x);
+                    else st_sc1_f4(a.dgh1 + ((int64_t)t * B + emL) * 3 * H + g * H + eu, x);
+                }
                 asm volatile("s_waitcnt vmcnt(0)" ::: "memory");
                 if (threadIdx.x == 0) arrive(cC + t * CNT_WORDS, i);
 #pragma unroll
-                for (int g = 0; g < 3; ++g)
-                    *reinterpret_cast<float4*>(a.dgi1 + ((int64_t)t * B + em) * 3 * H + g * H + eu) = make_float4(gi[g][0], gi[g][1], gi[g][2], gi[g][3]);
+                for (int g = 0; g < 3; ++g) {
+                    if (PL)
+                        *reinterpret_cast<float4*>(a.dgh1 + ((int64_t)t * B + emL) * 3 * H + g * H + eu) = make_float4(gh[g][0], gh[g][1], gh[g][2], gh[g][3]);
+                    *reinterpret_cast<float4*>(a.dgi1 + ((int64_t)t * B + emL) * 3 * H + g * H + eu) = make_float4(gi[g][0], gi[g][1], gi[g][2], gi[g][3]);
+                }
                 *reinterpret_cast<float4*>(c1_s + fr * 8 + 4 * hq) = make_float4(dr[0], dr[1], dr[2], dr[3]);
             } else if (threadIdx.x == 0) {
                 arrive(cC + t * CNT_WORDS, i);
@@ -1678,7 +1801,7 @@
         }
         float4 dadd = make_float4(0.f, 0.f, 0.f, 0.f), s2[4], hp2 = make_float4(0.f, 0.f, 0.f, 0.f);
         if (eok && t > 0) {
-            const int64_t o = (int64_t)em * H + eu;
+            const int64_t o = (int64_t)emL * H + eu;
             dadd = *reinterpret_cast<const float4*>(a.d_h2_all + (int64_t)(t - 1) * BH + o);
 #pragma unroll
             for (int q = 0; q < 4; ++q) s2[q] = *reinterpret_cast<const float4*>(a.g2 + ((int64_t)(t - 1) * 4 + q) * BH + o);
@@ -1689,15 +1812,21 @@
         VAG_STAMP(7);
         {
             f32x4 acc = {0.f, 0.f, 0.f, 0.f};
-            float4 ga[KC], gb[KC];
-            ld_rows_sc1<KC>(a.dgh1 + ((int64_t)t * B + lrow) * 3 * H + wave * (3 * H >> 3) + 8 * (lane & 3), ga, gb);
-#pragma unroll
-            for (int s = 0; s < KC; ++s) { ga[s] = perm4(ga[s], src4); gb[s] = perm4(gb[s], src4); }
-#pragma unroll
-            for (int s = 0; s < KC; ++s) {
-                bf16x8 hf[3];
-                split8(ga[s], gb[s], hf);
-                acc = mma6(wc[s], hf, acc);
+            if (PL) {
+                u32x4 gf[3 * KC];
+                ld_planes_sc1<KC>(pl_g1 + t * pl_g1_step + KC * pl_wave, 16u * lane, gf);
+                acc = mma6_planes<KC>(wc, gf, acc);
+            } else {
+                float4 ga[KC], gb[KC];
+                ld_rows_sc1<KC>(a.dgh1 + ((int64_t)t * B + lrow) * 3 * H + wave * (3 * H >> 3) + 8 * (lane & 3), ga, gb);
+#pragma unroll
+                for (int s = 0; s < KC; ++s) { ga[s] = perm4(ga[s], src4); gb[s] = perm4(gb[s], src4); }
+#pragma unroll
+                for (int s = 0; s < KC; ++s) {
+                    bf16x8 hf[3];
+                    split8(ga[s], gb[s], hf);
+                    acc = mma6(wc[s], hf, acc);
+                }
             }
             red[wave * 64 + lane] = make_float4(acc[0], acc[1], acc[2], acc[3]);
         }
@@ -1712,10 +1841,10 @@
                 else {
                     float4 o = make_float4(dh2[0], dh2[1], dh2[2], dh2[3]);
                     if (a.h0_tanh) {
-                        const float4 h = *reinterpret_cast<const float4*>(a.h0 + (int64_t)em * H + eu);
+                        const float4 h = *reinterpret_cast<const float4*>(a.h0 + (int64_t)emL * H + eu);
                         o.x *= 1.f - h.x * h.x; o.y *= 1.f - h.y * h.y; o.z *= 1.f - h.z * h.z; o.w *= 1.f - h.w * h.w;
                     }
-                    *reinterpret_cast<float4*>(a.d_h0 + (int64_t)em * H + eu) = o;
+                    *reinterpret_cast<float4*>(a.d_h0 + (int64_t)emL * H + eu) = o;
                 }
             }
         }
@@ -2043,13 +2172,14 @@
 }
 
 int vag_enc_bwd_persistent_launch(const float* whhT, const float* d_enc, const float* gates, const float* hst, const int* lengths,
-                                  const uint64_t* rng, float p_ctx, float* d_xp, float* dgh, unsigned* sync, int64_t B, int64_t Ts,
-                                  int64_t H, hipStream_t s) {
+                                  const uint64_t* rng, float p_ctx, float* d_xp, float* dgh, float* planes, unsigned* sync, int64_t B,
+                                  int64_t Ts, int64_t H, hipStream_t s) {
     VAG_CHECK_ARG(whhT && d_enc && gates && hst && lengths && d_xp && dgh && sync && (H == 512 || H == 256) && vag_enc_persistent_ok(B, Ts, H));
-    VAG_CHECK_ARG(aligned16(whhT) && aligned16(d_enc) && aligned16(gates) && aligned16(hst) && aligned16(d_xp) && aligned16(dgh));
+    VAG_CHECK_ARG(aligned16(whhT) && aligned16(d_enc) && aligned16(gates) && aligned16(hst) && aligned16(d_xp) && aligned16(dgh) && aligned16(planes));
+    const bool pl = planes && vag_opt().handoff_planes && vag_enc_bwd_planes_floats(B, Ts, H) > 0;
     EncBArgs a;
     a.WT[0] = whhT; a.WT[1] = whhT + 3 * H * H; a.d_enc = d_enc; a.gates = gates; a.hst = hst; a.lengths = lengths;
-    a.rng = rng; a.p_ctx = p_ctx; a.d_xp = d_xp; a.dgh = dgh;
+    a.rng = rng; a.p_ctx = p_ctx; a.d_xp = d_xp; a.dgh = dgh; a.pl = reinterpret_cast<char*>(planes);
     a.B = (int)B; a.Ts = (int)Ts; a.H = (int)H; a.RT = (int)cdiv64(B, 16); a.CS = (int)(H / 16);
     VAG_TRY(sync_begin(a, sync, vag_enc_persistent_sync_words(B, Ts), s));
     {
@@ -2057,8 +2187,10 @@
         row_tile_passes(a.RT, enc_tiles_per_pass(H), [&](int rt0, int tiles) {
             a.rt0 = rt0; a.RTP = tiles;
             const dim3 grid((unsigned)(2 * a.RTP * a.CS));
-            if (H == 512) hipLaunchKernelGGL(enc_bwd_persistent_kernel<6>, grid, dim3(512), 0, s, a);
-            else hipLaunchKernelGGL(enc_bwd_persistent_kernel<3>, grid, dim3(512), 0, s, a);
+            if (H == 512 && pl) hipLaunchKernelGGL((enc_bwd_persistent_kernel<6, true>), grid, dim3(512), 0, s, a);
+            else if (H == 512) hipLaunchKernelGGL((enc_bwd_persistent_kernel<6, false>), grid, dim3(512), 0, s, a);
+            else if (pl) hipLaunchKernelGGL((enc_bwd_persistent_kernel<3, true>), grid, dim3(512), 0, s, a);
+            else hipLaunchKernelGGL((enc_bwd_persistent_kernel<3, false>), grid, dim3(512), 0, s, a);
         });
     }
     VAG_LAUNCH_CHECK();
@@ -2084,19 +2216,34 @@
     const int64_t NP = 16 * Ts;
     return 4 * (2048 + NP * 16 + 24 * NP + 2 * NP + 384 + 3 * 128 + 256 + 8 * (2 * H + 4) + 64);
 }
+static bool pl_any_device_takes(int64_t rt, int tpp_max) {
+    for (int tpp = 1; tpp <= tpp_max; ++tpp)
+        if (passes_ok(rt, tpp, DEC_MAX_PASSES)) return true;
+    return false;
+}
+constexpr int PL_MAX_CUS = 256;
+int64_t vag_enc_bwd_planes_floats(int64_t B, int64_t Ts, int64_t H) {
+    if ((H != 512 && H != 256) || B <= 0 || Ts <= 0 || !pl_any_device_takes(cdiv64(B, 16), (int)(PL_MAX_CUS / (2 * (H / 16))))) return 0;
+    return 2 * Ts * cdiv64(B, 16) * pl_block_bytes(3 * H) / 4;
+}
+int64_t vag_dec_bwd_planes_floats(int64_t B, int64_t Tt, int64_t H) {
+    if ((H != 512 && H != 256) || B <= 0 || Tt <= 0 || !pl_any_device_takes(cdiv64(B, 16), PL_MAX_CUS / dec_wgs(H))) return 0;
+    return Tt * cdiv64(B, 16) * (pl_block_bytes(2 * H) + pl_block_bytes(3 * H)) / 4;
+}
 bool vag_dec_bwd_persistent_ok(int64_t B, int64_t Ts, int64_t Tt, int64_t H) {
     return vag_dec_persistent_ok(B, Ts, Tt, H) && dec_bwd_persistent_lds_bytes(Ts, H) <= 160 * 1024;
 }
 int vag_dec_bwd_persistent_launch(const float* pe, const float* encwp, const float* v, const float* wcatT, const float* whh1T,
                                   const float* h0, const float* h2_all, const float* h1, const float* g1, const float* g2,
                                   const float* qhp, const float* alpha, const float* d_h2_all, const float* dah, float* dgi2,
-                                  float* dqgh, float* ds, float* dgi1, float* dgh1, float* d_h0, float* dal, unsigned* sync,
-                                  int64_t B, int64_t Ts, int64_t Tt, int64_t H, hipStream_t s) {
+                                  float* dqgh, float* ds, float* dgi1, float* dgh1, float* d_h0, float* dal, float* planes,
+                                  unsigned* sync, int64_t B, int64_t Ts, int64_t Tt, int64_t H, hipStream_t s) {
     VAG_CHECK_ARG(pe && encwp && v && wcatT && whh1T && h0 && h2_all && h1 && g1 && g2 && qhp && alpha && d_h2_all && dah && dgi2 &&
                   dqgh && ds && dgi1 && dgh1 && d_h0 && dal && sync && vag_dec_bwd_persistent_ok(B, Ts, Tt, H));
     VAG_CHECK_ARG(aligned16(pe) && aligned16(encwp) && aligned16(wcatT) && aligned16(whh1T) && aligned16(h0) && aligned16(h2_all) &&
                   aligned16(h1) && aligned16(g1) && aligned16(g2) && aligned16(qhp) && aligned16(d_h2_all) && aligned16(dgi2) &&
-                  aligned16(dqgh) && aligned16(dgi1) && aligned16(dgh1) && aligned16(d_h0));
+                  aligned16(dqgh) && aligned16(dgi1) && aligned16(dgh1) && aligned16(d_h0) && aligned16(planes));
+    const bool pl = planes && vag_opt().handoff_planes && vag_dec_bwd_planes_floats(B, Tt, H) > 0;
     DecBArgs a;
     a.pe = pe; a.encwp = encwp; a.v = v; a.wcatT = wcatT; a.whh1T = whh1T; a.h0 = h0; a.h2_all = h2_all; a.h1 = h1; a.g1 = g1;
     a.g2 = g2; a.qhp = qhp; a.alpha = alpha; a.d_h2_all = d_h2_all; a.dah = dah; a.dgi2 = dgi2; a.dqgh = dqgh; a.ds = ds;
@@ -2111,18 +2258,22 @@
     a.dbg = nullptr;
 #endif
     a.B = (int)B; a.Ts = (int)Ts; a.Tt = (int)Tt; a.H = (int)H; a.RT = (int)cdiv64(B, 16);
+    a.pl_dq = reinterpret_cast<char*>(planes);
+    a.pl_dgh1 = a.pl_dq ? a.pl_dq + Tt * a.RT * pl_block_bytes(2 * H) : nullptr;
     a.xcd_map = vag_opt().dec_xcd_map >> 4;
     VAG_TRY(sync_begin(a, sync, vag_dec_persistent_sync_words(B, Tt), s, dal, (int)(Tt * B * Ts) * ACC_SHARDS));
     int64_t lds = dec_bwd_persistent_lds_bytes(Ts, H);
     if (lds < 84 * 1024) lds = 84 * 1024;
-    if (!max_lds_once<dec_bwd_persistent_kernel<64>>()) return VAG_EINVAL;
-    if (H == 256 && !max_lds_once<dec_bwd_persistent_kernel<32>>()) return VAG_EINVAL;
+    if (H == 512 && !(pl ? max_lds_once<dec_bwd_persistent_kernel<64, true>>() : max_lds_once<dec_bwd_persistent_kernel<64, false>>())) return VAG_EINVAL;
+    if (H == 256 && !(pl ? max_lds_once<dec_bwd_persistent_kernel<32, true>>() : max_lds_once<dec_bwd_persistent_kernel<32, false>>())) return VAG_EINVAL;
     {
         PTimerScope timed(3, s);
         row_tile_passes(a.RT, dec_tiles_per_pass(H), [&](int rt0, int tiles) {
             a.rt0 = rt0;
-            if (H == 512) hipLaunchKernelGGL(dec_bwd_persistent_kernel<64>, dim3(tiles * 64u), dim3(512), (size_t)lds, s, a);
-            else hipLaunchKernelGGL(dec_bwd_persistent_kernel<32>, dim3(tiles * 32u), dim3(512), (size_t)lds, s, a);
+            if (H == 512 && pl) hipLaunchKernelGGL((dec_bwd_persistent_kernel<64, true>), dim3(tiles * 64u), dim3(512), (size_t)lds, s, a);
+            else if (H == 512) hipLaunchKernelGGL((dec_bwd_persistent_kernel<64, false>), dim3(tiles * 64u), dim3(512), (size_t)lds, s, a);
+            else if (pl) hipLaunchKernelGGL((dec_bwd_persistent_kernel<32, true>), dim3(tiles * 32u), dim3(512), (size_t)lds, s, a);
+            else hipLaunchKernelGGL((dec_bwd_persistent_kernel<32, false>), dim3(tiles * 32u), dim3(512), (size_t)lds, s, a);
         });
     }
     VAG_LAUNCH_CHECK();
diff --git a/vag-nmt_amd/vagnmt_hip/_lib.py b/vag-nmt_amd/vagnmt_hip/_lib.py
--- a/vag-nmt_amd/vagnmt_hip/_lib.py
+++ b/vag-nmt_amd/vagnmt_hip/_lib.py
@@ -188,6 +188,8 @@
     "vag_copy4": (I32, [C.POINTER(P), C.POINTER(P), C.POINTER(I64), I32, P]),
     "vag_set_operator_context": (I32, [P, I32]),
     "vag_set_option": (I32, [C.c_char_p, I64]),
+    "vag_handoff_planes_floats": (I64, [I64, I64, I64, I64]),
+    "vag_set_handoff_planes": (I32, [P, I64]),
     "vag_recurrence_supported": (I32, [I32, I64, I64, I64, I64]),
     "vag_persistent_timeouts": (I32, []),
     "vag_set_operator_guard": (I32, [P]),
diff --git a/vag-nmt_amd/vagnmt_hip/fused.py b/vag-nmt_amd/vagnmt_hip/fused.py
--- a/vag-nmt_amd/vagnmt_hip/fused.py
+++ b/vag-nmt_amd/vagnmt_hip/fused.py
@@ -88,6 +88,7 @@
         self.losses = torch.zeros(4 + 4 * self.LOSS_RING, dtype=torch.float32, device=self.dev)
         self.executed = 0
         self.ws = None
+        self.planes = None
         self.cap = (0, 0, 0)
         self.src = self.tgt = self.im = self.lens = None
         self.mrt_cost = self.mrt_valid = None
@@ -128,6 +129,10 @@
         grown = False
         if self.ws is None or self.ws.numel() < need:
             self.ws = torch.empty(int(need * 1.25), dtype=torch.float32, device=self.dev)
+            grown = True
+        need = L.lib().vag_handoff_planes_floats(B, Ts, Tt, self.H)
+        if need > 0 and (self.planes is None or self.planes.numel() < need):
+            self.planes = torch.empty(int(need * 1.25), dtype=torch.float32, device=self.dev)
             grown = True
         cap = (max(self.cap[0], B * Ts), max(self.cap[1], B * Tt), max(self.cap[2], B))
         if cap != self.cap:
@@ -182,7 +187,13 @@
             rng = dropout_rng(m, self.dev)
         if (int(phases) & 1) and not (self.dev.type == "cuda" and torch.cuda.is_current_stream_capturing()):
             self.executed += 1
-        call("vag_train_step", c.ref(), C.byref(self.w), C.byref(self.g), ptr(self.src, torch.int64),
-             ptr(self.lens, torch.int32), ptr(self.tgt, torch.int64), ptr(self.im) if self.mm else None, ptr(self.vw),
-             ptr(rng, torch.int64) if rng is not None else None, ptr(self.derived), ptr(self.ws), ptr(self.losses),
-             int(phases), stream())
+        if self.planes is not None:
+            call("vag_set_handoff_planes", ptr(self.planes), self.planes.numel())
+        try:
+            call("vag_train_step", c.ref(), C.byref(self.w), C.byref(self.g), ptr(self.src, torch.int64),
+                 ptr(self.lens, torch.int32), ptr(self.tgt, torch.int64), ptr(self.im) if self.mm else None, ptr(self.vw),
+                 ptr(rng, torch.int64) if rng is not None else None, ptr(self.derived), ptr(self.ws), ptr(self.losses),
+                 int(phases), stream())
+        finally:
+            if self.planes is not None:
+                call("vag_set_handoff_planes", None, 0)
diff --git a/vag-nmt_amd/vagnmt_hip/ops.py b/vag-nmt_amd/vagnmt_hip/ops.py
--- a/vag-nmt_amd/vagnmt_hip/ops.py
+++ b/vag-nmt_amd/vagnmt_hip/ops.py
@@ -30,6 +30,18 @@
 
 def _f32(*shape, like):
     return torch.empty(*shape, dtype=torch.float32, device=like.device)
+
+
+def _backward_recurrence_call(name, B, Ts, Tt, H, like, *args):
+    n = L.lib().vag_handoff_planes_floats(B, Ts, Tt, H)
+    if n <= 0:
+        return _recurrence_call(name, *args)
+    planes = _f32(n, like=like)
+    call("vag_set_handoff_planes", ptr(planes), n)
+    try:
+        return _recurrence_call(name, *args)
+    finally:
+        call("vag_set_handoff_planes", None, 0)
 
 
 def _zeros(*shape, like):
@@ -79,7 +91,7 @@
         d_enc = _c(d_enc)
         t = _grad_targets(ctx.gviews, ctx.saved_tensors[3:])
         g = [x[0] for x in t]
-        _recurrence_call("vag_bigru_seq_bwd", ptr(src, I64), ptr(lengths, torch.int32), gru_w(wf_ih, wf_hh, bf_ih, bf_hh),
+        _backward_recurrence_call("vag_bigru_seq_bwd", B, Ts, 0, H, d_enc, ptr(src, I64), ptr(lengths, torch.int32), gru_w(wf_ih, wf_hh, bf_ih, bf_hh),
              gru_w(wb_ih, wb_hh, bb_ih, bb_hh), p_emb, p_ctx, ptr(rng, torch.int64) if rng is not None else None,
              B, Ts, E, H, ptr(d_enc), ptr(ws), ptr(g[0]), gru_w(g[1], g[2], g[3], g[4]), gru_w(g[5], g[6], g[7], g[8]),
              stream())
@@ -227,7 +239,7 @@
         g = [x[0] for x in t]
         gdec = DecW(ptr(g[0]), gru_w(g[1], g[2], g[3], g[4]), ptr(g[5]), ptr(g[6]), ptr(g[7]),
                     gru_w(g[8], g[9], g[10], g[11]))
-        _recurrence_call("vag_cgru_attn_decode_seq_bwd", ptr(enc), ptr(pe), ptr(mask), ptr(h0), ptr(tok, I64), _dec_w(emb, dec),
+        _backward_recurrence_call("vag_cgru_attn_decode_seq_bwd", B, 0, Tt, H, enc, ptr(enc), ptr(pe), ptr(mask), ptr(h0), ptr(tok, I64), _dec_w(emb, dec),
              B, Ts, Tt, E, H, V, ptr(h2), ptr(c), ptr(e), ptr(d_h2), ptr(d_c), ptr(d_e), ptr(ws), ptr(d_enc), 0,
              ptr(d_pe), ptr(d_h0), gdec, ptr(scratch), stream())
         r = _ret(t)
```
